# nnaisense/evotorch

Measured on NVIDIA H100. Metric: PGPE generations/sec at popsize=1Mxdim=10k (Rastrigin, fp32), higher is better.
Workload: dtype f32

## Files before the change

### evotorch_b200/_native.py

```python

from __future__ import annotations

import ctypes
import os
from ctypes import c_float, c_int, c_int64, c_size_t, c_uint64, c_void_p
from typing import Optional

import torch

_PKG = os.path.dirname(os.path.abspath(__file__))
LIB_PATH = os.path.join(_PKG, "lib", "libevok.so")

_P = c_void_p
_SIGNATURES = {
    "evok_abi_version": (c_int, []),
    "evok_launch_count": (c_uint64, []),
    "evok_error_string": (ctypes.c_char_p, [c_int]),
    "evok_sample_eval": (c_int, [c_int, _P, c_int64, _P, _P, c_int64, c_int64, c_int64, c_int, c_uint64, c_uint64, _P, _P, _P]),
    "evok_eval": (c_int, [c_int, _P, c_int64, c_int64, c_int64, _P, _P]),
    "evok_rank_workspace_bytes": (c_size_t, [c_int64]),
    "evok_rank": (c_int, [c_int, _P, c_int64, c_int, _P, _P, _P, c_size_t, _P]),
    "evok_argsort": (c_int, [_P, c_int64, c_int, _P, _P, c_size_t, _P]),
    "evok_sample_batched": (c_int, [_P, c_int64, c_int64, _P, c_int64, _P, c_int64, c_int64, c_int64, c_int64, c_int, c_uint64, c_uint64, _P]),
    "evok_rank_batched": (c_int, [c_int, _P, c_int64, c_int64, c_int, _P, _P, c_size_t, _P]),
    "evok_elite_mask_batched": (c_int, [_P, c_int64, c_int64, c_int64, _P, _P, c_size_t, _P]),
    "evok_weights_adjust_batched": (c_int, [_P, c_int64, c_int64, c_int, _P]),
    "evok_grad_batched_workspace_bytes": (c_size_t, [c_int64, c_int64, c_int64]),
    "evok_grad_batched": (c_int, [c_int, _P, c_int64, c_int64, _P, _P, c_int64, _P, c_int64, c_int64, c_int64, c_int64, c_float, c_float, _P, _P, _P,
                                  c_size_t, _P]),
    "evok_clipup_batched": (c_int, [_P, c_int64, c_int64, _P, _P, _P, _P, _P, _P]),
    "evok_sigma_update_batched": (c_int, [_P, _P, c_int64, c_int64, _P, c_int, _P, _P, _P, _P]),
    "evok_rank_table": (c_int, [_P, c_int64, c_int, _P, _P, _P, c_size_t, _P]),
    "evok_cholesky_workspace_bytes": (c_size_t, [c_int64]),
    "evok_cholesky": (c_int, [_P, c_int64, c_int64, _P, c_int64, _P, c_size_t, _P]),
    "evok_cmaes_row_weights": (c_int, [_P, _P, c_int64, c_int64, c_int64, c_int, _P, _P, _P]),
    "evok_cmaes_vector_update": (c_int, [_P, _P, c_int64, _P, _P, _P, _P, _P, c_int64, _P, c_int, _P, _P, _P]),
    "evok_weights_adjust": (c_int, [_P, c_int64, c_int, _P]),
    "evok_elite_mask": (c_int, [_P, c_int64, c_int64, _P, _P, c_size_t, _P]),
    "evok_grad_workspace_bytes": (c_size_t, [c_int64, c_int64]),
    "evok_grad": (c_int, [c_int, _P, c_int64, _P, _P, _P, c_int64, c_int64, c_float, c_float, _P, _P, _P, c_size_t, _P]),
    "evok_grad_regen": (c_int, [c_int, _P, _P, _P, c_int64, c_int64, c_int64, c_uint64, c_uint64, _P, c_float, c_float, _P, _P, _P,
                                c_size_t, _P]),
    "evok_clipup_step": (c_int, [_P, c_int64, _P, c_float, c_float, c_float, _P, _P, _P]),
    "evok_adam_step": (c_int, [_P, c_int64, _P, _P, c_int64, c_float, c_float, c_float, c_float, _P, _P, _P]),
    "evok_sgd_step": (c_int, [_P, c_int64, _P, c_int, c_float, c_float, _P, _P, _P]),
    "evok_axpy": (c_int, [_P, c_int64, c_float, _P, _P]),
    "evok_sigma_update": (c_int, [_P, _P, c_int64, c_float, c_int, _P, c_float, _P, c_float, _P, c_float, _P]),
    "evok_cem_finalize": (c_int, [_P, _P, _P, c_int64, c_int64, _P, _P, _P]),
    "evok_mlp_parameter_length": (c_int64, [c_int, _P]),
    "evok_mlp_forward": (c_int, [_P, c_int64, _P, c_int64, _P, c_int64, c_int64, c_int, _P, _P, _P]),
    "evok_mlp_forward_prep": (c_int, [_P, c_int64, _P, c_int64, _P, c_int64, c_int64, c_int, _P, _P, _P, _P, _P, c_float, c_float, c_float, _P, _P,
                                      c_size_t, _P]),
    "evok_mlp_forward_shared_workspace_bytes": (c_size_t, [c_int64, c_int64, c_int, _P]),
    "evok_mlp_forward_shared": (c_int, [_P, c_int64, c_int64, _P, c_int64, c_int64, c_int, _P, _P, _P, _P, c_size_t, _P]),
    "evok_gemm_gather_rows": (c_int, [_P, c_int64, c_int64, c_int64, c_int64, _P, c_int64, c_int64, c_int64, c_int64, c_int, _P, c_int64, _P]),
    "evok_gemm_gather_rows_workspace_bytes": (c_size_t, [c_int64, c_int64]),
    "evok_gemm_gather_rows_ws": (c_int, [_P, c_int64, c_int64, c_int64, c_int64, _P, c_int64, c_int64, c_int64, c_int64, c_int, _P, c_int64, c_int, _P, c_size_t, _P]),
    "evok_gemm_workspace_bytes": (c_size_t, [c_int64, c_int64, c_int64]),
    "evok_gemm_nt": (c_int, [_P, c_int64, _P, c_int64, c_int64, c_int64, c_int64, _P, c_int64, _P, c_int64, _P, _P, _P, c_size_t, _P]),
    "evok_gemm_nt_affine": (c_int, [_P, c_int64, _P, c_int64, c_int64, c_int64, c_int64, _P, c_int64, _P, _P, c_int64, _P, _P, c_size_t, _P]),
    "evok_transpose_pair": (c_int, [_P, c_int64, c_int64, c_int64, _P, _P, _P, c_int64, _P]),
    "evok_transpose_scale": (c_int, [_P, c_int64, c_int64, c_int64, _P, _P, c_int64, _P]),
    "evok_peer_alloc": (c_int, [c_size_t, _P, _P]),
    "evok_peer_open": (c_int, [_P, _P]),
    "evok_peer_close": (c_int, [_P]),
    "evok_peer_free": (c_int, [_P]),
    "evok_sample_eval_push": (c_int, [c_int, _P, c_int64, _P, _P, c_int64, c_int64, c_int64, c_int, c_uint64, c_uint64, _P, c_int, c_int, _P, _P,
                                      _P, _P, _P]),
    "evok_peer_push": (c_int, [_P, c_int64, c_int64, c_int, c_int, _P, _P, _P, _P]),
    "evok_peer_wait": (c_int, [_P, c_int, _P, _P, c_uint64, _P]),
    "evok_grad_push": (c_int, [c_int, _P, c_int64, _P, _P, _P, c_int64, c_int64, c_int64, c_uint64, c_uint64, _P, c_float, c_float, c_int, c_int,
                               _P, _P, _P, _P, _P, c_size_t, _P]),
    "evok_rank_sharded": (c_int, [c_int, _P, c_int64, c_int, c_int, c_int, _P, _P, _P, _P, _P, _P, _P, c_uint64, _P, _P, _P, c_size_t, _P]),
    "evok_peer_reduce": (c_int, [_P, c_int, c_int64, _P, _P, _P, _P, c_uint64, _P, _P]),
}

EXPORTED_SYMBOLS = tuple(sorted(_SIGNATURES))

_lib: Optional[ctypes.CDLL] = None


class EvokError(RuntimeError):
    pass


def lib() -> ctypes.CDLL:
    global _lib
    if _lib is None:
        if not os.path.exists(LIB_PATH):
            raise EvokError(
                f"{LIB_PATH} is missing: the sm_90a kernel library has not been built. "
                "Run `python -m evotorch_b200.build` (needs nvcc). There is no CPU/torch fallback for CUDA problems."
            )
        handle = ctypes.CDLL(LIB_PATH)
        for name, (res, args) in _SIGNATURES.items():
            fn = getattr(handle, name)
            fn.restype = res
            fn.argtypes = args
        if handle.evok_abi_version() != 1:
            raise EvokError("libevok.so ABI version mismatch; rebuild with `python -m evotorch_b200.build --force`")
        _lib = handle
    return _lib


def available() -> bool:
    return os.path.exists(LIB_PATH)


def check(rc: int, what: str) -> None:
    if rc != 0:
        msg = lib().evok_error_string(rc).decode()
        if rc < 0:
            raise ValueError(f"{what}: {msg} (code {rc})")
        raise EvokError(f"{what}: CUDA error {rc}: {msg}")


def ptr(t: Optional[torch.Tensor]) -> Optional[int]:
    return None if t is None else t.data_ptr()


def stream_of(t: torch.Tensor) -> int:
    return torch.cuda.current_stream(t.device).cuda_stream


_workspaces: dict = {}


def workspace(device: torch.device, nbytes: int, tag: str = "ws") -> torch.Tensor:
    dev = device.index if device.index is not None else torch.cuda.current_device()
    key = (dev, torch.cuda.current_stream(dev).cuda_stream, tag) if _private_depth == 0 else (dev, tag)
    buf = _workspaces.get(key)
    if buf is None or buf.numel() < nbytes:
        buf = torch.empty(max(int(nbytes), 256), dtype=torch.uint8, device=device)
        _workspaces[key] = buf
    return buf


_private_depth = 0


class private_workspaces:

    def __enter__(self) -> dict:
        global _workspaces, _private_depth
        self._saved = _workspaces
        _workspaces = self.store = {}
        _private_depth += 1
        import gc

        self._gc_was_enabled = gc.isenabled()
        gc.collect()
        gc.disable()
        return self.store

    def __exit__(self, *exc):
        global _workspaces, _private_depth
        _workspaces = self._saved
        _private_depth -= 1
        if self._gc_was_enabled:
            import gc

            gc.enable()
        return False
```

### evotorch_b200/algorithms/gaussian.py

```python

from __future__ import annotations

import math
import os
from copy import deepcopy
from typing import Optional

import torch

from .. import ops
from ..core import LazySolutionBatch, PhiloxRecipe, Problem, SolutionBatch
from ..distributed import world
from ..distributions import Distribution, ExpGaussian, ExpSeparableGaussian, SeparableGaussian, SymmetricSeparableGaussian
from ..optimizers import get_optimizer_class
from ..tools.misc import modify_tensor, to_stdev_init
from .searchalgorithm import SearchAlgorithm, SinglePopulationAlgorithmMixin


class GaussianSearchAlgorithm(SearchAlgorithm, SinglePopulationAlgorithmMixin):

    DISTRIBUTION_TYPE = NotImplemented
    DISTRIBUTION_PARAMS = NotImplemented

    def __init__(self, problem: Problem, *, popsize: int, center_learning_rate: float, stdev_learning_rate: float,
                 stdev_init=None, radius_init=None, num_interactions: Optional[int] = None, popsize_max: Optional[int] = None,
                 optimizer=None, optimizer_config: Optional[dict] = None, ranking_method: Optional[str] = None, center_init=None,
                 stdev_min=None, stdev_max=None, stdev_max_change=None, obj_index: Optional[int] = None, distributed: bool = False,
                 popsize_weighted_grad_avg: Optional[bool] = None, ensure_even_popsize: bool = False):
        problem.ensure_numeric()
        problem.ensure_unbounded()
        SearchAlgorithm.__init__(self, problem, center=self._get_mu, stdev=self._get_sigma, mean_eval=self._get_mean_eval)
        self._num_interactions = None if num_interactions is None else int(num_interactions)
        if popsize_max is not None and num_interactions is None:
            raise ValueError("`popsize_max` was expected as None, because `num_interactions` is None."
                             " The argument `popsize_max` is meaningful only when `num_interactions` is given.")
        self._popsize_max = None if popsize_max is None else int(popsize_max)
        self._ensure_even_popsize = bool(ensure_even_popsize)
        if self._ensure_even_popsize and (int(popsize) % 2) != 0 and not distributed:
            raise ValueError(f"`popsize` was expected as an even number. However, the received `popsize` is {popsize}.")

        if center_init is None:
            mu = problem.generate_values(1).reshape(-1)
        else:
            mu = problem.ensure_tensor_length_and_dtype(center_init, allow_scalar=False, about="center_init").clone()
        stdev_init = to_stdev_init(solution_length=problem.solution_length, stdev_init=stdev_init, radius_init=radius_init)
        sigma = problem.ensure_tensor_length_and_dtype(stdev_init, about="stdev_init", allow_scalar=False).clone()

        dist_params = deepcopy(self.DISTRIBUTION_PARAMS) if self.DISTRIBUTION_PARAMS is not None else {}
        dist_params.update({"mu": mu, "sigma": sigma})
        self._distribution: Distribution = self.DISTRIBUTION_TYPE(dist_params, dtype=problem.dtype, device=problem.device)

        self._popsize = int(popsize)
        self._center_learning_rate = float(center_learning_rate)
        self._stdev_learning_rate = float(stdev_learning_rate)
        self._optimizer = self._initialize_optimizer(self._center_learning_rate, optimizer, optimizer_config)
        self._ranking_method = None if ranking_method is None else str(ranking_method)

        def bound(x, about):
            return None if x is None else problem.ensure_tensor_length_and_dtype(x, about=about, allow_scalar=True)

        self._stdev_min = bound(stdev_min, "stdev_min")
        self._stdev_max = bound(stdev_max, "stdev_max")
        self._stdev_max_change = bound(stdev_max_change, "stdev_max_change")

        def host_side(x):
            return None if x is None else (float(x) if x.ndim == 0 else x)

        self._kernel_bounds = dict(lb=host_side(self._stdev_min), ub=host_side(self._stdev_max), max_change=host_side(self._stdev_max_change))
        self._obj_index = problem.normalize_obj_index(obj_index)

        self._distributed = bool(distributed) and world()[1] > 1
        self._step = self._step_distributed if self._distributed else self._step_non_distributed
        if popsize_weighted_grad_avg is not None and not distributed:
            raise ValueError("The argument `popsize_weighted_grad_avg` can only be used in distributed mode.")

        self._mean_eval = None
        self._population: Optional[SolutionBatch] = None
        self._first_iter = True
        self._use_graph = os.environ.get("EVOTORCH_B200_CUDA_GRAPH", "0") == "1"
        self._graph = None
        SinglePopulationAlgorithmMixin.__init__(self, exclude="mean_eval", enable=(not self._distributed))

    def _initialize_optimizer(self, learning_rate: float, optimizer=None, optimizer_config: Optional[dict] = None):
        if optimizer is None:
            return None
        if isinstance(optimizer, str):
            cls = get_optimizer_class(optimizer, optimizer_config)
            return cls(stepsize=float(learning_rate), dtype=self._distribution.dtype, solution_length=self._distribution.solution_length,
                       device=self._distribution.device)
        return optimizer

    def __getstate__(self) -> dict:
        state = dict(self.__dict__)
        state["_graph"] = None
        state.pop("_graph_workspaces", None)
        return state

    def _fill_and_eval_pop(self):
        if self._num_interactions is not None:
            self._fill_and_eval_adaptive_pop()
            return
        if self._population is None:
            if self.problem.lazy_population:
                self._population = LazySolutionBatch(self.problem, self._popsize, device=self._distribution.device)
            else:
                self._population = SolutionBatch(self.problem, popsize=self._popsize, device=self._distribution.device, empty=True)
        self.problem.sample_and_evaluate(self._distribution, self._population)

    def _fill_and_eval_adaptive_pop(self):
        prob = self.problem
        first = prob.status.get("total_interaction_count", 0)
        populations, total = [], 0
        while True:
            newpop = SolutionBatch(prob, popsize=self._popsize, device=self._distribution.device, empty=True)
            total += len(newpop)
            prob.sample_and_evaluate(self._distribution, newpop)
            populations.append(newpop)
            if self._popsize_max is not None and total >= self._popsize_max:
                break
            if prob.status["total_interaction_count"] - first > self._num_interactions:
                break
        self._population = populations[0] if len(populations) == 1 else SolutionBatch.cat(populations)

    def enable_cuda_graph(self, enabled: bool = True):
        self._use_graph = bool(enabled)
        self._graph = None
        return self

    def _graph_capturable(self) -> bool:
        from ..optimizers import ClipUp

        dist, prob = self._distribution, self.problem
        ok = (self._num_interactions is None and isinstance(dist, SeparableGaussian) and ops.uses_kernels(dist.mu) and prob.rng == "philox"
              and prob.evok_objective_id is not None and len(prob.senses) == 1 and prob.eval_data_length == 0
              and (self._optimizer is None or isinstance(self._optimizer, ClipUp))
              and len(prob.before_eval_hook) == 0)
        if self._distributed:
            return (ok and not prob.stores_solution_stats and len(prob.before_eval_hook) == 0 and len(prob.after_eval_hook) == 0
                    and len(prob.before_grad_hook) == 0 and len(prob.after_grad_hook) == 0)
        return ok and self._population is not None

    def _update_in_place(self, gradients: dict):
        dist = self._distribution
        gmu = gradients["mu"].contiguous()
        if self._optimizer is not None:
            self._optimizer.ascent_into_(gmu, dist.mu)
        else:
            ops.axpy_(dist.mu, gmu, self._center_learning_rate)
        ops.sigma_update_(dist.sigma, gradients["sigma"].contiguous(), self._stdev_learning_rate, isinstance(dist, ExpSeparableGaussian),
                          **self._kernel_bounds)

    def _graph_body(self, base_stream: int, counter: torch.Tensor):
        dist, prob, pop = self._distribution, self.problem, self._population
        lazy = isinstance(pop, LazySolutionBatch)
        n = len(pop)
        fitnesses = pop._evdata.view(-1)
        if lazy:
            samples = PhiloxRecipe(seed=prob._philox_seed, stream_id=base_stream - 1, row0=0, n_rows=n, solution_length=prob.solution_length,
                                   symmetric=dist.SYMMETRIC, stream_offset=counter, mu=dist.mu, sigma=dist.sigma)
        else:
            samples = pop._data
        gradients = dist.compute_gradients(samples, fitnesses, objective_sense=prob.senses[self._obj_index], ranking_method=self._ranking_method)
        self._update_in_place(gradients)
        ops.sample_eval(prob.evok_objective_id, None if lazy else samples, dist.mu, dist.sigma, n_rows=n, symmetric=dist.SYMMETRIC,
                        seed=prob._philox_seed, stream_id=base_stream, f=fitnesses, stream_offset=counter)
        counter.add_(1)
        if lazy:
            pop.recipe = PhiloxRecipe(seed=prob._philox_seed, stream_id=base_stream - 1, row0=0, n_rows=n, solution_length=prob.solution_length,
                                      symmetric=dist.SYMMETRIC, stream_offset=counter, mu=dist.mu, sigma=dist.sigma)

    def _capture_graph(self):
        prob = self.problem
        dist = self._distribution
        if not (dist.mu.is_contiguous() and dist.sigma.is_contiguous()):
            self._distribution = dist = dist.modified_copy(mu=dist.mu.contiguous(), sigma=dist.sigma.contiguous())
        self._graph_counter = torch.zeros(1, dtype=torch.int32, device=dist.mu.device)
        self._graph_base_stream = prob._philox_stream
        graph = torch.cuda.CUDAGraph()
        before = ops.launch_count()
        from .. import _native as nat

        with nat.private_workspaces() as store, torch.cuda.graph(graph):
            self._graph_body(self._graph_base_stream, self._graph_counter)
        self._graph_workspaces = store
        self._graph_kernels = ops.launch_count() - before
        ops.count_replayed_launches(-self._graph_kernels)
        self._graph_counter.zero_()
        self._graph = graph

    def _step_graph(self):
        prob, pop = self.problem, self._population
        if self._graph is None:
            self._step_eager()
            self._capture_graph()
            return
        self._graph.replay()
        ops.count_replayed_launches(self._graph_kernels)
        prob._philox_stream += 1
        prob._finish_evaluation(pop)

    def _step_non_distributed(self):
        if self._first_iter:
            self._fill_and_eval_pop()
            self._first_iter = False
            return
        if self._use_graph and self._graph_capturable():
            self._step_graph()
        else:
            self._graph = None
            self._step_eager()

    def _step_eager(self):
        lazy = isinstance(self._population, LazySolutionBatch)
        samples = self._population.recipe if lazy else self._population.access_values(keep_evals=True)
        fitnesses = self._population.access_evals()[:, self._obj_index]
        gradients = self._distribution.compute_gradients(samples, fitnesses, objective_sense=self.problem.senses[self._obj_index],
                                                         ranking_method=self._ranking_method)
        self._update_distribution(gradients)
        self._fill_and_eval_pop()

    def _distributed_body(self, in_place: bool):
        fetched = self.problem.sample_and_compute_gradients(self._distribution, self._popsize, obj_index=self._obj_index,
                                                            num_interactions=self._num_interactions, popsize_max=self._popsize_max,
                                                            ranking_method=self._ranking_method,
                                                            ensure_even_popsize=self._ensure_even_popsize)
        if in_place:
            self._update_in_place(fetched[0]["gradients"])
        else:
            self._update_distribution(fetched[0]["gradients"])
        self._mean_eval = fetched[0]["mean_eval"]

    def _sync_initial_state(self):
        from ..distributed import broadcast_search_state

        dist_ = self._distribution
        tensors = [v for v in dist_.parameters.values() if isinstance(v, torch.Tensor)]
        opt = self._optimizer
        for name in ("_velocity", "_m", "_v", "_buf"):
            t = getattr(opt, name, None) if opt is not None else None
            if isinstance(t, torch.Tensor):
                tensors.append(t)
        broadcast_search_state(tensors)
        self._state_synced = True

    def _step_distributed(self):
        prob = self.problem
        if not self.__dict__.get("_state_synced", False):
            self._sync_initial_state()
        if os.environ.get("EVOTORCH_B200_PEER", "0") == "1" and getattr(prob, "_peer_exchange", None) is None and not self.__dict__.get("_peer_tried"):
            self._peer_tried = True
            from ..distributed import world
            from ..peer import enable_peer_exchange

            if world()[1] > 1 and ops.uses_kernels(self._distribution.mu) and prob.evok_objective_id is not None and prob.rng == "philox":
                enable_peer_exchange(prob, self._popsize)
        if not (self._use_graph and self._graph_capturable()):
            self._graph = None
            self._distributed_body(in_place=False)
            return
        if self._graph is None:
            if self._steps_count < 2:
                self._distributed_body(in_place=False)
                return
            dist = self._distribution
            self._distribution = dist = dist.modified_copy(mu=dist.mu.contiguous().clone(), sigma=dist.sigma.contiguous().clone())
            prob.philox_stream_offset = torch.zeros(1, dtype=torch.int32, device=dist.mu.device)
            base = prob._philox_stream
            torch.cuda.synchronize()
            graph = torch.cuda.CUDAGraph()
            before = ops.launch_count()
            from .. import _native as nat

            with nat.private_workspaces() as store, torch.cuda.graph(graph):
                self._distributed_body(in_place=True)
                prob.philox_stream_offset.add_(1)
            self._graph_workspaces = store
            self._graph_kernels = ops.launch_count() - before
            ops.count_replayed_launches(-self._graph_kernels)
            prob._philox_stream = base
            prob.philox_stream_offset.zero_()
            self._graph = graph
        self._graph.replay()
        ops.count_replayed_launches(self._graph_kernels)
        prob._philox_stream += 1

    def _update_distribution(self, gradients: dict):
        dist = self._distribution
        separable = isinstance(dist, SeparableGaussian)
        if separable and ops.uses_kernels(dist.mu) and ops.uses_kernels(gradients["mu"]):
            new_mu, new_sigma = dist.mu.clone(), dist.sigma.clone()
            gmu = gradients["mu"].contiguous()
            if self._optimizer is not None and hasattr(self._optimizer, "ascent_into_"):
                self._optimizer.ascent_into_(gmu, new_mu)
            elif self._optimizer is not None:
                new_mu += self._optimizer.ascent(gmu)
            else:
                ops.axpy_(new_mu, gmu, self._center_learning_rate)
            ops.sigma_update_(new_sigma, gradients["sigma"].contiguous(), self._stdev_learning_rate,
                              isinstance(dist, ExpSeparableGaussian), **self._kernel_bounds)
            self._distribution = dist.modified_copy(mu=new_mu, sigma=new_sigma)
            return

        controlled = (self._stdev_min is not None) or (self._stdev_max is not None) or (self._stdev_max_change is not None)
        old_sigma = dist.sigma if controlled else None
        learning_rates, optimizers = {}, {}
        if self._optimizer is not None:
            optimizers["mu"] = self._optimizer
        else:
            learning_rates["mu"] = self._center_learning_rate
        learning_rates["sigma"] = self._stdev_learning_rate
        updated = dist.update_parameters(gradients, learning_rates=learning_rates, optimizers=optimizers)
        if controlled:
            updated = updated.modified_copy(
                sigma=modify_tensor(old_sigma, updated.sigma, lb=self._stdev_min, ub=self._stdev_max, max_change=self._stdev_max_change))
        self._distribution = updated

    def _get_mu(self) -> torch.Tensor:
        mu = self._distribution.parameters["mu"]
        return mu.clone() if self._graph is not None else mu

    def _get_sigma(self) -> torch.Tensor:
        sigma = self._distribution.parameters["sigma"]
        return sigma.clone() if self._graph is not None else sigma

    def _get_mean_eval(self) -> Optional[float]:
        if self._population is None:
            return None if self._mean_eval is None else float(self._mean_eval)
        return float(torch.mean(self._population.evals[:, self._obj_index]))

    @property
    def optimizer(self):
        return None if self._optimizer is None else self._optimizer.contained_optimizer

    @property
    def population(self) -> Optional[SolutionBatch]:
        return self._population

    @property
    def obj_index(self) -> int:
        return self._obj_index


class PGPE(GaussianSearchAlgorithm):

    DISTRIBUTION_TYPE = NotImplemented
    DISTRIBUTION_PARAMS = NotImplemented

    def __init__(self, problem: Problem, *, popsize: int, center_learning_rate: float, stdev_learning_rate: float, stdev_init=None,
                 radius_init=None, num_interactions: Optional[int] = None, popsize_max: Optional[int] = None, optimizer="clipup",
                 optimizer_config: Optional[dict] = None, ranking_method: Optional[str] = "centered", center_init=None, stdev_min=None,
                 stdev_max=None, stdev_max_change=0.2, symmetric: bool = True, obj_index: Optional[int] = None,
                 distributed: bool = False, popsize_weighted_grad_avg: Optional[bool] = None):
        if symmetric:
            self.DISTRIBUTION_TYPE = SymmetricSeparableGaussian
            divide_by = "num_directions"
        else:
            self.DISTRIBUTION_TYPE = SeparableGaussian
            divide_by = "num_solutions"
        self.DISTRIBUTION_PARAMS = {"divide_mu_grad_by": divide_by, "divide_sigma_grad_by": divide_by}
        super().__init__(problem, popsize=popsize, center_learning_rate=center_learning_rate, stdev_learning_rate=stdev_learning_rate,
                         stdev_init=stdev_init, radius_init=radius_init, popsize_max=popsize_max, num_interactions=num_interactions,
                         optimizer=optimizer, optimizer_config=optimizer_config, ranking_method=ranking_method, center_init=center_init,
                         stdev_min=stdev_min, stdev_max=stdev_max, stdev_max_change=stdev_max_change, obj_index=obj_index,
                         distributed=distributed, popsize_weighted_grad_avg=popsize_weighted_grad_avg, ensure_even_popsize=symmetric)


def _default_popsize(n: int) -> int:
    return int(4 + math.floor(3 * math.log(n)))


class SNES(GaussianSearchAlgorithm):

    DISTRIBUTION_TYPE = ExpSeparableGaussian
    DISTRIBUTION_PARAMS = None

    def __init__(self, problem: Problem, *, stdev_init=None, radius_init=None, popsize: Optional[int] = None,
                 center_learning_rate: Optional[float] = None, stdev_learning_rate: Optional[float] = None,
                 scale_learning_rate: bool = True, num_interactions: Optional[int] = None, popsize_max: Optional[int] = None,
                 optimizer=None, optimizer_config: Optional[dict] = None, ranking_method: Optional[str] = "nes", center_init=None,
                 stdev_min=None, stdev_max=None, stdev_max_change=None, obj_index: Optional[int] = None, distributed: bool = False,
                 popsize_weighted_grad_avg: Optional[bool] = None):
        n = problem.solution_length
        if popsize is None:
            popsize = _default_popsize(n)
        if center_learning_rate is None:
            center_learning_rate = 1.0
        default_lr = 0.2 * (3 + math.log(n)) / math.sqrt(n)
        if stdev_learning_rate is None:
            stdev_learning_rate = default_lr
        else:
            stdev_learning_rate = float(stdev_learning_rate) * (default_lr if scale_learning_rate else 1.0)
        super().__init__(problem, popsize=popsize, center_learning_rate=center_learning_rate, stdev_learning_rate=stdev_learning_rate,
                         stdev_init=stdev_init, radius_init=radius_init, popsize_max=popsize_max, num_interactions=num_interactions,
                         optimizer=optimizer, optimizer_config=optimizer_config, ranking_method=ranking_method, center_init=center_init,
                         stdev_min=stdev_min, stdev_max=stdev_max, stdev_max_change=stdev_max_change, obj_index=obj_index,
                         distributed=distributed, popsize_weighted_grad_avg=popsize_weighted_grad_avg)


class CEM(GaussianSearchAlgorithm):

    DISTRIBUTION_TYPE = SeparableGaussian
    DISTRIBUTION_PARAMS = NotImplemented

    def __init__(self, problem: Problem, *, popsize: int, parenthood_ratio: float, stdev_init=None, radius_init=None,
                 num_interactions: Optional[int] = None, popsize_max: Optional[int] = None, center_init=None, stdev_min=None,
                 stdev_max=None, stdev_max_change=None, obj_index: Optional[int] = None, distributed: bool = False,
                 popsize_weighted_grad_avg: Optional[bool] = None):
        self.DISTRIBUTION_PARAMS = {"parenthood_ratio": float(parenthood_ratio)}
        super().__init__(problem, popsize=popsize, center_learning_rate=1.0, stdev_learning_rate=1.0, stdev_init=stdev_init,
                         radius_init=radius_init, popsize_max=popsize_max, num_interactions=num_interactions, optimizer=None,
                         optimizer_config=None, ranking_method=None, center_init=center_init, stdev_min=stdev_min, stdev_max=stdev_max,
                         stdev_max_change=stdev_max_change, obj_index=obj_index, distributed=distributed,
                         popsize_weighted_grad_avg=popsize_weighted_grad_avg)


class XNES(GaussianSearchAlgorithm):

    DISTRIBUTION_TYPE = ExpGaussian
    DISTRIBUTION_PARAMS = None

    def __init__(self, problem: Problem, *, stdev_init=None, radius_init=None, popsize: Optional[int] = None,
                 center_learning_rate: Optional[float] = None, stdev_learning_rate: Optional[float] = None,
                 scale_learning_rate: bool = True, num_interactions: Optional[int] = None, popsize_max: Optional[int] = None,
                 optimizer=None, optimizer_config: Optional[dict] = None, ranking_method: Optional[str] = "nes", center_init=None,
                 obj_index: Optional[int] = None, distributed: bool = False, popsize_weighted_grad_avg: Optional[bool] = None):
        n = problem.solution_length
        if popsize is None:
            popsize = _default_popsize(n)
        if center_learning_rate is None:
            center_learning_rate = 1.0
        default_lr = 0.6 * (3 + math.log(n)) / (n * math.sqrt(n))
        if stdev_learning_rate is None:
            stdev_learning_rate = default_lr
        else:
            stdev_learning_rate = float(stdev_learning_rate) * (default_lr if scale_learning_rate else 1.0)
        super().__init__(problem, popsize=popsize, center_learning_rate=center_learning_rate, stdev_learning_rate=stdev_learning_rate,
                         stdev_init=stdev_init, radius_init=radius_init, popsize_max=popsize_max, num_interactions=num_interactions,
                         optimizer=optimizer, optimizer_config=optimizer_config, ranking_method=ranking_method, center_init=center_init,
                         stdev_min=None, stdev_max=None, stdev_max_change=None, obj_index=obj_index, distributed=distributed,
                         popsize_weighted_grad_avg=popsize_weighted_grad_avg)
```

### evotorch_b200/core.py

```python

from __future__ import annotations

import math
from typing import Any, Callable, Iterable, Optional, Union

import torch

from . import ops
from .tools.cloning import Clonable
from .tools.hook import Hook
from .tools.readonlytensor import as_read_only_tensor
from .tools.misc import ensure_tensor_length_and_dtype, extract_generator, make_gaussian, make_uniform, to_torch_dtype

ObjectiveSense = Union[str, Iterable[str]]


class Problem(Clonable):

    def __init__(self, objective_sense: ObjectiveSense, objective_func: Optional[Callable] = None, *, initial_bounds=None, bounds=None,
                 solution_length: Optional[int] = None, dtype=None, eval_dtype=None, device=None, eval_data_length: Optional[int] = None,
                 seed: Optional[int] = None, num_actors=None, actor_config=None, num_gpus_per_actor=None, num_subbatches=None,
                 subbatch_size=None, store_solution_stats: Optional[bool] = None, vectorized: Optional[bool] = None,
                 rng: Optional[str] = None, lazy_population: bool = False):
        if num_actors not in (None, 0, 1):
            import warnings

            warnings.warn(
                f"num_actors={num_actors!r}: evotorch_b200 has no Ray actors. The population is evaluated by this process"
                " (or sharded over the torch.distributed ranks when launched with torchrun and distributed=True is given to the"
                " searcher; see evotorch_b200.distributed).", stacklevel=2)
        self._requested_num_actors = num_actors
        self._dtype = torch.float32 if dtype is None else to_torch_dtype(dtype)
        if eval_dtype is None:
            self._eval_dtype = self._dtype if self._dtype.is_floating_point else torch.float32
        else:
            self._eval_dtype = to_torch_dtype(eval_dtype)
        self._device = torch.device("cpu") if device is None else torch.device(device)
        if solution_length is None:
            raise ValueError(f"Together with a numeric dtype ({self._dtype!r}), expected to receive `solution_length` as an integer."
                             " However, `solution_length` is None.")
        self._solution_length = int(solution_length)

        if isinstance(objective_sense, str):
            senses = [objective_sense]
        else:
            senses = list(objective_sense)
            if len(senses) == 0:
                raise ValueError("Encountered an empty sequence via `objective_sense`.")
        for s in senses:
            if s not in ("min", "max"):
                raise ValueError(f"Invalid objective sense: {s!r}. Instead, please provide the objective sense as 'min' or 'max'.")
        self._senses = senses
        self._objective_sense = objective_sense

        self._initial_lower_bounds = self._initial_upper_bounds = None
        self._lower_bounds = self._upper_bounds = None
        if bounds is not None and initial_bounds is None:
            initial_bounds = bounds
        if initial_bounds is not None:
            self._initial_lower_bounds, self._initial_upper_bounds = self._process_bounds(initial_bounds)
        if bounds is not None:
            self._lower_bounds, self._upper_bounds = self._process_bounds(bounds)

        self._objective_func = objective_func
        if objective_func is None:
            if vectorized is not None:
                raise ValueError("This problem object received no external fitness function; `vectorized` must be left as None.")
            self._vectorized = None
        elif getattr(objective_func, "__evotorch_vectorized__", False):
            if vectorized is not None:
                raise ValueError("Received a fitness function that was decorated via @vectorized; `vectorized` must be left as None.")
            self._vectorized = True
        else:
            self._vectorized = bool(vectorized)

        self._eval_data_length = 0 if eval_data_length is None else int(eval_data_length)
        self._store_solution_stats = None if store_solution_stats is None else bool(store_solution_stats)
        self._best = self._worst = None
        self._best_evals = self._worst_evals = None
        self._after_eval_status: dict = {}
        self._before_eval_hook, self._after_eval_hook = Hook(), Hook()

        self._generator = torch.Generator(device=self._device)
        self._seed = None
        self.manual_seed(seed)
        if rng is None:
            rng = "philox" if self._device.type == "cuda" and self._dtype == torch.float32 else "torch"
        if rng not in ("philox", "torch"):
            raise ValueError(f"rng must be 'philox' or 'torch', got {rng!r}")
        self.rng = rng
        self.lazy_population = bool(lazy_population)

    def _process_bounds(self, pair) -> tuple:
        lb, ub = pair
        out = []
        for b in (lb, ub):
            t = torch.as_tensor(b, dtype=self._dtype, device=self._device)
            if t.ndim not in (0, 1):
                raise ValueError(f"Lower and upper bounds are expected as scalars or as 1-dimensional vectors, got shape {tuple(t.shape)}.")
            if t.ndim == 1 and len(t) != self._solution_length:
                raise ValueError(f"Boundary vectors must have length {self._solution_length}, got {len(t)}.")
            out.append(t)
        return tuple(out)

    def manual_seed(self, seed: Optional[int] = None):
        if seed is None:
            seed = int(torch.randint(0, 2**62, (1,)).item())
            self._seed = None
        else:
            self._seed = int(seed)
        self._generator.manual_seed(int(seed))
        self._philox_seed = int(seed) & 0xFFFFFFFFFFFFFFFF
        self._philox_stream = 0
        self.philox_row0 = 0
        self.philox_stream_offset = None

    def next_philox_stream(self) -> tuple:
        sid = self._philox_stream
        self._philox_stream += 1
        return self._philox_seed, sid

    @property
    def dtype(self) -> torch.dtype:
        return self._dtype

    @property
    def eval_dtype(self) -> torch.dtype:
        return self._eval_dtype

    @property
    def device(self) -> torch.device:
        return self._device

    @property
    def generator(self) -> torch.Generator:
        return self._generator

    @property
    def has_own_generator(self) -> bool:
        return True

    @property
    def objective_sense(self) -> ObjectiveSense:
        return self._senses[0] if len(self._senses) == 1 else self._senses

    @property
    def senses(self) -> list:
        return self._senses

    @property
    def is_single_objective(self) -> bool:
        return len(self._senses) == 1

    @property
    def is_multi_objective(self) -> bool:
        return len(self._senses) > 1

    @property
    def solution_length(self) -> int:
        return self._solution_length

    @property
    def eval_data_length(self) -> int:
        return self._eval_data_length

    @property
    def initial_lower_bounds(self):
        return self._initial_lower_bounds

    @property
    def initial_upper_bounds(self):
        return self._initial_upper_bounds

    @property
    def lower_bounds(self):
        return self._lower_bounds

    @property
    def upper_bounds(self):
        return self._upper_bounds

    @property
    def num_actors(self) -> int:
        return 0

    @property
    def actors(self):
        return None

    @property
    def is_main(self) -> bool:
        return True

    @property
    def is_remote(self) -> bool:
        return False

    @property
    def before_eval_hook(self) -> Hook:
        return self._before_eval_hook

    @property
    def after_eval_hook(self) -> Hook:
        return self._after_eval_hook

    @property
    def before_grad_hook(self) -> Hook:
        return self.__dict__.setdefault("_before_grad_hook", Hook())

    @property
    def after_grad_hook(self) -> Hook:
        return self.__dict__.setdefault("_after_grad_hook", Hook())

    def is_on_cpu(self) -> bool:
        return str(self._device) == "cpu"

    def kill_actors(self):
        """No-op: there are no Ray actors here (one process per GPU replaces them, distributed.py)."""

    @property
    def all_remote_problems(self):
        raise NotImplementedError("Ray actors are out of scope: shard the population over GPUs with torchrun (evotorch_b200/distributed.py)")

    @property
    def status(self) -> dict:
        return self._after_eval_status

    @property
    def stores_solution_stats(self) -> Optional[bool]:
        return self._store_solution_stats

    @property
    def evok_objective_id(self) -> Optional[int]:
        return getattr(self._objective_func, "evok_objective_id", None)

    def _tm(self, dtype, device, use_eval_dtype=False):
        if dtype is None:
            dtype = self._eval_dtype if use_eval_dtype else self._dtype
        return to_torch_dtype(dtype), (self._device if device is None else torch.device(device))

    def _size(self, size, num_solutions):
        if num_solutions is not None:
            if len(size) > 0:
                raise ValueError("Provide either a size or `num_solutions`, not both.")
            return (int(num_solutions), self._solution_length)
        if len(size) == 1 and isinstance(size[0], (tuple, list, torch.Size)):
            return tuple(size[0])
        return tuple(int(s) for s in size)

    def make_tensor(self, data, *, dtype=None, device=None, use_eval_dtype: bool = False) -> torch.Tensor:
        dt, dev = self._tm(dtype, device, use_eval_dtype)
        return torch.as_tensor(data, dtype=dt, device=dev) if isinstance(data, torch.Tensor) else torch.tensor(data, dtype=dt, device=dev)

    def _target(self, size, num_solutions, out, dtype, device, use_eval_dtype) -> torch.Tensor:
        if out is not None:
            if len(size) > 0 or num_solutions is not None or dtype is not None or device is not None or use_eval_dtype:
                raise ValueError("When `out` is given, the arguments `size`, `num_solutions`, `dtype`, `device`, `use_eval_dtype` are not expected")
            return out
        dt, dev = self._tm(dtype, device, use_eval_dtype)
        return torch.empty(self._size(size, num_solutions), dtype=dt, device=dev)

    def make_empty(self, *size, num_solutions=None, out=None, dtype=None, device=None, use_eval_dtype: bool = False) -> torch.Tensor:
        return self._target(size, num_solutions, out, dtype, device, use_eval_dtype)

    def make_zeros(self, *size, num_solutions=None, out=None, dtype=None, device=None, use_eval_dtype: bool = False) -> torch.Tensor:
        return self._target(size, num_solutions, out, dtype, device, use_eval_dtype).zero_()

    def make_ones(self, *size, num_solutions=None, out=None, dtype=None, device=None, use_eval_dtype: bool = False) -> torch.Tensor:
        return self._target(size, num_solutions, out, dtype, device, use_eval_dtype).fill_(1)

    def make_nan(self, *size, num_solutions=None, out=None, dtype=None, device=None, use_eval_dtype: bool = False) -> torch.Tensor:
        return self._target(size, num_solutions, out, dtype, device, use_eval_dtype).fill_(float("nan"))

    def make_I(self, size=None, *, out=None, dtype=None, device=None, use_eval_dtype: bool = False) -> torch.Tensor:
        if isinstance(size, tuple):
            if len(size) != 1:
                raise ValueError(f"When the size argument is given as a tuple, the method `make_I(...)` expects the tuple to have only one"
                                 f" element. The given tuple is {size}.")
            size = size[0]
        if out is not None:
            if size is not None or dtype is not None or device is not None or use_eval_dtype:
                raise ValueError("When `out` is given, the arguments `size`, `dtype`, `device`, `use_eval_dtype` are not expected")
            if out.ndim != 2 or out.shape[0] != out.shape[1]:
                raise ValueError(f"`out` was expected as a square matrix, but its shape is {tuple(out.shape)}")
            out.zero_()
            out.fill_diagonal_(1)
            return out
        dt, dev = self._tm(dtype, device, use_eval_dtype)
        return torch.eye(self._solution_length if size is None else int(size), dtype=dt, device=dev)

    def make_gaussian(self, *size, num_solutions=None, center=None, stdev=None, symmetric: bool = False, out=None, dtype=None,
                      device=None, use_eval_dtype: bool = False, generator=None) -> torch.Tensor:
        out = self._target(size, num_solutions, out, dtype, device, use_eval_dtype)
        return make_gaussian(out=out, center=center, stdev=stdev, symmetric=symmetric,
                             generator=self._generator if generator is None else generator)

    def make_uniform(self, *size, num_solutions=None, lb=None, ub=None, out=None, dtype=None, device=None, use_eval_dtype: bool = False,
                     generator=None) -> torch.Tensor:
        out = self._target(size, num_solutions, out, dtype, device, use_eval_dtype)
        return make_uniform(out=out, lb=lb, ub=ub, generator=self._generator if generator is None else generator)

    def make_randint(self, *size, n, num_solutions=None, out=None, dtype=None, device=None, use_eval_dtype: bool = False,
                     generator=None) -> torch.Tensor:
        out = self._target(size, num_solutions, out, dtype, device, use_eval_dtype)
        gen = extract_generator(self._generator if generator is None else generator)
        n = int(n)
        if out.dtype.is_floating_point:
            out.copy_(torch.randint(0, n, out.shape, generator=gen, device=out.device, dtype=torch.int64))
        else:
            out.random_(0, n, generator=gen)
        return out

    def make_uniform_shaped_like(self, t: torch.Tensor, *, lb=None, ub=None) -> torch.Tensor:
        return self.make_uniform(out=torch.empty_like(t), lb=lb, ub=ub)

    def make_gaussian_shaped_like(self, t: torch.Tensor, *, center=None, stdev=None) -> torch.Tensor:
        return self.make_gaussian(out=torch.empty_like(t), center=center, stdev=stdev)

    def ensure_tensor_length_and_dtype(self, t: Any, *, allow_scalar: bool = False, about: Optional[str] = None) -> torch.Tensor:
        return ensure_tensor_length_and_dtype(t, self._solution_length, self._dtype, about=about, allow_scalar=allow_scalar,
                                              device=self._device)

    def generate_values(self, num_solutions: int) -> torch.Tensor:
        result = torch.empty(int(num_solutions), self._solution_length, dtype=self._dtype, device=self._device)
        self._fill(result)
        return result

    def _fill(self, values: torch.Tensor):
        if self._initial_lower_bounds is None or self._initial_upper_bounds is None:
            raise RuntimeError(
                "The default implementation of the method `_fill(...)` does not know how to initialize solutions because it appears"
                " that this Problem object was not given neither `initial_bounds` nor `bounds` during the moment of initialization."
            )
        return self.make_uniform(out=values, lb=self._initial_lower_bounds, ub=self._initial_upper_bounds)

    def generate_batch(self, popsize: Optional[int] = None, *, empty: bool = False, center=None, stdev=None,
                       symmetric: bool = False) -> "SolutionBatch":
        if (center is None) != (stdev is None):
            raise ValueError("The arguments `center` and `stdev` were expected to be None or non-None at the same time.")
        if center is None:
            if symmetric:
                raise ValueError("The argument `symmetric` can be set as True only when `center` and `stdev` are provided.")
            return SolutionBatch(self, popsize, empty=empty, device=self._device)
        if empty:
            raise ValueError("When `center` and `stdev` are provided, the argument `empty` must be False.")
        result = SolutionBatch(self, popsize, device=self._device, empty=True)
        self.make_gaussian(out=result.access_values(), center=center, stdev=stdev, symmetric=symmetric)
        return result

    def ensure_numeric(self):
        if not (self._dtype.is_floating_point or self._dtype in (torch.int32, torch.int64, torch.int16, torch.int8)):
            raise ValueError("Expected a problem with numeric dtype.")

    def ensure_unbounded(self):
        if self._lower_bounds is not None or self._upper_bounds is not None:
            raise ValueError("Expected an unbounded problem. However, this problem object has its `lower_bounds` and/or `upper_bounds` set.")

    def ensure_single_objective(self):
        if len(self._senses) != 1:
            raise ValueError(f"Expected a single-objective problem, but this problem has {len(self._senses)} objectives.")

    def normalize_obj_index(self, obj_index: Optional[int] = None) -> int:
        n = len(self._senses)
        if obj_index is None:
            if n == 1:
                return 0
            raise ValueError("This problem has multiple objectives: `obj_index` must be given.")
        obj_index = int(obj_index)
        if not (-n <= obj_index < n):
            raise IndexError(f"Objective index out of range: {obj_index}")
        return obj_index % n

    @torch.no_grad()
    def evaluate(self, x: Union["SolutionBatch", "Solution"]):
        if isinstance(x, Solution):
            batch = x.to_batch()
        elif isinstance(x, SolutionBatch):
            batch = x
        else:
            raise TypeError(f"The method `evaluate(...)` expected a Solution or a SolutionBatch as its argument, got {type(x)!r}.")
        self._before_eval_hook(batch)
        self._evaluate_all(batch)
        self._finish_evaluation(batch)

    @property
    def aux_device(self) -> torch.device:
        if self._device.type == "cpu":
            return torch.device("cuda") if torch.cuda.is_available() else self._device
        return self._device

    def _device_of_fitness_function(self) -> Optional[torch.device]:
        for fn in (self._objective_func, self._evaluate_batch, self._evaluate):
            if fn is None:
                continue
            if getattr(fn, "__evotorch_on_aux_device__", False):
                return self.aux_device
            if hasattr(fn, "device"):
                return torch.device(fn.device)
        return None

    def _evaluate_all(self, batch: "SolutionBatch"):
        wanted = self._device_of_fitness_function()
        if wanted is None or torch.device(wanted) == batch.device:
            self._evaluate_batch(batch)
            return
        moved = batch.to(wanted)
        self._evaluate_batch(moved)
        batch._evdata[:] = moved._evdata.to(batch.device)

    def _finish_evaluation(self, batch: "SolutionBatch"):
        self._after_eval_status = {}
        self._after_eval_status.update(self._get_best_and_worst(batch))
        self._after_eval_status.update(self._extra_status(batch))
        self._after_eval_status.update(self._after_eval_hook.accumulate_dict(batch))

    def _extra_status(self, batch: "SolutionBatch") -> dict:
        return {}

    def _evaluate_batch(self, batch: "SolutionBatch"):
        if self._vectorized and self._objective_func is not None:
            result = self._objective_func(batch.values)
            if isinstance(result, tuple):
                batch.set_evals(*result)
            else:
                batch.set_evals(result)
        else:
            for sln in batch:
                self._evaluate(sln)

    def _evaluate(self, solution: "Solution"):
        if self._objective_func is None:
            raise NotImplementedError
        result = self._objective_func(solution.values)
        if isinstance(result, tuple):
            solution.set_evals(*result)
        else:
            solution.set_evals(result)

    def _get_best_and_worst(self, batch: "SolutionBatch") -> dict:
        if self._store_solution_stats is None:
            self._store_solution_stats = str(batch.device) == "cpu"
        if not self._store_solution_stats:
            return {}
        nobjs = len(self._senses)
        if self._best is None:
            self._best, self._worst = [None] * nobjs, [None] * nobjs
            self._best_evals = [math.inf if s == "min" else -math.inf for s in self._senses]
            self._worst_evals = [-math.inf if s == "min" else math.inf for s in self._senses]
        for i, sense in enumerate(self._senses):
            scores = batch.access_evals(i)
            ibest, iworst = batch.argbest(i), batch.argworst(i)
            best_score, worst_score = float(scores[ibest]), float(scores[iworst])
            better = best_score < self._best_evals[i] if sense == "min" else best_score > self._best_evals[i]
            worse = worst_score > self._worst_evals[i] if sense == "min" else worst_score < self._worst_evals[i]
            if better:
                self._best_evals[i], self._best[i] = best_score, batch[int(ibest)].clone()
            if worse:
                self._worst_evals[i], self._worst[i] = worst_score, batch[int(iworst)].clone()
        if nobjs == 1:
            return dict(best=self._best[0], worst=self._worst[0], best_eval=float(self._best[0].evals[0]),
                        worst_eval=float(self._worst[0].evals[0]))
        return {"best": self._best, "worst": self._worst}

    _TRANSIENT = ("_peer_exchange", "_active_peer", "_grad_batches", "_grad_scratch", "_d2h_stage")

    def __getstate__(self) -> dict:
        state = {k: v for k, v in self.__dict__.items() if k not in self._TRANSIENT}
        state["philox_stream_offset"] = None
        return state

    def sample_and_evaluate(self, distribution, batch: "SolutionBatch"):
        obj = self.evok_objective_id
        if isinstance(batch, LazySolutionBatch):
            if not (obj is not None and self.rng == "philox" and len(self._senses) == 1 and hasattr(distribution, "SYMMETRIC")
                    and ops.uses_kernels(distribution.mu)):
                raise ValueError("a lazy population needs a built-in objective, rng='philox', a separable Gaussian and CUDA float32")
            n = len(batch)
            if distribution.SYMMETRIC and n % 2 != 0:
                raise ValueError(f"Symmetric sampling cannot be done if the number of solutions is odd: {n}")
            seed, stream_id = self.next_philox_stream()
            mu, sigma = distribution.mu.contiguous(), distribution.sigma.contiguous()
            batch.recipe = PhiloxRecipe(seed=seed, stream_id=stream_id, row0=self.philox_row0, n_rows=n, solution_length=self._solution_length,
                                        symmetric=distribution.SYMMETRIC, stream_offset=self.philox_stream_offset, mu=mu, sigma=sigma)
            self._before_eval_hook(batch)
            peer = getattr(self, "_active_peer", None)
            if peer is not None:
                ops.sample_eval_push(obj, None, mu, sigma, n_rows=n, symmetric=distribution.SYMMETRIC, seed=seed, stream_id=stream_id,
                                     row0=self.philox_row0, peer=peer, stream_offset=self.philox_stream_offset)
            else:
                ops.sample_eval(obj, None, mu, sigma, n_rows=n, symmetric=distribution.SYMMETRIC, seed=seed, stream_id=stream_id,
                                row0=self.philox_row0, f=batch._evdata.view(-1), stream_offset=self.philox_stream_offset)
            self._finish_evaluation(batch)
            return
        values = batch.access_values()
        fused = (obj is not None and self.rng == "philox" and ops.uses_kernels(values) and len(self._senses) == 1
                 and hasattr(distribution, "SYMMETRIC") and ops.uses_kernels(distribution.mu) and len(self._before_eval_hook) == 0)
        if not fused:
            distribution.sample(out=values, generator=self)
            self.evaluate(batch)
            return
        n = values.shape[0]
        if distribution.SYMMETRIC and n % 2 != 0:
            raise ValueError(f"Symmetric sampling cannot be done if the leftmost dimension of the target tensor is odd: {tuple(values.shape)}")
        seed, stream_id = self.next_philox_stream()
        evdata = batch._evdata
        direct = evdata.shape[1] == 1 and evdata.dtype == torch.float32 and evdata.is_contiguous()
        f = evdata.view(-1) if direct else torch.empty(n, dtype=torch.float32, device=values.device)
        peer = getattr(self, "_active_peer", None)
        if peer is not None:
            ops.sample_eval_push(obj, values, distribution.mu.contiguous(), distribution.sigma.contiguous(), n_rows=n,
                                 symmetric=distribution.SYMMETRIC, seed=seed, stream_id=stream_id, row0=self.philox_row0, peer=peer,
                                 stream_offset=self.philox_stream_offset)
            self._finish_evaluation(batch)
            return
        ops.sample_eval(obj, values, distribution.mu.contiguous(), distribution.sigma.contiguous(), n_rows=n,
                        symmetric=distribution.SYMMETRIC, seed=seed, stream_id=stream_id, row0=self.philox_row0, f=f,
                        stream_offset=self.philox_stream_offset)
        if not direct:
            batch.set_evals(f)
        self._finish_evaluation(batch)

    def sample_and_compute_gradients(self, distribution, popsize: int, *, num_interactions: Optional[int] = None,
                                     popsize_max: Optional[int] = None, obj_index: Optional[int] = None,
                                     ranking_method: Optional[str] = None, with_stats: bool = True,
                                     ensure_even_popsize: bool = False):
        from .distributed import adaptive_sample_and_gradients, sharded_sample_and_gradients

        popsize = int(popsize)
        if ensure_even_popsize and popsize % 2 != 0:
            popsize += 1
        obj_index = self.normalize_obj_index(obj_index)
        hooks = self.__dict__
        if len(hooks.get("_before_grad_hook", ())) >= 1:
            hooks["_before_grad_hook"]()
        if num_interactions is not None:
            result = adaptive_sample_and_gradients(self, distribution, popsize, num_interactions=int(num_interactions),
                                                   popsize_max=None if popsize_max is None else int(popsize_max), obj_index=obj_index,
                                                   ranking_method=ranking_method)
        else:
            result = sharded_sample_and_gradients(self, distribution, popsize, obj_index=obj_index, ranking_method=ranking_method)
        if len(hooks.get("_after_grad_hook", ())) >= 1:
            self._after_eval_status = hooks["_after_grad_hook"].accumulate_dict([result])
        return [result] if with_stats else result["gradients"]

    def _get_local_interaction_count(self) -> int:
        if "total_interaction_count" in self._after_eval_status:
            return int(self._after_eval_status["total_interaction_count"])
        raise NotImplementedError

    def compare_solutions(self, a: "Solution", b: "Solution", obj_index: Optional[int] = None) -> float:
        i = self.normalize_obj_index(obj_index)
        sign = 1.0 if self._senses[i] == "max" else -1.0
        return sign * float(a.evals[i] - b.evals[i])

    def is_better(self, a, b, obj_index=None) -> bool:
        return self.compare_solutions(a, b, obj_index) > 0

    def is_worse(self, a, b, obj_index=None) -> bool:
        return self.compare_solutions(a, b, obj_index) < 0


class SolutionBatch:

    def __init__(self, problem: Optional[Problem] = None, popsize: Optional[int] = None, *, device=None, slice_of=None,
                 like: Optional["SolutionBatch"] = None, merging_of: Iterable = None, empty: Optional[bool] = None):
        if slice_of is not None:
            source, sl = slice_of
            self._data = source._data[sl]
            self._evdata = source._evdata[sl]
            self._senses = source._senses
            self._num_objs = source._num_objs
            return
        if merging_of is not None:
            batches = list(merging_of)
            self._data = torch.cat([b._data for b in batches], dim=0)
            self._evdata = torch.cat([b._evdata for b in batches], dim=0)
            self._senses = batches[0]._senses
            self._num_objs = batches[0]._num_objs
            return
        if like is not None and problem is None:
            popsize = len(like) if popsize is None else int(popsize)
            device = like.device if device is None else device
            self._data = torch.empty(popsize, like._data.shape[1], dtype=like._data.dtype, device=device)
            self._evdata = torch.full((popsize, like._evdata.shape[1]), float("nan"), dtype=like._evdata.dtype, device=device)
            self._senses, self._num_objs = like._senses, like._num_objs
            return
        if problem is None or popsize is None:
            if like is not None and problem is not None and popsize is None:
                popsize = len(like)
            else:
                raise ValueError("SolutionBatch needs `problem` and `popsize` (or `like`, `slice_of`, `merging_of`).")
        device = problem.device if device is None else torch.device(device)
        popsize = int(popsize)
        self._senses = problem.senses
        self._num_objs = len(problem.senses)
        self._data = torch.empty(popsize, problem.solution_length, dtype=problem.dtype, device=device)
        self._evdata = torch.full((popsize, self._num_objs + problem.eval_data_length), float("nan"), dtype=problem.eval_dtype,
                                  device=device)
        if not empty:
            problem._fill(self._data)

    def __len__(self) -> int:
        return self._data.shape[0]

    def __iter__(self):
        for i in range(len(self)):
            yield self[i]

    def __getitem__(self, i):
        if isinstance(i, slice):
            return SolutionBatch(slice_of=(self, i))
        if isinstance(i, (list, torch.Tensor)):
            return self.take(i)
        i = int(i)
        n = len(self)
        if not (-n <= i < n):
            raise IndexError(f"Solution index out of range: {i}")
        return Solution(self, i % n)

    @property
    def device(self) -> torch.device:
        return self._data.device

    @property
    def dtype(self) -> torch.dtype:
        return self._data.dtype

    values_dtype = dtype

    @property
    def eval_dtype(self) -> torch.dtype:
        return self._evdata.dtype

    @property
    def values_shape(self) -> torch.Size:
        return self._data.shape

    @property
    def eval_shape(self) -> torch.Size:
        return self._evdata.shape

    @property
    def solution_length(self) -> int:
        return self._data.shape[1]

    @property
    def senses(self) -> list:
        return self._senses

    @property
    def objective_sense(self):
        return self._senses[0] if len(self._senses) == 1 else self._senses

    @property
    def values(self) -> torch.Tensor:
        return as_read_only_tensor(self._data)

    @property
    def evals(self) -> torch.Tensor:
        return as_read_only_tensor(self._evdata)

    def access_values(self, *, keep_evals: bool = False) -> torch.Tensor:
        if not keep_evals:
            self.forget_evals()
        return self._data

    def access_evals(self, obj_index: Optional[int] = None) -> torch.Tensor:
        return self._evdata if obj_index is None else self._evdata[:, self._normalize_obj_index(obj_index)]

    def forget_evals(self, *, solutions=None):
        if solutions is None:
            self._evdata.fill_(float("nan"))
        else:
            self._evdata[solutions] = float("nan")

    def _normalize_obj_index(self, i) -> int:
        if i is None:
            if self._num_objs != 1:
                raise ValueError("The objective index was expected as an integer (multi-objective batch).")
            return 0
        i = int(i)
        if not (-self._num_objs <= i < self._num_objs):
            raise IndexError(f"Objective index out of range: {i}")
        return i % self._num_objs

    def set_values(self, values: Any, *, solutions=None):
        if solutions is None:
            solutions = slice(None, None, None)
        self._data[solutions] = torch.as_tensor(values, dtype=self._data.dtype, device=self._data.device)
        self._evdata[solutions] = float("nan")

    def set_evals(self, evals: torch.Tensor, eval_data: Optional[torch.Tensor] = None, *, solutions=None):
        if solutions is None:
            solutions = slice(None, None, None)
        num_solutions = self._evdata[solutions].shape[0]
        evals = torch.as_tensor(evals, dtype=self._evdata.dtype, device=self._evdata.device)
        if evals.ndim == 1:
            if self._num_objs != 1 and eval_data is None and evals.shape[0] == num_solutions:
                raise ValueError("A 1-dimensional `evals` tensor can only be used with single-objective problems.")
            evals = evals.reshape(-1, 1)
        elif evals.ndim != 2:
            raise ValueError(f"`evals` was expected with 1 or 2 dimensions, got shape {tuple(evals.shape)}")
        if evals.shape[0] != num_solutions:
            raise ValueError(f"Number of evaluation results ({evals.shape[0]}) does not match the number of solutions ({num_solutions}).")
        total_cols = self._evdata.shape[1]
        if eval_data is not None:
            eval_data = torch.as_tensor(eval_data, dtype=self._evdata.dtype, device=self._evdata.device).reshape(num_solutions, -1)
            if evals.shape[1] != self._num_objs or eval_data.shape[1] != total_cols - self._num_objs:
                raise ValueError("Shapes of `evals` / `eval_data` do not match the problem's objectives / eval_data_length.")
            self._evdata[solutions, : self._num_objs] = evals
            self._evdata[solutions, self._num_objs:] = eval_data
        elif evals.shape[1] == total_cols:
            self._evdata[solutions] = evals
        elif evals.shape[1] == self._num_objs:
            self._evdata[solutions, : self._num_objs] = evals
            self._evdata[solutions, self._num_objs:] = float("nan")
        else:
            raise ValueError(f"`evals` has {evals.shape[1]} columns; expected {self._num_objs} or {total_cols}.")

    def _sort_keys(self, obj_index) -> tuple:
        i = self._normalize_obj_index(obj_index)
        return self._evdata[:, i], self._senses[i] == "max"

    def argsort(self, obj_index: Optional[int] = None) -> torch.Tensor:
        keys, descending = self._sort_keys(obj_index)
        if ops.uses_kernels(keys):
            return ops.argsort(keys.contiguous(), descending)
        return torch.argsort(keys, descending=descending, stable=True)

    def argbest(self, obj_index: Optional[int] = None) -> torch.Tensor:
        keys, is_max = self._sort_keys(obj_index)
        return torch.argmax(keys) if is_max else torch.argmin(keys)

    def argworst(self, obj_index: Optional[int] = None) -> torch.Tensor:
        keys, is_max = self._sort_keys(obj_index)
        return torch.argmin(keys) if is_max else torch.argmax(keys)

    def utility(self, obj_index: Optional[int] = None, *, ranking_method: Optional[str] = None) -> torch.Tensor:
        from .tools.ranking import rank

        keys, is_max = self._sort_keys(obj_index)
        return rank(keys, "raw" if ranking_method is None else ranking_method, higher_is_better=is_max)

    def utils(self, *, ranking_method: Optional[str] = None) -> torch.Tensor:
        return torch.stack([self.utility(i, ranking_method=ranking_method) for i in range(self._num_objs)], dim=1)

    def take(self, indices: Iterable) -> "SolutionBatch":
        idx = torch.as_tensor(indices, device=self._data.device)
        out = SolutionBatch(like=self, popsize=len(idx))
        out._data[:] = self._data[idx]
        out._evdata[:] = self._evdata[idx]
        return out

    def take_best(self, n: int, *, obj_index: Optional[int] = None) -> "SolutionBatch":
        return self.take(self.argsort(obj_index)[: int(n)])

    def split(self, num_pieces: Optional[int] = None, *, max_size: Optional[int] = None) -> list:
        n = len(self)
        if (num_pieces is None) == (max_size is None):
            raise ValueError("Provide exactly one of `num_pieces` and `max_size`.")
        if num_pieces is None:
            num_pieces = math.ceil(n / int(max_size))
        from .tools.misc import split_workload

        pieces, start = [], 0
        for share in split_workload(n, int(num_pieces)):
            pieces.append(SolutionBatch(slice_of=(self, slice(start, start + share))))
            start += share
        return pieces

    def concat(self, other: Union["SolutionBatch", Iterable]) -> "SolutionBatch":
        others = [other] if isinstance(other, SolutionBatch) else list(other)
        return SolutionBatch(merging_of=[self, *others])

    @staticmethod
    def cat(solution_batches: Iterable) -> "SolutionBatch":
        return SolutionBatch(merging_of=list(solution_batches))

    def to(self, device) -> "SolutionBatch":
        if torch.device(device) == self.device:
            return self
        out = SolutionBatch(like=self, device=device)
        out._data[:] = self._data.to(device)
        out._evdata[:] = self._evdata.to(device)
        return out

    def clone(self) -> "SolutionBatch":
        out = SolutionBatch(like=self)
        out._data[:] = self._data
        out._evdata[:] = self._evdata
        return out

    def __copy__(self) -> "SolutionBatch":
        return self.clone()

    def __deepcopy__(self, memo) -> "SolutionBatch":
        return self.clone()

    def __repr__(self) -> str:
        return f"<SolutionBatch: {len(self)} x {self.solution_length}, {self.dtype}, {self.device}>"


class PhiloxRecipe:

    def __init__(self, *, seed: int, stream_id: int, row0: int, n_rows: int, solution_length: int, symmetric: bool,
                 stream_offset: Optional[torch.Tensor], mu: torch.Tensor, sigma: torch.Tensor):
        self.seed, self.stream_id, self.row0, self.n_rows = seed, stream_id, row0, n_rows
        self.solution_length, self.symmetric, self.stream_offset = solution_length, symmetric, stream_offset
        self.mu, self.sigma = mu, sigma

    @property
    def shape(self) -> tuple:
        return (self.n_rows, self.solution_length)

    def materialize(self) -> torch.Tensor:
        out = torch.empty(self.n_rows, self.solution_length, dtype=torch.float32, device=self.mu.device)
        ops.sample_eval(ops.OBJ_NONE, out, self.mu, self.sigma, n_rows=self.n_rows, symmetric=self.symmetric, seed=self.seed,
                        stream_id=self.stream_id, row0=self.row0, stream_offset=self.stream_offset)
        return out


class LazySolutionBatch(SolutionBatch):

    def __init__(self, problem: "Problem", popsize: int, *, device=None):
        device = problem.device if device is None else torch.device(device)
        self._senses = problem.senses
        self._num_objs = len(problem.senses)
        self._popsize, self._solution_length = int(popsize), problem.solution_length
        self._values_dtype = problem.dtype
        self._evdata = torch.full((int(popsize), self._num_objs + problem.eval_data_length), float("nan"), dtype=problem.eval_dtype,
                                  device=device)
        self.recipe: Optional[PhiloxRecipe] = None

    @property
    def _data(self) -> torch.Tensor:
        if self.recipe is None:
            raise ValueError("This lazy population has not been sampled yet.")
        return self.recipe.materialize()

    def __len__(self) -> int:
        return self._popsize

    @property
    def device(self) -> torch.device:
        return self._evdata.device

    @property
    def dtype(self) -> torch.dtype:
        return self._values_dtype

    values_dtype = dtype

    @property
    def solution_length(self) -> int:
        return self._solution_length

    @property
    def values_shape(self) -> torch.Size:
        return torch.Size((self._popsize, self._solution_length))

    def access_values(self, *, keep_evals: bool = False) -> torch.Tensor:
        if not keep_evals:
            raise ValueError("The decision values of a lazy population are read-only (they are a function of the Philox counters).")
        return self._data

    def set_values(self, values: Any, *, solutions=None):
        raise ValueError("The decision values of a lazy population are read-only (they are a function of the Philox counters).")

    def __getitem__(self, i):
        if isinstance(i, (slice, list, torch.Tensor)):
            raise NotImplementedError("slicing a lazy population is not supported; use `.values` to materialise it")
        i = int(i) % self._popsize
        out = SolutionBatch(like=None, problem=None, popsize=None, slice_of=(_Materialized(self, i), slice(0, 1)))
        return Solution(out, 0)

    def __repr__(self) -> str:
        return f"<LazySolutionBatch: {self._popsize} x {self._solution_length}, {self.device}>"


class _Materialized:

    def __init__(self, lazy: LazySolutionBatch, i: int):
        r = lazy.recipe
        first = (i // 2) * 2 if r.symmetric else i
        rows = 2 if r.symmetric else 1
        block = torch.empty(rows, r.solution_length, dtype=torch.float32, device=r.mu.device)
        ops.sample_eval(ops.OBJ_NONE, block, r.mu, r.sigma, n_rows=rows, symmetric=r.symmetric, seed=r.seed, stream_id=r.stream_id,
                        row0=r.row0 + first, stream_offset=r.stream_offset)
        self._data = block[i - first: i - first + 1]
        self._evdata = lazy._evdata[i: i + 1]
        self._senses, self._num_objs = lazy._senses, lazy._num_objs


class Solution:

    def __init__(self, parent: SolutionBatch, index: int):
        self._batch = parent[int(index): int(index) + 1]

    @property
    def values(self) -> torch.Tensor:
        return as_read_only_tensor(self._batch._data[0])

    @property
    def evals(self) -> torch.Tensor:
        return as_read_only_tensor(self._batch._evdata[0])

    @property
    def evaluation(self) -> torch.Tensor:
        return as_read_only_tensor(self._batch._evdata[0])

    def access_values(self, *, keep_evals: bool = False) -> torch.Tensor:
        return self._batch.access_values(keep_evals=keep_evals)[0]

    def access_evals(self) -> torch.Tensor:
        return self._batch.access_evals()[0]

    def set_values(self, values: Any):
        self._batch.set_values(torch.as_tensor(values, dtype=self._batch.dtype, device=self._batch.device).reshape(1, -1))

    def set_evals(self, evals, eval_data=None):
        evals = torch.as_tensor(evals, dtype=self._batch.eval_dtype, device=self._batch.device).reshape(1, -1)
        if eval_data is not None:
            eval_data = torch.as_tensor(eval_data, dtype=self._batch.eval_dtype, device=self._batch.device).reshape(1, -1)
        self._batch.set_evals(evals, eval_data)

    set_evaluation = set_evals

    @property
    def is_evaluated(self) -> bool:
        n = self._batch._num_objs
        return not bool(torch.any(torch.isnan(self._batch._evdata[0, :n])))

    @property
    def senses(self) -> list:
        return self._batch.senses

    @property
    def objective_sense(self):
        return self._batch.objective_sense

    @property
    def dtype(self) -> torch.dtype:
        return self._batch.dtype

    @property
    def eval_dtype(self) -> torch.dtype:
        return self._batch.eval_dtype

    @property
    def device(self) -> torch.device:
        return self._batch.device

    @property
    def shape(self) -> torch.Size:
        return self.values.shape

    def __len__(self) -> int:
        return self._batch.solution_length

    def __iter__(self):
        return iter(self.values)

    def __getitem__(self, i):
        return self.values[i]

    def clone(self) -> "Solution":
        return Solution(self._batch.clone(), 0)

    def __copy__(self) -> "Solution":
        return self.clone()

    def __deepcopy__(self, memo) -> "Solution":
        return self.clone()

    def to(self, device) -> "Solution":
        return Solution(self._batch.to(device), 0)

    def to_batch(self) -> SolutionBatch:
        return self._batch

    def __repr__(self) -> str:
        return f"<Solution values={self.values}, evals={self.evals}>"
```

### evotorch_b200/csrc/evok_grad.cu

```cuda
#include <cstdlib>

#include "evok_common.cuh"

#ifndef EVOK_GRAD_TMA_DEFAULT
#define EVOK_GRAD_TMA_DEFAULT 1
#endif

namespace evok {

#ifndef EVOK_GRAD_UNROLL
#define EVOK_GRAD_UNROLL 4
#endif
#ifndef EVOK_GRAD_MINB
#define EVOK_GRAD_MINB 4
#endif
#ifndef EVOK_GRAD_CTAS_PER_SM
#define EVOK_GRAD_CTAS_PER_SM 4
#endif
constexpr int kGradThreads = 256;
constexpr int kGradUnroll = EVOK_GRAD_UNROLL;
constexpr int kMaxResidentCtas = kNumSMs * 8;

template <int VEC>
struct VecF;
template <>
struct VecF<4> {
  float v[4];
};
template <>
struct VecF<1> {
  float v[1];
};

template <int VEC>
__device__ __forceinline__ VecF<VEC> load_row(const float* p) {
  VecF<VEC> r;
  if (VEC == 4) {
    const float4 t = ld_stream4(p);
    r.v[0] = t.x; r.v[1] = t.y; r.v[2] = t.z; r.v[3] = t.w;
  } else {
    r.v[0] = ld_stream1(p);
  }
  return r;
}

struct GradItems {
  int64_t x, w, mu, sigma, partial;
};

template <int VEC, int TX, bool SYM, bool REGEN>
__global__ void __launch_bounds__(kGradThreads, EVOK_GRAD_MINB)
    grad_partial_kernel(int form, const float* __restrict__ X, int64_t ldx, const float* __restrict__ w, const float* __restrict__ mu,
                        const float* __restrict__ sigma, int64_t n_units, int64_t D, int64_t units_per_chunk, uint64_t unit0,
                        const __grid_constant__ PhiloxKey key, const uint32_t* __restrict__ stream_off, float* __restrict__ partial,
                        const __grid_constant__ GradItems items) {
  constexpr int TY = kGradThreads / TX;
  if (gridDim.z > 1) {
    const int64_t item = blockIdx.z;
    X += item * items.x;
    w += item * items.w;
    mu += item * items.mu;
    sigma += item * items.sigma;
    partial += item * items.partial;
  }
  const uint32_t sw = key.stream_lo + ((REGEN && stream_off) ? __ldg(stream_off) : 0u);
  const int tx = threadIdx.x % TX, ty = threadIdx.x / TX;
  const int64_t col = ((int64_t)blockIdx.x * TX + tx) * VEC;
  const bool active = col < D;

  float m[VEC], c1[VEC], c0[VEC], sg[VEC];
#pragma unroll
  for (int c = 0; c < VEC; ++c) {
    const bool ok = active && (col + c < D);
    const float s = ok ? __ldg(sigma + col + c) : 1.0f;
    m[c] = ok ? __ldg(mu + col + c) : 0.0f;
    sg[c] = s;
    if (form == EVOK_GRAD_EXP) {
      c1[c] = __fdiv_rn(1.0f, s * s);
      c0[c] = 1.0f;
    } else if (form == EVOK_GRAD_MOMENTS) {
      c1[c] = 1.0f;
      c0[c] = 0.0f;
    } else {
      c1[c] = __fdiv_rn(1.0f, s);
      c0[c] = s;
    }
  }

  float s1[VEC], s2[VEC];
#pragma unroll
  for (int c = 0; c < VEC; ++c) s1[c] = s2[c] = 0.0f;

  const int64_t r_begin = (int64_t)blockIdx.y * units_per_chunk;
  const int64_t r_end = min(n_units, r_begin + units_per_chunk);

  for (int64_t r0 = r_begin + ty; r0 < r_end; r0 += (int64_t)TY * kGradUnroll) {
    float a[kGradUnroll], b[kGradUnroll];
    bool need[kGradUnroll];
    VecF<VEC> x[kGradUnroll];
#pragma unroll
    for (int u = 0; u < kGradUnroll; ++u) {
      const int64_t r = r0 + (int64_t)u * TY;
      a[u] = b[u] = 0.0f;
      if (r < r_end) {
        if (SYM) {
          const float wp = __ldg(w + 2 * r), wm = __ldg(w + 2 * r + 1);
          a[u] = 0.5f * (wp - wm);
          b[u] = 0.5f * (wp + wm);
        } else {
          a[u] = b[u] = __ldg(w + r);
        }
      }
      need[u] = active && (a[u] != 0.0f || b[u] != 0.0f);
    }
#pragma unroll
    for (int u = 0; u < kGradUnroll; ++u) {
      const int64_t r = r0 + (int64_t)u * TY;
      if (need[u]) {
        if (REGEN) {
          if (VEC == 4) {
            normals4(key, sw, unit0 + (uint64_t)r, (uint32_t)(col >> 2), x[u].v);
          } else {
            float z[4];
            normals4(key, sw, unit0 + (uint64_t)r, (uint32_t)(col >> 2), z);
            x[u].v[0] = z[col & 3];
          }
        } else {
          x[u] = load_row<VEC>(X + (SYM ? 2 * r : r) * ldx + col);
        }
      }
    }
#pragma unroll
    for (int u = 0; u < kGradUnroll; ++u) {
      if (need[u]) {
#pragma unroll
        for (int c = 0; c < VEC; ++c) {
          const float e = REGEN ? sg[c] * x[u].v[c] : x[u].v[c] - m[c];
          s1[c] = fmaf(a[u], e, s1[c]);
          s2[c] = fmaf(b[u], fmaf(e * e, c1[c], -c0[c]), s2[c]);
        }
      }
    }
  }

  __shared__ float red[TY > 1 ? TY : 1][TX][2 * VEC];
  if (TY > 1) {
#pragma unroll
    for (int c = 0; c < VEC; ++c) {
      red[ty][tx][c] = s1[c];
      red[ty][tx][VEC + c] = s2[c];
    }
    __syncthreads();
    if (ty == 0) {
#pragma unroll
      for (int c = 0; c < VEC; ++c) {
        float t1 = red[0][tx][c], t2 = red[0][tx][VEC + c];
        for (int y = 1; y < TY; ++y) {
          t1 += red[y][tx][c];
          t2 += red[y][tx][VEC + c];
        }
        s1[c] = t1;
        s2[c] = t2;
      }
    }
  }
  if (ty == 0 && active) {
    float* p1 = partial + ((int64_t)blockIdx.y * 2 + 0) * D + col;
    float* p2 = partial + ((int64_t)blockIdx.y * 2 + 1) * D + col;
#pragma unroll
    for (int c = 0; c < VEC; ++c) {
      if (col + c < D) {
        p1[c] = s1[c];
        p2[c] = s2[c];
      }
    }
  }
}

__global__ void __launch_bounds__(256) grad_finalize_kernel(const float* __restrict__ partial, int n_chunks, int64_t D, float scale_mu,
                                                            float scale_sigma, float* __restrict__ out_mu, float* __restrict__ out_sigma,
                                                            int64_t item_stride_partial = 0) {
  const int64_t j = (int64_t)blockIdx.x * blockDim.x + threadIdx.x;
  if (j >= D) return;
  partial += (int64_t)blockIdx.y * item_stride_partial;
  out_mu += (int64_t)blockIdx.y * D;
  out_sigma += (int64_t)blockIdx.y * D;
  float t1 = 0.0f, t2 = 0.0f;
  for (int c = 0; c < n_chunks; ++c) {
    t1 += partial[((int64_t)c * 2 + 0) * D + j];
    t2 += partial[((int64_t)c * 2 + 1) * D + j];
  }
  out_mu[j] = t1 * scale_mu;
  out_sigma[j] = t2 * scale_sigma;
}

struct GradPush {
  PeerSink sink;
  const unsigned long long* epoch;
  unsigned int* done;
};

__global__ void __launch_bounds__(256) grad_finalize_push_kernel(const float* __restrict__ partial, int n_chunks, int64_t D, float scale_mu,
                                                                 float scale_sigma, const __grid_constant__ PeerSink sink,
                                                                 const unsigned long long* epoch, unsigned int* done) {
  const int64_t j = (int64_t)blockIdx.x * blockDim.x + threadIdx.x;
  if (j < D) {
    float t1 = 0.0f, t2 = 0.0f;
    for (int c = 0; c < n_chunks; ++c) {
      t1 += partial[((int64_t)c * 2 + 0) * D + j];
      t2 += partial[((int64_t)c * 2 + 1) * D + j];
    }
    t1 *= scale_mu;
    t2 *= scale_sigma;
    for (int p = 0; p < sink.world; ++p) {
      float* slot = static_cast<float*>(sink.data[p]) + (int64_t)sink.rank * 2 * D;
      slot[j] = t1;
      slot[D + j] = t2;
    }
  }
  peer_signal_tail(sink, epoch, done);
}

static int launch_finalize(const float* partial, int n_chunks, int64_t D, float scale_mu, float scale_sigma, float* out_mu, float* out_sigma,
                           const GradPush* push, cudaStream_t st) {
  const unsigned grid = (unsigned)((D + 255) / 256);
  if (push) grad_finalize_push_kernel<<<grid, 256, 0, st>>>(partial, n_chunks, D, scale_mu, scale_sigma, push->sink, push->epoch, push->done);
  else grad_finalize_kernel<<<grid, 256, 0, st>>>(partial, n_chunks, D, scale_mu, scale_sigma, out_mu, out_sigma);
  EVOK_CHECK_LAUNCH();
  return 0;
}

#ifndef EVOK_GRAD_TMA_ROWS
#define EVOK_GRAD_TMA_ROWS 4
#endif
#ifndef EVOK_GRAD_TMA_STAGES
#define EVOK_GRAD_TMA_STAGES 4
#endif
#ifndef EVOK_GRAD_TMA_CTAS_PER_SM
#define EVOK_GRAD_TMA_CTAS_PER_SM 3
#endif
constexpr int kTmaRows = EVOK_GRAD_TMA_ROWS;
constexpr int kTmaStages = EVOK_GRAD_TMA_STAGES;
constexpr int kTmaCols = 1024;
constexpr int kTmaConsumers = 256;
constexpr int kTmaThreads = kTmaConsumers + 32;
constexpr size_t kTmaSmemBytes = (size_t)kTmaStages * kTmaRows * kTmaCols * sizeof(float) + 2 * kTmaStages * sizeof(uint64_t) + 128;

__device__ __forceinline__ uint32_t smem_u32(const void* p) { return (uint32_t)__cvta_generic_to_shared(p); }
__device__ __forceinline__ void mbar_init(uint64_t* bar, uint32_t count) {
  asm volatile("mbarrier.init.shared::cta.b64 [%0], %1;" ::"r"(smem_u32(bar)), "r"(count) : "memory");
}
__device__ __forceinline__ void mbar_expect_tx(uint64_t* bar, uint32_t bytes) {
  asm volatile("mbarrier.arrive.expect_tx.shared::cta.b64 _, [%0], %1;" ::"r"(smem_u32(bar)), "r"(bytes) : "memory");
}
__device__ __forceinline__ void mbar_arrive(uint64_t* bar) {
  asm volatile("mbarrier.arrive.shared::cta.b64 _, [%0];" ::"r"(smem_u32(bar)) : "memory");
}
__device__ __forceinline__ void mbar_wait(uint64_t* bar, uint32_t parity) {
  asm volatile(
      "{\n"
      ".reg .pred P1;\n"
      "LAB_WAIT:\n"
      "mbarrier.try_wait.parity.shared::cta.b64 P1, [%0], %1;\n"
      "@P1 bra DONE;\n"
      "bra LAB_WAIT;\n"
      "DONE:\n"
      "}" ::"r"(smem_u32(bar)), "r"(parity) : "memory");
}
__device__ __forceinline__ void bulk_load(void* dst_smem, const void* src_gmem, uint32_t bytes, uint64_t* bar) {
  asm volatile("cp.async.bulk.shared::cluster.global.mbarrier::complete_tx::bytes [%0], [%1], %2, [%3];" ::"r"(smem_u32(dst_smem)),
               "l"(src_gmem), "r"(bytes), "r"(smem_u32(bar))
               : "memory");
}

template <bool SYM>
__global__ void __launch_bounds__(kTmaThreads, EVOK_GRAD_TMA_CTAS_PER_SM)
    grad_partial_tma_kernel(int form, const float* __restrict__ X, int64_t ldx, const float* __restrict__ w, const float* __restrict__ mu,
                            const float* __restrict__ sigma, int64_t n_units, int64_t D, int64_t units_per_chunk,
                            float* __restrict__ partial) {
  extern __shared__ __align__(128) unsigned char smem_raw[];
  float* tiles = reinterpret_cast<float*>(smem_raw);
  uint64_t* full = reinterpret_cast<uint64_t*>(smem_raw + (size_t)kTmaStages * kTmaRows * kTmaCols * sizeof(float));
  uint64_t* empty = full + kTmaStages;

  const int tid = threadIdx.x, warp = tid >> 5, lane = tid & 31;
  const int64_t col0 = (int64_t)blockIdx.x * kTmaCols;
  const int64_t width = min((int64_t)kTmaCols, D - col0);
  const int64_t r_begin = (int64_t)blockIdx.y * units_per_chunk;
  const int64_t r_end = min(n_units, r_begin + units_per_chunk);
  const int64_t n_rows = r_end - r_begin;
  const int64_t n_groups = (n_rows + kTmaRows - 1) / kTmaRows;
  const int64_t row_stride = (SYM ? 2 : 1) * ldx;

  if (tid == 0) {
    for (int s = 0; s < kTmaStages; ++s) {
      mbar_init(&full[s], 1);
      mbar_init(&empty[s], kTmaConsumers / 32);
    }
    asm volatile("fence.mbarrier_init.release.cluster;" ::: "memory");
  }
  __syncthreads();

  if (warp == kTmaConsumers / 32) {
    if (lane == 0) {
      const uint32_t row_bytes = (uint32_t)(width * sizeof(float));
      for (int64_t g = 0; g < n_groups; ++g) {
        const int s = (int)(g % kTmaStages);
        const uint32_t use = (uint32_t)(g / kTmaStages);
        if (use > 0) mbar_wait(&empty[s], (use - 1) & 1);
        const int64_t r0 = r_begin + g * kTmaRows;
        const int rows = (int)min((int64_t)kTmaRows, r_end - r0);
        mbar_expect_tx(&full[s], rows * row_bytes);
        float* dst = tiles + (size_t)s * kTmaRows * kTmaCols;
        for (int i = 0; i < rows; ++i) bulk_load(dst + (size_t)i * kTmaCols, X + (r0 + i) * row_stride + col0, row_bytes, &full[s]);
      }
    }
    return;
  }

  const int64_t col = col0 + (int64_t)tid * 4;
  const bool active = col < D;
  float m[4], c1[4], c0[4];
#pragma unroll
  for (int c = 0; c < 4; ++c) {
    const float sg = active ? __ldg(sigma + col + c) : 1.0f;
    m[c] = active ? __ldg(mu + col + c) : 0.0f;
    if (form == EVOK_GRAD_EXP) {
      c1[c] = __fdiv_rn(1.0f, sg * sg);
      c0[c] = 1.0f;
    } else if (form == EVOK_GRAD_MOMENTS) {
      c1[c] = 1.0f;
      c0[c] = 0.0f;
    } else {
      c1[c] = __fdiv_rn(1.0f, sg);
      c0[c] = sg;
    }
  }
  float s1[4] = {0.f, 0.f, 0.f, 0.f}, s2[4] = {0.f, 0.f, 0.f, 0.f};

  for (int64_t g = 0; g < n_groups; ++g) {
    const int s = (int)(g % kTmaStages);
    const uint32_t use = (uint32_t)(g / kTmaStages);
    const int64_t r0 = r_begin + g * kTmaRows;
    const int rows = (int)min((int64_t)kTmaRows, r_end - r0);
    float a[kTmaRows], b[kTmaRows];
#pragma unroll
    for (int i = 0; i < kTmaRows; ++i) {
      a[i] = b[i] = 0.0f;
      if (i < rows) {
        if (SYM) {
          const float wp = __ldg(w + 2 * (r0 + i)), wm = __ldg(w + 2 * (r0 + i) + 1);
          a[i] = 0.5f * (wp - wm);
          b[i] = 0.5f * (wp + wm);
        } else {
          a[i] = b[i] = __ldg(w + r0 + i);
        }
      }
    }
    mbar_wait(&full[s], use & 1);
    const float4* tile = reinterpret_cast<const float4*>(tiles + (size_t)s * kTmaRows * kTmaCols) + tid;
    if (active) {
#pragma unroll
      for (int i = 0; i < kTmaRows; ++i) {
        if (i < rows) {
          const float4 v = tile[(size_t)i * (kTmaCols / 4)];
          const float x[4] = {v.x, v.y, v.z, v.w};
#pragma unroll
          for (int c = 0; c < 4; ++c) {
            const float e = x[c] - m[c];
            s1[c] = fmaf(a[i], e, s1[c]);
            s2[c] = fmaf(b[i], fmaf(e * e, c1[c], -c0[c]), s2[c]);
          }
        }
      }
    }
    __syncwarp();
    if (lane == 0) mbar_arrive(&empty[s]);
  }
  if (active) {
    float* p1 = partial + ((int64_t)blockIdx.y * 2 + 0) * D + col;
    float* p2 = partial + ((int64_t)blockIdx.y * 2 + 1) * D + col;
#pragma unroll
    for (int c = 0; c < 4; ++c) {
      p1[c] = s1[c];
      p2[c] = s2[c];
    }
  }
}

struct GradPlan {
  int vec, tx, n_coltiles, n_chunks;
  int64_t units_per_chunk;
};

static GradPlan plan_grad(int64_t n_units, int64_t D, bool vec_ok) {
  GradPlan p;
  p.vec = vec_ok ? 4 : 1;
  const int64_t col_threads = (D + p.vec - 1) / p.vec;
  p.tx = 32;
  while (p.tx < kGradThreads && p.tx < col_threads) p.tx <<= 1;
  p.n_coltiles = (int)((col_threads + p.tx - 1) / p.tx);
  const int ty = kGradThreads / p.tx;
  int64_t chunks = (int64_t)kNumSMs * EVOK_GRAD_CTAS_PER_SM / p.n_coltiles;
  const int64_t max_useful = (n_units + (int64_t)ty * kGradUnroll * 16 - 1) / ((int64_t)ty * kGradUnroll * 16);
  if (chunks > max_useful) chunks = max_useful;
  if (chunks < 1) chunks = 1;
  if (chunks > 65535) chunks = 65535;
  p.units_per_chunk = (n_units + chunks - 1) / chunks;
  p.n_chunks = (int)((n_units + p.units_per_chunk - 1) / p.units_per_chunk);
  if (p.n_chunks < 1) p.n_chunks = 1;
  return p;
}

template <int VEC, bool SYM, bool REGEN>
static void launch_partial(const GradPlan& p, int form, const float* X, int64_t ldx, const float* w, const float* mu, const float* sigma,
                           int64_t n_units, int64_t D, uint64_t unit0, uint64_t seed, uint64_t stream_id, const uint32_t* stream_off, float* partial,
                           cudaStream_t st, int64_t n_items = 1, const GradItems* items = nullptr) {
  dim3 grid(p.n_coltiles, p.n_chunks, (unsigned)n_items);
  const PhiloxKey key = make_philox_key(seed, stream_id);
  const GradItems it = items ? *items : GradItems{0, 0, 0, 0, 0};
#define EVOK_LAUNCH_TX(TXV)                                                                                                         \
  grad_partial_kernel<VEC, TXV, SYM, REGEN><<<grid, kGradThreads, 0, st>>>(form, X, ldx, w, mu, sigma, n_units, D, p.units_per_chunk, \
                                                                           unit0, key, stream_off, partial, it)
  switch (p.tx) {
    case 32: EVOK_LAUNCH_TX(32); break;
    case 64: EVOK_LAUNCH_TX(64); break;
    case 128: EVOK_LAUNCH_TX(128); break;
    default: EVOK_LAUNCH_TX(256); break;
  }
#undef EVOK_LAUNCH_TX
}

static int grad_impl(int form, const float* X, int64_t ldx, const float* w, const float* mu, const float* sigma, int64_t row0, int64_t n_rows,
                     int64_t D, bool regen, uint64_t seed, uint64_t stream_id, const uint32_t* stream_off, float scale_mu, float scale_sigma, float* out_mu,
                     float* out_sigma, void* ws, size_t ws_bytes, void* stream, const GradPush* push = nullptr) {
  if (!w || !mu || !sigma || !ws || (!regen && !X) || (!push && (!out_mu || !out_sigma))) return EVOK_E_NULLPTR;
  if (form < EVOK_GRAD_SEPARABLE || form > EVOK_GRAD_MOMENTS) return EVOK_E_BADENUM;
  if (n_rows < 0 || D <= 0 || row0 < 0 || (!regen && ldx < D)) return EVOK_E_BADSIZE;
  const bool sym = form == EVOK_GRAD_SYMMETRIC;
  if (sym && ((n_rows & 1) || (row0 & 1))) return EVOK_E_ODDROWS;
  if (ws_bytes < evok_grad_workspace_bytes(n_rows, D)) return EVOK_E_WORKSPACE;
  cudaStream_t st = (cudaStream_t)stream;
  const int64_t n_units = sym ? n_rows / 2 : n_rows;
  const bool vec_ok = regen ? true : ((D % 4 == 0) && (ldx % 4 == 0) && aligned16(X));
  const uint64_t unit0 = (uint64_t)(sym ? row0 / 2 : row0);
  GradPlan p = plan_grad(n_units, D, vec_ok);
  float* partial = (float*)ws;
  if (n_units == 0 && push) return launch_finalize(partial, 0, D, scale_mu, scale_sigma, nullptr, nullptr, push, st);
  if (n_units == 0) {
    cudaMemsetAsync(out_mu, 0, (size_t)D * 4, st);
    cudaMemsetAsync(out_sigma, 0, (size_t)D * 4, st);
    return 0;
  }
  const char* tma_env = getenv("EVOK_GRAD_TMA");
  const int use_tma = tma_env ? atoi(tma_env) : EVOK_GRAD_TMA_DEFAULT;
  if (use_tma && !regen && vec_ok && form != EVOK_GRAD_MOMENTS && D >= 512 && n_units >= 4096) {
    const int n_coltiles = (int)((D + kTmaCols - 1) / kTmaCols);
    int64_t chunks = (int64_t)kNumSMs * EVOK_GRAD_TMA_CTAS_PER_SM / n_coltiles;
    if (chunks < 1) chunks = 1;
    if (chunks > 65535) chunks = 65535;
    const int64_t upc = (n_units + chunks - 1) / chunks;
    const int n_chunks = (int)((n_units + upc - 1) / upc);
    dim3 grid(n_coltiles, n_chunks);
    if (sym) {
      cudaFuncSetAttribute(grad_partial_tma_kernel<true>, cudaFuncAttributeMaxDynamicSharedMemorySize, (int)kTmaSmemBytes);
      grad_partial_tma_kernel<true><<<grid, kTmaThreads, kTmaSmemBytes, st>>>(form, X, ldx, w, mu, sigma, n_units, D, upc, partial);
    } else {
      cudaFuncSetAttribute(grad_partial_tma_kernel<false>, cudaFuncAttributeMaxDynamicSharedMemorySize, (int)kTmaSmemBytes);
      grad_partial_tma_kernel<false><<<grid, kTmaThreads, kTmaSmemBytes, st>>>(form, X, ldx, w, mu, sigma, n_units, D, upc, partial);
    }
    EVOK_CHECK_LAUNCH();
    return launch_finalize(partial, n_chunks, D, scale_mu, scale_sigma, out_mu, out_sigma, push, st);
  }
  if (regen) {
    if (sym) launch_partial<4, true, true>(p, form, X, ldx, w, mu, sigma, n_units, D, unit0, seed, stream_id, stream_off, partial, st);
    else launch_partial<4, false, true>(p, form, X, ldx, w, mu, sigma, n_units, D, unit0, seed, stream_id, stream_off, partial, st);
  } else if (vec_ok) {
    if (sym) launch_partial<4, true, false>(p, form, X, ldx, w, mu, sigma, n_units, D, unit0, seed, stream_id, stream_off, partial, st);
    else launch_partial<4, false, false>(p, form, X, ldx, w, mu, sigma, n_units, D, unit0, seed, stream_id, stream_off, partial, st);
  } else {
    if (sym) launch_partial<1, true, false>(p, form, X, ldx, w, mu, sigma, n_units, D, unit0, seed, stream_id, stream_off, partial, st);
    else launch_partial<1, false, false>(p, form, X, ldx, w, mu, sigma, n_units, D, unit0, seed, stream_id, stream_off, partial, st);
  }
  EVOK_CHECK_LAUNCH();
  return launch_finalize(partial, p.n_chunks, D, scale_mu, scale_sigma, out_mu, out_sigma, push, st);
}

}

using namespace evok;

extern "C" EVOK_API size_t evok_grad_workspace_bytes(int64_t n_rows, int64_t D) {
  (void)n_rows;
  if (D <= 0) return 256;
  return ((size_t)kMaxResidentCtas * 1024 + 2 * (size_t)D + 64) * sizeof(float);
}

extern "C" EVOK_API int evok_grad(int form, const float* X, int64_t ldx, const float* w, const float* mu, const float* sigma, int64_t n_rows,
                         int64_t D, float scale_mu, float scale_sigma, float* out_mu, float* out_sigma, void* ws, size_t ws_bytes,
                         void* stream) {
  return grad_impl(form, X, ldx, w, mu, sigma, 0, n_rows, D, false, 0, 0, nullptr, scale_mu, scale_sigma, out_mu, out_sigma, ws, ws_bytes, stream);
}

extern "C" EVOK_API int evok_grad_regen(int form, const float* w, const float* mu, const float* sigma, int64_t row0, int64_t n_rows, int64_t D,
                               uint64_t seed, uint64_t stream_id, const uint32_t* stream_offset_dev, float scale_mu, float scale_sigma,
                               float* out_mu, float* out_sigma, void* ws, size_t ws_bytes, void* stream) {
  return grad_impl(form, nullptr, 0, w, mu, sigma, row0, n_rows, D, true, seed, stream_id, stream_offset_dev, scale_mu, scale_sigma, out_mu, out_sigma, ws,
                   ws_bytes, stream);
}

extern "C" EVOK_API int evok_grad_push(int form, const float* X, int64_t ldx, const float* w, const float* mu, const float* sigma, int64_t row0,
                                       int64_t n_rows, int64_t D, uint64_t seed, uint64_t stream_id, const uint32_t* stream_offset_dev,
                                       float scale_mu, float scale_sigma, int world, int rank, void* const* peer_slots, void* const* peer_flags,
                                       const uint64_t* epoch_dev, uint32_t* done_dev, void* ws, size_t ws_bytes, void* stream) {
  if (!peer_slots || !peer_flags || !epoch_dev || !done_dev) return EVOK_E_NULLPTR;
  if (world < 1 || world > EVOK_MAX_PEERS || rank < 0 || rank >= world) return EVOK_E_BADSIZE;
  GradPush push{};
  push.sink.world = world;
  push.sink.rank = rank;
  for (int p = 0; p < world; ++p) {
    if (!peer_slots[p] || !peer_flags[p]) return EVOK_E_NULLPTR;
    push.sink.data[p] = peer_slots[p];
    push.sink.flags[p] = static_cast<unsigned long long*>(peer_flags[p]);
  }
  push.epoch = reinterpret_cast<const unsigned long long*>(epoch_dev);
  push.done = done_dev;
  return grad_impl(form, X, X ? ldx : 0, w, mu, sigma, row0, n_rows, D, X == nullptr, seed, stream_id, stream_offset_dev, scale_mu, scale_sigma, nullptr,
                   nullptr, ws, ws_bytes, stream, &push);
}

extern "C" EVOK_API size_t evok_grad_batched_workspace_bytes(int64_t n_items, int64_t n_rows, int64_t D) {
  if (n_items <= 0 || D <= 0) return 256;
  (void)n_rows;
  return ((size_t)kMaxResidentCtas * 1024 + 4 * (size_t)n_items * (size_t)D + 64) * sizeof(float);
}

extern "C" EVOK_API int evok_grad_batched(int form, const float* X, int64_t item_stride_x, int64_t ldx, const float* w, const float* mu,
                                          int64_t item_stride_mu, const float* sigma, int64_t item_stride_sigma, int64_t n_items, int64_t n_rows,
                                          int64_t D, float scale_mu, float scale_sigma, float* out_mu, float* out_sigma, void* ws, size_t ws_bytes,
                                          void* stream) {
  if (!X || !w || !mu || !sigma || !out_mu || !out_sigma || !ws) return EVOK_E_NULLPTR;
  if (form < EVOK_GRAD_SEPARABLE || form > EVOK_GRAD_MOMENTS) return EVOK_E_BADENUM;
  if (n_items < 0 || n_items > 65535 || n_rows < 0 || D <= 0 || ldx < D) return EVOK_E_BADSIZE;
  const bool sym = form == EVOK_GRAD_SYMMETRIC;
  if (sym && (n_rows & 1)) return EVOK_E_ODDROWS;
  if (n_items == 0) return 0;
  cudaStream_t st = (cudaStream_t)stream;
  const int64_t n_units = sym ? n_rows / 2 : n_rows;
  if (n_units == 0) {
    cudaMemsetAsync(out_mu, 0, (size_t)n_items * D * 4, st);
    cudaMemsetAsync(out_sigma, 0, (size_t)n_items * D * 4, st);
    return 0;
  }
  const bool vec_ok = (D % 4 == 0) && (ldx % 4 == 0) && aligned16(X) && item_stride_x % 4 == 0 && item_stride_mu % 4 == 0 && item_stride_sigma % 4 == 0;
  GradPlan p = plan_grad(n_units, D, vec_ok);
  int64_t chunks = ((int64_t)kNumSMs * EVOK_GRAD_CTAS_PER_SM + (int64_t)p.n_coltiles * n_items - 1) / ((int64_t)p.n_coltiles * n_items);
  if (chunks < p.n_chunks) {
    if (chunks < 1) chunks = 1;
    p.units_per_chunk = (n_units + chunks - 1) / chunks;
    p.n_chunks = (int)((n_units + p.units_per_chunk - 1) / p.units_per_chunk);
  }
  GradItems items;
  items.x = item_stride_x;
  items.w = n_rows;
  items.mu = item_stride_mu;
  items.sigma = item_stride_sigma;
  items.partial = (int64_t)p.n_chunks * 2 * D;
  if (ws_bytes < (size_t)n_items * items.partial * sizeof(float)) return EVOK_E_WORKSPACE;
  float* partial = (float*)ws;
  if (vec_ok) {
    if (sym) launch_partial<4, true, false>(p, form, X, ldx, w, mu, sigma, n_units, D, 0, 0, 0, nullptr, partial, st, n_items, &items);
    else launch_partial<4, false, false>(p, form, X, ldx, w, mu, sigma, n_units, D, 0, 0, 0, nullptr, partial, st, n_items, &items);
  } else {
    if (sym) launch_partial<1, true, false>(p, form, X, ldx, w, mu, sigma, n_units, D, 0, 0, 0, nullptr, partial, st, n_items, &items);
    else launch_partial<1, false, false>(p, form, X, ldx, w, mu, sigma, n_units, D, 0, 0, 0, nullptr, partial, st, n_items, &items);
  }
  EVOK_CHECK_LAUNCH();
  grad_finalize_kernel<<<dim3((unsigned)((D + 255) / 256), (unsigned)n_items), 256, 0, st>>>(partial, p.n_chunks, D, scale_mu, scale_sigma, out_mu,
                                                                                             out_sigma, items.partial);
  EVOK_CHECK_LAUNCH();
  return 0;
}
```

### evotorch_b200/distributed.py

```python

from __future__ import annotations

import os
from typing import Optional

import torch
import torch.distributed as dist

from .tools.misc import split_workload
from .tools.ranking import rank


def world() -> tuple:
    if dist.is_available() and dist.is_initialized():
        return dist.get_rank(), dist.get_world_size()
    return 0, 1


def shard_rows(popsize: int, world_size: int, rank_: int, symmetric: bool) -> tuple:
    unit = 2 if symmetric else 1
    if popsize % unit != 0:
        raise ValueError(f"popsize ({popsize}) must be even for a symmetric distribution")
    shares = split_workload(popsize // unit, world_size)
    row0 = unit * sum(shares[:rank_])
    return row0, unit * shares[rank_], [unit * s for s in shares]


def all_gather_rows(local: torch.Tensor, counts: list) -> torch.Tensor:
    rank_, ws = world()
    if ws == 1:
        return local
    if len(set(counts)) == 1:
        out = torch.empty(sum(counts), dtype=local.dtype, device=local.device)
        dist.all_gather_into_tensor(out, local.contiguous())
        return out
    width = max(counts)
    padded = torch.zeros(width, dtype=local.dtype, device=local.device)
    padded[: local.numel()] = local
    gathered = torch.empty(ws * width, dtype=local.dtype, device=local.device)
    dist.all_gather_into_tensor(gathered, padded)
    return torch.cat([gathered[r * width: r * width + counts[r]] for r in range(ws)])


def broadcast_seed(problem) -> None:
    rank_, ws = world()
    if ws == 1 or getattr(problem, "_seed_synced", False):
        return
    t = torch.tensor([problem._philox_seed & 0x7FFFFFFFFFFFFFFF, problem._philox_stream], dtype=torch.int64, device=problem.device)
    dist.broadcast(t, src=0)
    problem._philox_seed, problem._philox_stream = int(t[0].item()), int(t[1].item())
    if problem.rng == "torch":
        problem.generator.manual_seed((problem._philox_seed + 0x9E3779B97F4A7C15 * (rank_ + 1)) & 0x7FFFFFFFFFFFFFFF)
    problem._seed_synced = True


def broadcast_search_state(tensors: list) -> None:
    rank_, ws = world()
    if ws == 1:
        return
    for t in tensors:
        if isinstance(t, torch.Tensor) and t.numel() > 0:
            if t.is_contiguous():
                dist.broadcast(t, src=0)
            else:
                c = t.contiguous()
                dist.broadcast(c, src=0)
                t.copy_(c)


def _results_to_home(problem, grads: dict, mean_eval: torch.Tensor, home_device: torch.device) -> tuple:
    if home_device == problem.device:
        return grads, mean_eval
    if home_device.type != "cpu" or problem.device.type != "cuda":
        return {k: v.to(home_device) for k, v in grads.items()}, mean_eval.to(home_device)
    keys = sorted(grads)
    sizes = [grads[k].numel() for k in keys]
    total = sum(sizes) + 1
    stage = problem.__dict__.get("_d2h_stage")
    if stage is None or stage[0].numel() != total:
        stage = problem.__dict__["_d2h_stage"] = (torch.empty(total, dtype=torch.float32).pin_memory(),
                                                  torch.empty(total, dtype=torch.float32, device=problem.device))
    host, dev = stage
    off = 0
    for k, n in zip(keys, sizes):
        dev[off:off + n].copy_(grads[k].reshape(-1))
        off += n
    dev[off:off + 1].copy_(mean_eval.reshape(1))
    host.copy_(dev, non_blocking=True)
    torch.cuda.current_stream(problem.device).synchronize()
    out, off = {}, 0
    for k, n in zip(keys, sizes):
        out[k] = host[off:off + n].clone().reshape(grads[k].shape)
        off += n
    return out, host[off].clone()


def _usable_peer_exchange(problem, dev_dist, popsize: int, ws: int):
    peer = getattr(problem, "_peer_exchange", None)
    if peer is None or ws == 1:
        return None
    from . import ops

    ok = (peer.popsize == popsize and peer.world == ws and problem.evok_objective_id is not None and problem.rng == "philox"
          and len(problem.senses) == 1 and problem.eval_data_length == 0 and hasattr(dev_dist, "partial_gradients")
          and hasattr(dev_dist, "SYMMETRIC") and ops.uses_kernels(dev_dist.mu) and len(problem.before_eval_hook) == 0)
    if not ok:
        raise ValueError("the attached PeerExchange does not fit this generation (needs: same popsize and world size, a built-in "
                         "objective, rng='philox', one objective, a separable Gaussian on CUDA float32, no before_eval_hook)")
    return peer


def sharded_sample_and_gradients(problem, distribution, popsize: int, *, obj_index: int, ranking_method: Optional[str]) -> dict:
    from .core import LazySolutionBatch, SolutionBatch

    rank_, ws = world()
    home_device = distribution.device
    dev_dist = distribution.to(problem.device)
    symmetric = bool(getattr(dev_dist, "SYMMETRIC", False))
    if ws > 1 and not hasattr(dev_dist, "partial_gradients"):
        raise NotImplementedError(f"{type(dev_dist).__name__} cannot be sharded over ranks (full-covariance search is a small-D method)")
    row0, n_local, counts = shard_rows(popsize, ws, rank_, symmetric)
    broadcast_seed(problem)

    peer = _usable_peer_exchange(problem, dev_dist, popsize, ws)
    cache = problem.__dict__.setdefault("_grad_batches", {})
    batch = cache.get(n_local)
    if batch is None:
        if problem.lazy_population:
            batch = cache[n_local] = LazySolutionBatch(problem, n_local, device=problem.device)
        else:
            batch = cache[n_local] = SolutionBatch(problem, n_local, device=problem.device, empty=True)
        if peer is not None:
            batch._evdata = peer.f_all[row0:row0 + n_local].view(n_local, 1)
    sense = problem.senses[obj_index]
    method = "raw" if ranking_method is None else ranking_method
    sharded_rank = (peer is not None and method in ("centered", "linear", "nes") and dev_dist.accepts_local_weights(method)
                    and os.environ.get("EVOTORCH_B200_SHARDED_RANK", "0") == "1")
    push_in_sampler = peer is not None and not sharded_rank and os.environ.get("EVOTORCH_B200_PUSH_IN_SAMPLER", "0") == "1"
    problem.philox_row0 = row0
    problem._active_peer = peer if push_in_sampler else None
    try:
        problem.sample_and_evaluate(dev_dist, batch)
    finally:
        problem.philox_row0 = 0
        problem._active_peer = None

    samples = batch.recipe if isinstance(batch, LazySolutionBatch) else batch.access_values(keep_evals=True)
    if sharded_rank:
        offsets = [0]
        for c in counts:
            offsets.append(offsets[-1] + c)
        scratch = problem.__dict__.setdefault("_grad_scratch", {})
        w_local = scratch.get(n_local)
        if w_local is None:
            w_local = scratch[n_local] = torch.empty(n_local, dtype=torch.float32, device=problem.device)
        w_local, mean_buf = peer.rank_sharded(batch._evdata.view(-1), method, sense == "max", offsets, w_local)
        dev_dist._peer = peer
        try:
            summed = dev_dist.partial_gradients(samples, w_local, row0, method, local_weights_of=popsize)
        finally:
            dev_dist._peer = None
        grads = dev_dist.finalize_gradients(summed, popsize)
        mean_eval = mean_buf.reshape(())
        grads, mean_eval = _results_to_home(problem, grads, mean_eval, home_device)
        return {"gradients": grads, "num_solutions": popsize, "mean_eval": mean_eval}
    if peer is not None:
        if not push_in_sampler:
            peer.push_fitness(row0, n_local)
        f_all = peer.wait_fitness()
    else:
        f_local = batch.access_evals(obj_index)
        f_all = all_gather_rows(f_local.to(dev_dist.dtype), counts)
    weights_all = rank(f_all, method, higher_is_better=(sense == "max"))

    if peer is not None:
        dev_dist._peer = peer
        try:
            summed = dev_dist.partial_gradients(samples, weights_all, row0, method)
        finally:
            dev_dist._peer = None
        grads = dev_dist.finalize_gradients(summed, popsize)
    elif hasattr(dev_dist, "partial_gradients"):
        partial = dev_dist.partial_gradients(samples, weights_all, row0, method)
        if ws > 1:
            keys = sorted(partial)
            stacked = torch.stack([partial[k] for k in keys])
            dist.all_reduce(stacked, op=dist.ReduceOp.SUM)
            partial = {k: stacked[i] for i, k in enumerate(keys)}
        grads = dev_dist.finalize_gradients(partial, popsize)
    else:
        grads = dev_dist._compute_gradients(samples, weights_all, method)

    mean_eval = torch.mean(f_all)
    grads, mean_eval = _results_to_home(problem, grads, mean_eval, home_device)
    return {"gradients": grads, "num_solutions": popsize, "mean_eval": mean_eval}


def adaptive_sample_and_gradients(problem, distribution, popsize: int, *, num_interactions: int, popsize_max: Optional[int], obj_index: int,
                                  ranking_method: Optional[str]) -> dict:
    from .core import SolutionBatch

    if world()[1] > 1:
        raise NotImplementedError("adaptive population size (num_interactions) is not available with a population sharded over ranks: "
                                  "the global ranking needs a fixed, common population size")
    home_device = distribution.device
    dev_dist = distribution.to(problem.device)
    first = problem._get_local_interaction_count()
    batches, total = [], 0
    while True:
        batch = SolutionBatch(problem, popsize, device=problem.device, empty=True)
        problem.sample_and_evaluate(dev_dist, batch)
        batches.append(batch)
        total += popsize
        if problem._get_local_interaction_count() - first > num_interactions:
            break
        if popsize_max is not None and total >= popsize_max:
            break
    merged = batches[0] if len(batches) == 1 else SolutionBatch.cat(batches)
    grads = dev_dist.compute_gradients(merged.access_values(keep_evals=True), merged.access_evals(obj_index),
                                       objective_sense=problem.senses[obj_index], ranking_method=ranking_method)
    mean_eval = torch.mean(merged.access_evals(obj_index))
    if home_device != problem.device:
        grads = {k: v.to(home_device) for k, v in grads.items()}
        mean_eval = mean_eval.to(home_device)
    return {"gradients": grads, "num_solutions": len(merged), "mean_eval": mean_eval}
```

### evotorch_b200/distributions.py

```python

from __future__ import annotations

import math
from copy import copy
from typing import Any, Iterable, Optional

import torch

from . import ops
from .core import PhiloxRecipe
from .tools.cloning import Clonable
from .tools.readonlytensor import as_plain_tensor
from .tools.misc import extract_generator, make_gaussian, to_torch_dtype
from .tools.ranking import rank


def _philox_source(generator: Any):
    return generator if (generator is not None and hasattr(generator, "next_philox_stream")
                         and getattr(generator, "rng", "philox") == "philox") else None


class Distribution(Clonable):

    MANDATORY_PARAMETERS: set = set()
    OPTIONAL_PARAMETERS: set = set()
    PARAMETER_NDIMS: dict = {}

    def __init__(self, *, solution_length: int, parameters: dict, dtype=None, device=None):
        self.__solution_length = int(solution_length)
        found = 0
        for name in parameters:
            if name in self.MANDATORY_PARAMETERS:
                found += 1
            elif name not in self.OPTIONAL_PARAMETERS:
                raise ValueError(f"Unrecognized parameter: {name!r}")
        if found < len(self.MANDATORY_PARAMETERS):
            raise ValueError(
                f"Not all mandatory parameters of this Distribution were specified. Mandatory parameters of this distribution:"
                f" {self.MANDATORY_PARAMETERS}; optional parameters of this distribution: {self.OPTIONAL_PARAMETERS};"
                f" encountered parameters: {set(parameters.keys())}."
            )
        tensors = [v for v in parameters.values() if isinstance(v, torch.Tensor)]
        self.__dtype = to_torch_dtype(dtype) if dtype is not None else tensors[0].dtype
        self.__device = torch.device(device) if device is not None else tensors[0].device
        self.__parameters = {
            k: (v.to(dtype=self.__dtype, device=self.__device) if isinstance(v, torch.Tensor) else v) for k, v in parameters.items()
        }

    @property
    def solution_length(self) -> int:
        return self.__solution_length

    @property
    def device(self) -> torch.device:
        return self.__device

    @property
    def dtype(self) -> torch.dtype:
        return self.__dtype

    @property
    def parameters(self) -> dict:
        return self.__parameters

    def to(self, device) -> "Distribution":
        if torch.device(self.device) == torch.device(device):
            return self
        device = torch.device(device)
        if device.type == "cuda":
            params = {k: (v.to(device, non_blocking=v.is_pinned()) if isinstance(v, torch.Tensor) else v) for k, v in self.parameters.items()}
            return type(self)(solution_length=self.solution_length, parameters=params, device=device)
        return type(self)(solution_length=self.solution_length, parameters=self.parameters, device=device)

    def modified_copy(self, *, dtype=None, device=None, **parameters) -> "Distribution":
        new_parameters = copy(self.parameters)
        new_parameters.update(parameters)
        return type(self)(parameters=new_parameters, dtype=self.dtype if dtype is None else dtype,
                          device=self.device if device is None else device)

    def make_empty(self, *, num_solutions: int) -> torch.Tensor:
        return torch.empty(int(num_solutions), self.solution_length, dtype=self.dtype, device=self.device)

    def make_zeros(self, *, num_solutions: int) -> torch.Tensor:
        return torch.zeros(int(num_solutions), self.solution_length, dtype=self.dtype, device=self.device)

    def _fill(self, out: torch.Tensor, *, generator: Any = None):
        raise NotImplementedError

    def sample(self, num_solutions: Optional[int] = None, *, out: Optional[torch.Tensor] = None, generator: Any = None) -> torch.Tensor:
        if (num_solutions is not None) and (out is not None):
            raise ValueError("Received both `num_solutions` and `out` with values other than None. Please provide only one of them.")
        if (num_solutions is None) and (out is None):
            raise ValueError("Received both `num_solutions` and `out` as None. Please provide one of these arguments.")
        if out is None:
            out = self.make_empty(num_solutions=int(num_solutions))
        else:
            if out.ndim != 2:
                raise ValueError(f"The `sample(...)` method can fill only 2-dimensional tensors. However, the provided `out` tensor has"
                                 f" {out.ndim} dimensions, its shape being {out.shape}.")
            if out.shape[1] != self.solution_length:
                raise ValueError(f"The solution length declared by this distribution is {self.solution_length}. However, the provided"
                                 f" `out` tensor has {out.shape[1]} columns.")
        self._fill(out, generator=generator)
        return out

    def _compute_gradients(self, samples: torch.Tensor, weights: torch.Tensor, ranking_used: Optional[str]) -> dict:
        raise NotImplementedError

    def compute_gradients(self, samples: torch.Tensor, fitnesses: torch.Tensor, *, objective_sense: str,
                          ranking_method: Optional[str] = None) -> dict:
        if objective_sense == "max":
            higher_is_better = True
        elif objective_sense == "min":
            higher_is_better = False
        else:
            raise ValueError(f'`objective_sense` was expected as "min" or as "max". However, it was encountered as {objective_sense!r}.')
        if ranking_method is None:
            ranking_method = "raw"
        fitnesses = as_plain_tensor(torch.as_tensor(fitnesses, dtype=self.dtype))
        samples = as_plain_tensor(samples)
        [num_samples, _] = samples.shape
        [num_fitnesses] = fitnesses.shape
        if num_samples != num_fitnesses:
            raise ValueError(f"The number of samples and the number of fitnesses do not match: {num_samples} != {num_fitnesses}.")
        weights = rank(fitnesses, ranking_method=ranking_method, higher_is_better=higher_is_better)
        return self._compute_gradients(samples, weights, ranking_method)

    def update_parameters(self, gradients: dict, *, learning_rates: Optional[dict] = None, optimizers: Optional[dict] = None) -> "Distribution":
        raise NotImplementedError

    def _follow_gradient(self, param_name: str, x: torch.Tensor, *, learning_rates: Optional[dict] = None,
                         optimizers: Optional[dict] = None) -> torch.Tensor:
        x = torch.as_tensor(x, dtype=self.dtype, device=self.device)
        lr = (learning_rates or {}).get(param_name)
        opt = (optimizers or {}).get(param_name)
        if lr is None and opt is None:
            return x
        if opt is None:
            return lr * x
        if lr is None:
            return opt.ascent(x)
        raise ValueError("Encountered both `learning_rate` and `optimizer` as values other than None.")


def _weighted_colsum(w: torch.Tensor, m: torch.Tensor) -> torch.Tensor:
    return torch.mv(m.T, w) if m.dtype.is_floating_point else torch.sum(w.unsqueeze(-1) * m, dim=0)


class SeparableGaussian(Distribution):

    MANDATORY_PARAMETERS = {"mu", "sigma"}
    OPTIONAL_PARAMETERS = {"divide_mu_grad_by", "divide_sigma_grad_by", "parenthood_ratio"}
    PARAMETER_NDIMS = {"mu": 1, "sigma": 1}
    SYMMETRIC = False
    GRAD_FORM = ops.GRAD_SEPARABLE

    def __init__(self, parameters: dict, *, solution_length: Optional[int] = None, device=None, dtype=None):
        [mu_length] = parameters["mu"].shape
        [sigma_length] = parameters["sigma"].shape
        if solution_length is None:
            solution_length = mu_length
        elif solution_length != mu_length:
            raise ValueError(f"The argument `solution_length` does not match the length of `mu` provided in `parameters`."
                             f" solution_length={solution_length}, parameters[\"mu\"]={mu_length}.")
        if mu_length != sigma_length:
            raise ValueError(f"The tensors `mu` and `sigma` provided within `parameters` have mismatching lengths."
                             f" parameters[\"mu\"]={mu_length}, parameters[\"sigma\"]={sigma_length}.")
        super().__init__(solution_length=solution_length, parameters=parameters, device=device, dtype=dtype)

    @property
    def mu(self) -> torch.Tensor:
        return self.parameters["mu"]

    @mu.setter
    def mu(self, new_mu: Iterable):
        self.parameters["mu"] = torch.as_tensor(new_mu, dtype=self.dtype, device=self.device)

    @property
    def sigma(self) -> torch.Tensor:
        return self.parameters["sigma"]

    @sigma.setter
    def sigma(self, new_sigma: Iterable):
        self.parameters["sigma"] = torch.as_tensor(new_sigma, dtype=self.dtype, device=self.device)

    def _fill(self, out: torch.Tensor, *, generator: Any = None):
        src = _philox_source(generator)
        if src is not None and ops.uses_kernels(out) and out.stride(1) == 1:
            if self.SYMMETRIC and out.shape[0] % 2 != 0:
                raise ValueError(f"Symmetric sampling cannot be done if the leftmost dimension of the target tensor is odd: {tuple(out.shape)}")
            seed, stream_id = src.next_philox_stream()
            ops.sample_eval(ops.OBJ_NONE, out, self.mu.contiguous(), self.sigma.contiguous(), n_rows=out.shape[0],
                            symmetric=self.SYMMETRIC, seed=seed, stream_id=stream_id, row0=getattr(src, "philox_row0", 0))
        else:
            make_gaussian(out=out, center=self.mu, stdev=self.sigma, symmetric=self.SYMMETRIC, generator=extract_generator(generator))

    def _grad_scale(self, param_name: str, weights: torch.Tensor, n_total: Optional[int] = None):
        option = self.parameters.get(f"divide_{param_name}_grad_by")
        n = weights.shape[0] if n_total is None else int(n_total)
        if option is None:
            return 1.0, None
        if option == "num_solutions":
            return 1.0 / n, None
        if option == "num_directions":
            return 1.0 / (n // 2), None
        if option == "total_weight":
            return 1.0, torch.sum(torch.abs(weights))
        if option == "weight_stdev":
            return 1.0, torch.std(weights)
        raise ValueError(f"The parameter divide_{param_name}_grad_by has an unrecognized value: {option}")

    def _prepared_weights(self, weights: torch.Tensor, ranking_used: Optional[str]) -> torch.Tensor:
        if ranking_used not in self._UNTOUCHED_RANKINGS:
            if ops.uses_kernels(weights):
                return ops.weights_adjust_(weights.clone(), 1)
            return weights - torch.mean(weights)
        return weights

    _UNTOUCHED_RANKINGS = ("centered", "normalized")

    def _weighted_sums(self, form: int, samples: torch.Tensor, w: torch.Tensor, scale_mu: float, scale_sigma: float) -> tuple:
        mu, sigma = self.mu, self.sigma
        peer = getattr(self, "_peer", None)
        if peer is not None:
            if isinstance(samples, PhiloxRecipe):
                ops.grad_push(form, None, w.contiguous(), mu.contiguous(), sigma.contiguous(), scale_mu=scale_mu, scale_sigma=scale_sigma, peer=peer,
                              seed=samples.seed, stream_id=samples.stream_id, row0=samples.row0, stream_offset=samples.stream_offset)
            else:
                ops.grad_push(form, samples, w.contiguous(), mu.contiguous(), sigma.contiguous(), scale_mu=scale_mu, scale_sigma=scale_sigma, peer=peer)
            return peer.reduce_gradients()
        if isinstance(samples, PhiloxRecipe):
            return ops.grad_regen(form, w.contiguous(), mu.contiguous(), sigma.contiguous(), seed=samples.seed, stream_id=samples.stream_id,
                                  row0=samples.row0, scale_mu=scale_mu, scale_sigma=scale_sigma, stream_offset=samples.stream_offset)
        if ops.uses_kernels(samples) and ops.uses_kernels(w):
            return ops.grad(form, samples, w.contiguous(), mu.contiguous(), sigma.contiguous(), scale_mu, scale_sigma)
        if form == ops.GRAD_SYMMETRIC:
            eps = samples[0::2] - mu
            a, b = (w[0::2] - w[1::2]) / 2, (w[0::2] + w[1::2]) / 2
        else:
            eps = samples - mu
            a = b = w
        if form == ops.GRAD_EXP:
            g = ((eps / sigma) ** 2) - 1
        elif form == ops.GRAD_MOMENTS:
            g = eps**2
        else:
            g = ((eps**2) - (sigma**2)) / sigma
        return _weighted_colsum(a, eps) * scale_mu, _weighted_colsum(b, g) * scale_sigma

    def accepts_local_weights(self, ranking_used: Optional[str]) -> bool:
        if "parenthood_ratio" in self.parameters:
            return False
        for name in ("mu", "sigma"):
            if self.parameters.get(f"divide_{name}_grad_by") not in (None, "num_solutions", "num_directions"):
                return False
        return ranking_used in self._UNTOUCHED_RANKINGS and ranking_used in ("centered", "linear", "nes")

    def partial_gradients(self, samples: torch.Tensor, all_weights: torch.Tensor, row0: int, ranking_used: Optional[str],
                          local_weights_of: Optional[int] = None) -> dict:
        n_local = samples.shape[0]
        if local_weights_of is not None:
            if not self.accepts_local_weights(ranking_used):
                raise ValueError("this distribution / ranking needs the utilities of the whole population")
            smu, _ = self._grad_scale("mu", all_weights, local_weights_of)
            ssig, _ = self._grad_scale("sigma", all_weights, local_weights_of)
            gmu, gsig = self._weighted_sums(self.GRAD_FORM, samples, all_weights, smu, ssig)
            return {"mu": gmu, "sigma": gsig}
        if "parenthood_ratio" in self.parameters:
            num_elites = math.floor(all_weights.shape[0] * self.parameters["parenthood_ratio"])
            if ops.uses_kernels(all_weights):
                mask = ops.elite_mask(all_weights.contiguous(), num_elites)
            else:
                mask = torch.zeros_like(all_weights)
                mask[torch.argsort(all_weights, descending=True, stable=True)[:num_elites]] = 1
            s1, s2 = self._weighted_sums(ops.GRAD_MOMENTS, samples, mask[row0:row0 + n_local], 1.0, 1.0)
            return {"elite_sum": s1, "elite_sqsum": s2}
        w = self._prepared_weights(all_weights, ranking_used)
        smu, dmu = self._grad_scale("mu", w)
        ssig, dsig = self._grad_scale("sigma", w)
        gmu, gsig = self._weighted_sums(self.GRAD_FORM, samples, w[row0:row0 + n_local], smu, ssig)
        if dmu is not None:
            gmu = gmu / dmu
        if dsig is not None:
            gsig = gsig / dsig
        return {"mu": gmu, "sigma": gsig}

    def finalize_gradients(self, summed: dict, num_solutions: int) -> dict:
        if "elite_sum" in summed:
            num_elites = math.floor(num_solutions * self.parameters["parenthood_ratio"])
            s1, s2 = summed["elite_sum"], summed["elite_sqsum"]
            if ops.uses_kernels(s1):
                gmu, gsig = ops.cem_finalize(s1.contiguous(), s2.contiguous(), self.sigma.contiguous(), num_elites)
            else:
                gmu = s1 / num_elites
                var = (s2 - s1 * s1 / num_elites) / (num_elites - 1)
                gsig = torch.sqrt(torch.clamp_min(var, 0)) - self.sigma
            return {"mu": gmu, "sigma": gsig}
        return summed

    def _compute_gradients(self, samples: torch.Tensor, weights: torch.Tensor, ranking_used: Optional[str]) -> dict:
        return self.finalize_gradients(self.partial_gradients(samples, weights, 0, ranking_used), weights.shape[0])

    def update_parameters(self, gradients: dict, *, learning_rates: Optional[dict] = None, optimizers: Optional[dict] = None):
        new_mu = self.mu + self._follow_gradient("mu", gradients["mu"], learning_rates=learning_rates, optimizers=optimizers)
        new_sigma = self.sigma + self._follow_gradient("sigma", gradients["sigma"], learning_rates=learning_rates, optimizers=optimizers)
        return self.modified_copy(mu=new_mu, sigma=new_sigma)

    def relative_entropy(dist_0: "SeparableGaussian", dist_1: "SeparableGaussian") -> float:
        cov_0, cov_1 = dist_0.sigma.pow(2.0), dist_1.sigma.pow(2.0)
        mu_delta = dist_1.mu - dist_0.mu
        k = dist_0.solution_length
        return 0.5 * (torch.sum(cov_0 / cov_1) - k + torch.sum(mu_delta.pow(2.0) / cov_1) + torch.sum(torch.log(cov_1))
                      - torch.sum(torch.log(cov_0)))


class SymmetricSeparableGaussian(SeparableGaussian):

    SYMMETRIC = True
    GRAD_FORM = ops.GRAD_SYMMETRIC


class ExpSeparableGaussian(SeparableGaussian):

    OPTIONAL_PARAMETERS: set = set()
    GRAD_FORM = ops.GRAD_EXP

    def _prepared_weights(self, weights: torch.Tensor, ranking_used: Optional[str]) -> torch.Tensor:
        if ranking_used != "nes":
            if ops.uses_kernels(weights):
                return ops.weights_adjust_(weights.clone(), 2)
            return weights / torch.sum(torch.abs(weights))
        return weights

    _UNTOUCHED_RANKINGS = ("nes",)

    def update_parameters(self, gradients: dict, *, learning_rates: Optional[dict] = None, optimizers: Optional[dict] = None):
        new_mu = self.mu + self._follow_gradient("mu", gradients["mu"], learning_rates=learning_rates, optimizers=optimizers)
        new_sigma = self.sigma * torch.exp(
            0.5 * self._follow_gradient("sigma", gradients["sigma"], learning_rates=learning_rates, optimizers=optimizers))
        return self.modified_copy(mu=new_mu, sigma=new_sigma)


class ExpGaussian(Distribution):

    MANDATORY_PARAMETERS = {"mu", "sigma"}
    OPTIONAL_PARAMETERS = {"sigma_inv"}
    PARAMETER_NDIMS = {"mu": 1, "sigma": 2, "sigma_inv": 2}

    def __init__(self, parameters: dict, *, solution_length: Optional[int] = None, device=None, dtype=None):
        parameters = dict(parameters)
        [mu_length] = parameters["mu"].shape
        if parameters["sigma"].ndim == 1:
            parameters["sigma"] = torch.diag(parameters["sigma"])
        if "sigma_inv" not in parameters:
            parameters["sigma_inv"] = torch.inverse(parameters["sigma"])
        [sigma_length, _] = parameters["sigma"].shape
        if solution_length is None:
            solution_length = mu_length
        elif solution_length != mu_length:
            raise ValueError(f"The argument `solution_length` does not match the length of `mu` provided in `parameters`.")
        if mu_length != sigma_length:
            raise ValueError("The tensors `mu` and `sigma` provided within `parameters` have mismatching lengths.")
        super().__init__(solution_length=solution_length, parameters=parameters, device=device, dtype=dtype)
        self.eye = torch.eye(solution_length, dtype=self.dtype, device=self.device)

    @property
    def mu(self) -> torch.Tensor:
        return self.parameters["mu"]

    @property
    def sigma(self) -> torch.Tensor:
        return self.parameters["sigma"]

    @property
    def sigma_inv(self) -> torch.Tensor:
        return self.parameters["sigma_inv"]

    A = sigma
    A_inv = sigma_inv

    @property
    def cov(self) -> torch.Tensor:
        return self.sigma.transpose(0, 1) @ self.sigma

    def to_global_coordinates(self, local_coordinates: torch.Tensor) -> torch.Tensor:
        if ops.uses_kernels(local_coordinates) and ops.uses_kernels(self.A) and local_coordinates.ndim == 2:
            z = local_coordinates.contiguous()
            out = torch.empty_like(z)
            ops.gemm_nt(z, self.A.contiguous(), torch.empty_like(z), out2=out, bias=self.mu.contiguous())
            return out
        return self.mu.unsqueeze(0) + (self.A @ local_coordinates.T).T

    def to_local_coordinates(self, global_coordinates: torch.Tensor) -> torch.Tensor:
        centered = global_coordinates - self.mu.unsqueeze(0)
        if ops.uses_kernels(centered) and ops.uses_kernels(self.A_inv) and centered.ndim == 2:
            return ops.gemm_nt(centered.contiguous(), self.A_inv.contiguous())
        return (self.A_inv @ centered.T).T

    def _fill(self, out: torch.Tensor, *, generator: Any = None):
        make_gaussian(out=out, generator=extract_generator(generator))
        out[:] = self.to_global_coordinates(out)

    def _compute_gradients(self, samples: torch.Tensor, weights: torch.Tensor, ranking_used: Optional[str]) -> dict:
        z = self.to_local_coordinates(samples)
        if ranking_used not in ("centered", "normalized"):
            weights = weights - torch.mean(weights)
        d_grad = torch.mv(z.T, weights)
        if ops.uses_kernels(z) and ops.uses_kernels(weights):
            zc = z.contiguous()
            outer = ops.gemm_nt(ops.transpose_scale(zc, weights.contiguous()), ops.transpose_scale(zc))
        else:
            outer = (z.T * weights) @ z
        m_grad = outer - torch.sum(weights) * self.eye
        return {"d": d_grad, "M": m_grad}

    def update_parameters(self, gradients: dict, *, learning_rates: Optional[dict] = None, optimizers: Optional[dict] = None):
        learning_rates = dict(learning_rates or {})
        learning_rates.setdefault("d", learning_rates.get("mu"))
        learning_rates.setdefault("M", learning_rates.get("sigma"))
        optimizers = dict(optimizers or {})
        if "mu" in optimizers:
            optimizers.setdefault("d", optimizers["mu"])
            learning_rates["d"] = None
        update_d = self._follow_gradient("d", gradients["d"], learning_rates=learning_rates, optimizers=optimizers)
        update_m = self._follow_gradient("M", gradients["M"], learning_rates=learning_rates, optimizers=optimizers)
        new_mu = self.mu + torch.mv(self.A, update_d)
        new_a = self.A @ torch.matrix_exp(0.5 * update_m)
        new_a_inv = torch.matrix_exp(-0.5 * update_m) @ self.A_inv
        return self.modified_copy(mu=new_mu, sigma=new_a, sigma_inv=new_a_inv)
```

### evotorch_b200/ops.py

```python

from __future__ import annotations

import math
from typing import Optional

import torch

from . import _native as nat
from .tools.readonlytensor import as_plain_tensor

OBJ_NONE, OBJ_SPHERE, OBJ_RASTRIGIN, OBJ_ACKLEY = 0, 1, 2, 3
OBJECTIVE_IDS = {"sphere": OBJ_SPHERE, "rastrigin": OBJ_RASTRIGIN, "ackley": OBJ_ACKLEY}
RANK_IDS = {"centered": 0, "linear": 1, "nes": 2, "normalized": 3, "raw": 4}
GRAD_SEPARABLE, GRAD_SYMMETRIC, GRAD_EXP, GRAD_MOMENTS = 0, 1, 2, 3
NAN = float("nan")


_timers: Optional[dict] = None


def enable_timers() -> None:
    global _timers
    _timers = {}


def disable_timers() -> None:
    global _timers
    _timers = None


class _timed:
    __slots__ = ("name", "start")

    def __init__(self, name: str):
        self.name = name

    def __enter__(self):
        if _timers is not None:
            self.start = torch.cuda.Event(enable_timing=True)
            self.start.record()
        return self

    def __exit__(self, *exc):
        if _timers is not None:
            end = torch.cuda.Event(enable_timing=True)
            end.record()
            _timers.setdefault(self.name, []).append((self.start, end))
        return False


def timer_results() -> dict:
    out = {}
    for name, pairs in (_timers or {}).items():
        ms = [a.elapsed_time(b) for a, b in pairs]
        out[name] = (len(ms), sum(ms) / max(len(ms), 1))
    return out


_replayed_launches = 0


def count_replayed_launches(n: int) -> None:
    global _replayed_launches
    _replayed_launches += int(n)


def launch_count() -> int:
    return int(nat.lib().evok_launch_count()) + _replayed_launches


def uses_kernels(t: torch.Tensor) -> bool:
    return t.is_cuda and t.dtype == torch.float32


def _vec(t: torch.Tensor, name: str, n: Optional[int] = None) -> torch.Tensor:
    if not (t.is_cuda and t.dtype == torch.float32 and t.ndim == 1 and t.is_contiguous()):
        raise ValueError(f"{name}: expected a contiguous 1-D float32 CUDA tensor, got {tuple(t.shape)} {t.dtype} {t.device}")
    if n is not None and t.numel() != n:
        raise ValueError(f"{name}: expected length {n}, got {t.numel()}")
    return as_plain_tensor(t)


def _mat(t: torch.Tensor, name: str) -> torch.Tensor:
    if not (t.is_cuda and t.dtype == torch.float32 and t.ndim == 2 and t.stride(1) == 1 and t.stride(0) >= t.shape[1]):
        raise ValueError(f"{name}: expected a row-major 2-D float32 CUDA tensor, got {tuple(t.shape)} strides {t.stride()} {t.dtype}")
    return as_plain_tensor(t)


def _offset_ptr(stream_offset: Optional[torch.Tensor]) -> Optional[int]:
    if stream_offset is None:
        return None
    if not (stream_offset.is_cuda and stream_offset.dtype == torch.int32 and stream_offset.numel() >= 1):
        raise ValueError("stream_offset: expected an int32 CUDA tensor with one element")
    return stream_offset.data_ptr()


def sample_eval(objective: int, X: Optional[torch.Tensor], mu: torch.Tensor, sigma: torch.Tensor, *, n_rows: int, symmetric: bool,
                seed: int, stream_id: int, row0: int = 0, f: Optional[torch.Tensor] = None,
                stream_offset: Optional[torch.Tensor] = None) -> None:
    D = mu.numel()
    _vec(mu, "mu"); _vec(sigma, "sigma", D)
    ldx = 0
    if X is not None:
        _mat(X, "X")
        if X.shape != (n_rows, D):
            raise ValueError(f"X: expected shape {(n_rows, D)}, got {tuple(X.shape)}")
        ldx = X.stride(0)
    if f is not None:
        _vec(f, "f", n_rows)
    if objective != OBJ_NONE and f is None:
        raise ValueError("f: a fitness buffer is required when an objective is fused into the sampler")
    if symmetric and (n_rows % 2 or row0 % 2):
        raise ValueError("symmetric sampling needs an even number of rows and an even first row")
    if n_rows == 0:
        return
    with _timed("sample_eval" if objective != OBJ_NONE else "sample"):
        rc = nat.lib().evok_sample_eval(objective, nat.ptr(X), ldx, mu.data_ptr(), sigma.data_ptr(), row0, n_rows, D, int(symmetric),
                                        seed & 0xFFFFFFFFFFFFFFFF, stream_id & 0xFFFFFFFFFFFFFFFF, _offset_ptr(stream_offset), nat.ptr(f),
                                        nat.stream_of(mu))
    nat.check(rc, "evok_sample_eval")


def sample_eval_push(objective: int, X: Optional[torch.Tensor], mu: torch.Tensor, sigma: torch.Tensor, *, n_rows: int, symmetric: bool,
                     seed: int, stream_id: int, row0: int, peer, stream_offset: Optional[torch.Tensor] = None) -> None:
    D = mu.numel()
    _vec(mu, "mu"); _vec(sigma, "sigma", D)
    ldx = 0
    if X is not None:
        _mat(X, "X")
        if X.shape != (n_rows, D):
            raise ValueError(f"X: expected shape {(n_rows, D)}, got {tuple(X.shape)}")
        ldx = X.stride(0)
    if row0 + n_rows > peer.popsize:
        raise ValueError("rows beyond the population the peer exchange was sized for")
    with _timed("sample_eval"):
        rc = nat.lib().evok_sample_eval_push(objective, nat.ptr(X), ldx, mu.data_ptr(), sigma.data_ptr(), row0, n_rows, D, int(symmetric),
                                             seed & 0xFFFFFFFFFFFFFFFF, stream_id & 0xFFFFFFFFFFFFFFFF, _offset_ptr(stream_offset), peer.world,
                                             peer.rank, peer.peer_f, peer.peer_flags_f, peer.epoch_f, peer._counter(0), nat.stream_of(mu))
    nat.check(rc, "evok_sample_eval_push")


def grad_push(form: int, X: Optional[torch.Tensor], w: torch.Tensor, mu: torch.Tensor, sigma: torch.Tensor, *, scale_mu: float,
              scale_sigma: float, peer, seed: int = 0, stream_id: int = 0, row0: int = 0, stream_offset: Optional[torch.Tensor] = None) -> None:
    n, D = w.numel(), mu.numel()
    _vec(w, "weights"); _vec(mu, "mu"); _vec(sigma, "sigma", D)
    ldx = 0
    if X is not None:
        _mat(X, "X")
        if X.shape != (n, D):
            raise ValueError(f"X: expected shape {(n, D)}, got {tuple(X.shape)}")
        ldx = X.stride(0)
    ws = nat.workspace(mu.device, nat.lib().evok_grad_workspace_bytes(n, D), "grad")
    with _timed("grad" if X is not None else "grad_regen"):
        rc = nat.lib().evok_grad_push(form, nat.ptr(X), ldx, w.data_ptr(), mu.data_ptr(), sigma.data_ptr(), row0, n, D, seed & 0xFFFFFFFFFFFFFFFF,
                                      stream_id & 0xFFFFFFFFFFFFFFFF, _offset_ptr(stream_offset), scale_mu, scale_sigma, peer.world, peer.rank,
                                      peer.peer_slots, peer.peer_flags_g, peer.epoch_g, peer._counter(1), ws.data_ptr(), ws.numel(),
                                      nat.stream_of(mu))
    nat.check(rc, "evok_grad_push")


def evaluate(objective: int, X: torch.Tensor, f: Optional[torch.Tensor] = None) -> torch.Tensor:
    _mat(X, "X")
    n, D = X.shape
    if f is None:
        f = torch.empty(n, dtype=torch.float32, device=X.device)
    _vec(f, "f", n)
    with _timed("eval"):
        rc = nat.lib().evok_eval(objective, X.data_ptr(), X.stride(0), n, D, f.data_ptr(), nat.stream_of(X))
    nat.check(rc, "evok_eval")
    return f


def _rank_ws(device: torch.device, n: int) -> torch.Tensor:
    return nat.workspace(device, nat.lib().evok_rank_workspace_bytes(n), "rank")


def rank(f: torch.Tensor, method: str, higher_is_better: bool, out: Optional[torch.Tensor] = None,
         perm: Optional[torch.Tensor] = None) -> torch.Tensor:
    f = _vec(f, "fitnesses")
    n = f.numel()
    w = torch.empty_like(f) if out is None else _vec(out, "out", n)
    if perm is not None and not (perm.is_cuda and perm.dtype == torch.int64 and perm.is_contiguous() and perm.numel() == n):
        raise ValueError("perm: expected a contiguous int64 CUDA tensor of the same length")
    ws = _rank_ws(f.device, n)
    method_id = RANK_IDS[method]
    with _timed("rank"):
        rc = nat.lib().evok_rank(method_id, f.data_ptr(), n, int(bool(higher_is_better)), w.data_ptr(), nat.ptr(perm), ws.data_ptr(),
                                 ws.numel(), nat.stream_of(f))
    nat.check(rc, "evok_rank")
    return w


def argsort(keys: torch.Tensor, descending: bool) -> torch.Tensor:
    keys = _vec(keys, "keys")
    n = keys.numel()
    perm = torch.empty(n, dtype=torch.int64, device=keys.device)
    ws = _rank_ws(keys.device, n)
    nat.check(nat.lib().evok_argsort(keys.data_ptr(), n, int(bool(descending)), perm.data_ptr(), ws.data_ptr(), ws.numel(),
                                     nat.stream_of(keys)), "evok_argsort")
    return perm


def rank_table(keys: torch.Tensor, descending: bool, table: torch.Tensor, out: Optional[torch.Tensor] = None) -> torch.Tensor:
    keys = _vec(keys, "keys")
    n = keys.numel()
    _vec(table, "table", n)
    out = torch.empty_like(keys) if out is None else _vec(out, "out", n)
    ws = _rank_ws(keys.device, n)
    with _timed("rank"):
        rc = nat.lib().evok_rank_table(keys.data_ptr(), n, int(bool(descending)), table.data_ptr(), out.data_ptr(), ws.data_ptr(), ws.numel(),
                                       nat.stream_of(keys))
    nat.check(rc, "evok_rank_table")
    return out


def cmaes_row_weights(assigned: torch.Tensor, Z: torch.Tensor, active: bool, w_pos: torch.Tensor, w_act: torch.Tensor) -> None:
    _mat(Z, "Z")
    n, d = Z.shape
    _vec(assigned, "assigned", n); _vec(w_pos, "w_pos", n); _vec(w_act, "w_act", n)
    nat.check(nat.lib().evok_cmaes_row_weights(assigned.data_ptr(), Z.data_ptr(), Z.stride(0), n, d, int(bool(active)), w_pos.data_ptr(),
                                               w_act.data_ptr(), nat.stream_of(Z)), "evok_cmaes_row_weights")


def cmaes_vector_update(local_disp: torch.Tensor, shaped_disp: torch.Tensor, m: torch.Tensor, p_sigma: torch.Tensor, p_c: torch.Tensor,
                        sigma: torch.Tensor, consts, csa_squared: bool, k_out: torch.Tensor, *, steps: int = 0,
                        steps_dev: Optional[torch.Tensor] = None, h_sig_out: Optional[torch.Tensor] = None) -> None:
    import ctypes

    d = m.numel()
    _vec(local_disp, "local_disp", d); _vec(shaped_disp, "shaped_disp", d); _vec(m, "m"); _vec(p_sigma, "p_sigma", d); _vec(p_c, "p_c", d)
    _vec(k_out, "k_out", 3)
    if not (sigma.is_cuda and sigma.dtype == torch.float32 and sigma.numel() == 1):
        raise ValueError("sigma: expected a 1-element float32 CUDA tensor")
    if steps_dev is not None and not (steps_dev.is_cuda and steps_dev.dtype == torch.int64 and steps_dev.numel() == 1):
        raise ValueError("steps_dev: expected a 1-element int64 CUDA tensor")
    carr = (ctypes.c_float * 10)(*[float(x) for x in consts])
    nat.check(nat.lib().evok_cmaes_vector_update(local_disp.data_ptr(), shaped_disp.data_ptr(), d, m.data_ptr(), p_sigma.data_ptr(), p_c.data_ptr(),
                                                 sigma.data_ptr(), nat.ptr(steps_dev), int(steps), carr, int(bool(csa_squared)), k_out.data_ptr(),
                                                 nat.ptr(h_sig_out), nat.stream_of(m)), "evok_cmaes_vector_update")


def weights_adjust_(w: torch.Tensor, mode: int) -> torch.Tensor:
    _vec(w, "weights")
    nat.check(nat.lib().evok_weights_adjust(w.data_ptr(), w.numel(), mode, nat.stream_of(w)), "evok_weights_adjust")
    return w


def elite_mask(w: torch.Tensor, num_elites: int) -> torch.Tensor:
    w = _vec(w, "weights")
    n = w.numel()
    mask = torch.empty_like(w)
    ws = _rank_ws(w.device, n)
    nat.check(nat.lib().evok_elite_mask(w.data_ptr(), n, num_elites, mask.data_ptr(), ws.data_ptr(), ws.numel(), nat.stream_of(w)),
              "evok_elite_mask")
    return mask


def grad(form: int, X: torch.Tensor, w: torch.Tensor, mu: torch.Tensor, sigma: torch.Tensor, scale_mu: float, scale_sigma: float,
         out_mu: Optional[torch.Tensor] = None, out_sigma: Optional[torch.Tensor] = None) -> tuple:
    _mat(X, "samples")
    n, D = X.shape
    _vec(w, "weights", n); _vec(mu, "mu", D); _vec(sigma, "sigma", D)
    out_mu = torch.empty_like(mu) if out_mu is None else _vec(out_mu, "out_mu", D)
    out_sigma = torch.empty_like(mu) if out_sigma is None else _vec(out_sigma, "out_sigma", D)
    ws = nat.workspace(X.device, nat.lib().evok_grad_workspace_bytes(n, D), "grad")
    with _timed("grad"):
        rc = nat.lib().evok_grad(form, X.data_ptr(), X.stride(0), w.data_ptr(), mu.data_ptr(), sigma.data_ptr(), n, D, scale_mu,
                                 scale_sigma, out_mu.data_ptr(), out_sigma.data_ptr(), ws.data_ptr(), ws.numel(), nat.stream_of(X))
    nat.check(rc, "evok_grad")
    return out_mu, out_sigma


def grad_regen(form: int, w: torch.Tensor, mu: torch.Tensor, sigma: torch.Tensor, *, seed: int, stream_id: int, row0: int,
               scale_mu: float, scale_sigma: float, out_mu: Optional[torch.Tensor] = None,
               out_sigma: Optional[torch.Tensor] = None, stream_offset: Optional[torch.Tensor] = None) -> tuple:
    n, D = w.numel(), mu.numel()
    _vec(w, "weights"); _vec(mu, "mu"); _vec(sigma, "sigma", D)
    out_mu = torch.empty_like(mu) if out_mu is None else _vec(out_mu, "out_mu", D)
    out_sigma = torch.empty_like(mu) if out_sigma is None else _vec(out_sigma, "out_sigma", D)
    ws = nat.workspace(mu.device, nat.lib().evok_grad_workspace_bytes(n, D), "grad")
    with _timed("grad_regen"):
        rc = nat.lib().evok_grad_regen(form, w.data_ptr(), mu.data_ptr(), sigma.data_ptr(), row0, n, D, seed & 0xFFFFFFFFFFFFFFFF,
                                       stream_id & 0xFFFFFFFFFFFFFFFF, _offset_ptr(stream_offset), scale_mu, scale_sigma, out_mu.data_ptr(),
                                       out_sigma.data_ptr(), ws.data_ptr(), ws.numel(), nat.stream_of(mu))
    nat.check(rc, "evok_grad_regen")
    return out_mu, out_sigma


def clipup_step(g: torch.Tensor, velocity: torch.Tensor, stepsize: float, momentum: float, max_speed: float,
                step_out: Optional[torch.Tensor] = None, mu: Optional[torch.Tensor] = None) -> None:
    D = g.numel()
    _vec(g, "g"); _vec(velocity, "velocity", D)
    with _timed("mu_step"):
        rc = nat.lib().evok_clipup_step(g.data_ptr(), D, velocity.data_ptr(), stepsize, momentum, max_speed, nat.ptr(step_out),
                                        nat.ptr(mu), nat.stream_of(g))
    nat.check(rc, "evok_clipup_step")


def adam_step(g: torch.Tensor, m: torch.Tensor, v: torch.Tensor, t: int, lr: float, beta1: float, beta2: float, eps: float,
              step_out: Optional[torch.Tensor] = None, mu: Optional[torch.Tensor] = None) -> None:
    D = g.numel()
    _vec(g, "g"); _vec(m, "m", D); _vec(v, "v", D)
    rc = nat.lib().evok_adam_step(g.data_ptr(), D, m.data_ptr(), v.data_ptr(), t, lr, beta1, beta2, eps, nat.ptr(step_out), nat.ptr(mu),
                                  nat.stream_of(g))
    nat.check(rc, "evok_adam_step")


def sgd_step(g: torch.Tensor, buf: Optional[torch.Tensor], first_step: bool, lr: float, momentum: float,
             step_out: Optional[torch.Tensor] = None, mu: Optional[torch.Tensor] = None) -> None:
    D = g.numel()
    _vec(g, "g")
    rc = nat.lib().evok_sgd_step(g.data_ptr(), D, nat.ptr(buf), int(first_step), lr, momentum, nat.ptr(step_out), nat.ptr(mu),
                                 nat.stream_of(g))
    nat.check(rc, "evok_sgd_step")


def axpy_(mu: torch.Tensor, g: torch.Tensor, lr: float) -> None:
    D = g.numel()
    _vec(g, "g"); _vec(mu, "mu", D)
    nat.check(nat.lib().evok_axpy(g.data_ptr(), D, lr, mu.data_ptr(), nat.stream_of(g)), "evok_axpy")


def _bound(x, D: int, device) -> tuple:
    if x is None:
        return None, NAN
    if isinstance(x, torch.Tensor) and x.ndim >= 1 and x.numel() > 1:
        v = x.to(device=device, dtype=torch.float32).contiguous()
        if v.numel() != D:
            raise IndexError(f"bound vector has length {v.numel()}, expected {D}")
        return v, NAN
    return None, float(x)


def sigma_update_(sigma: torch.Tensor, g: torch.Tensor, lr: float, exp_form: bool, lb=None, ub=None, max_change=None) -> None:
    D = sigma.numel()
    _vec(sigma, "sigma"); _vec(g, "g", D)
    lbv, lbs = _bound(lb, D, sigma.device)
    ubv, ubs = _bound(ub, D, sigma.device)
    mcv, mcs = _bound(max_change, D, sigma.device)
    with _timed("sigma_step"):
        rc = nat.lib().evok_sigma_update(sigma.data_ptr(), g.data_ptr(), D, lr, int(exp_form), nat.ptr(lbv), lbs, nat.ptr(ubv), ubs,
                                         nat.ptr(mcv), mcs, nat.stream_of(sigma))
    nat.check(rc, "evok_sigma_update")


def cem_finalize(s1: torch.Tensor, s2: torch.Tensor, sigma: torch.Tensor, num_elites: int) -> tuple:
    D = sigma.numel()
    gm, gs = torch.empty_like(sigma), torch.empty_like(sigma)
    nat.check(nat.lib().evok_cem_finalize(s1.data_ptr(), s2.data_ptr(), sigma.data_ptr(), D, num_elites, gm.data_ptr(), gs.data_ptr(),
                                          nat.stream_of(sigma)), "evok_cem_finalize")
    return gm, gs


def _items(t: torch.Tensor, core_shape: tuple, name: str) -> tuple:
    if not (t.is_cuda and t.dtype == torch.float32):
        raise ValueError(f"{name}: expected a float32 CUDA tensor")
    t = as_plain_tensor(t)
    if tuple(t.shape) == tuple(core_shape):
        return t.contiguous(), None, 0
    if tuple(t.shape[1:]) != tuple(core_shape) or t.ndim != len(core_shape) + 1:
        raise ValueError(f"{name}: expected shape {core_shape} or (items, {', '.join(map(str, core_shape))}), got {tuple(t.shape)}")
    t = t.contiguous()
    return t, t.shape[0], int(t.stride(0))


def sample_batched(out: torch.Tensor, mu: torch.Tensor, sigma: torch.Tensor, *, symmetric: bool, seed: int, stream_id0: int = 0) -> torch.Tensor:
    if not (out.is_cuda and out.dtype == torch.float32 and out.ndim == 3 and out.is_contiguous()):
        raise ValueError("out: expected a contiguous float32 CUDA tensor of shape (items, popsize, D)")
    B, n, d = out.shape
    mu, bm, sm = _items(mu, (d,), "mu")
    sigma, bs, ss = _items(sigma, (d,), "sigma")
    for cnt in (bm, bs):
        if cnt is not None and cnt != B:
            raise ValueError("mu / sigma: number of items differs from out")
    if symmetric and n % 2:
        raise ValueError(f"Symmetric sampling cannot be done if the number of solutions is odd: {n}")
    with _timed("sample"):
        rc = nat.lib().evok_sample_batched(out.data_ptr(), n * d, d, mu.data_ptr(), sm, sigma.data_ptr(), ss, B, n, d, int(symmetric),
                                           seed & 0xFFFFFFFFFFFFFFFF, stream_id0 & 0xFFFFFFFFFFFFFFFF, nat.stream_of(out))
    nat.check(rc, "evok_sample_batched")
    return out


def rank_batched(f: torch.Tensor, method: str, higher_is_better: bool) -> torch.Tensor:
    if not (f.is_cuda and f.dtype == torch.float32 and f.ndim == 2):
        raise ValueError("f: expected a float32 CUDA tensor of shape (items, N)")
    f = as_plain_tensor(f).contiguous()
    B, n = f.shape
    w = torch.empty_like(f)
    lib = nat.lib()
    ws = nat.workspace(f.device, max(lib.evok_rank_workspace_bytes(n), 8 * B + 256), "rank")
    with _timed("rank"):
        rc = lib.evok_rank_batched(RANK_IDS[method], f.data_ptr(), n, B, int(bool(higher_is_better)), w.data_ptr(), ws.data_ptr(), ws.numel(),
                                   nat.stream_of(f))
    nat.check(rc, "evok_rank_batched")
    return w


def elite_mask_batched(w: torch.Tensor, num_elites: int) -> torch.Tensor:
    w = as_plain_tensor(w).contiguous()
    B, n = w.shape
    mask = torch.empty_like(w)
    ws = _rank_ws(w.device, n)
    nat.check(nat.lib().evok_elite_mask_batched(w.data_ptr(), n, B, num_elites, mask.data_ptr(), ws.data_ptr(), ws.numel(), nat.stream_of(w)),
              "evok_elite_mask_batched")
    return mask


def weights_adjust_batched_(w: torch.Tensor, mode: int) -> torch.Tensor:
    B, n = w.shape
    nat.check(nat.lib().evok_weights_adjust_batched(w.data_ptr(), n, B, mode, nat.stream_of(w)), "evok_weights_adjust_batched")
    return w


def grad_batched(form: int, X: torch.Tensor, w: torch.Tensor, mu: torch.Tensor, sigma: torch.Tensor, scale_mu: float, scale_sigma: float) -> tuple:
    if not (X.is_cuda and X.dtype == torch.float32 and X.ndim == 3):
        raise ValueError("X: expected a float32 CUDA tensor of shape (items, N, D)")
    X = as_plain_tensor(X).contiguous()
    B, n, d = X.shape
    w = as_plain_tensor(w).contiguous()
    if tuple(w.shape) != (B, n):
        raise ValueError(f"w: expected shape {(B, n)}, got {tuple(w.shape)}")
    mu, bm, sm = _items(mu, (d,), "mu")
    sigma, bs, ss = _items(sigma, (d,), "sigma")
    out_mu = torch.empty(B, d, dtype=torch.float32, device=X.device)
    out_sigma = torch.empty_like(out_mu)
    lib = nat.lib()
    ws = nat.workspace(X.device, lib.evok_grad_batched_workspace_bytes(B, n, d), "grad_batched")
    with _timed("grad"):
        rc = lib.evok_grad_batched(form, X.data_ptr(), n * d, d, w.data_ptr(), mu.data_ptr(), sm, sigma.data_ptr(), ss, B, n, d, scale_mu, scale_sigma,
                                   out_mu.data_ptr(), out_sigma.data_ptr(), ws.data_ptr(), ws.numel(), nat.stream_of(X))
    nat.check(rc, "evok_grad_batched")
    return out_mu, out_sigma


def _host_floats(values, n: int):
    import ctypes

    vals = [float(v) for v in values]
    if len(vals) != n:
        raise ValueError(f"expected {n} per-item scalars, got {len(vals)}")
    return (ctypes.c_float * n)(*vals)


def clipup_batched_(g: torch.Tensor, velocity: torch.Tensor, center: torch.Tensor, stepsizes, momenta, max_speeds) -> None:
    B, d = center.shape
    for t, name in ((g, "g"), (velocity, "velocity"), (center, "center")):
        if not (t.is_cuda and t.dtype == torch.float32 and t.is_contiguous() and tuple(t.shape) == (B, d)):
            raise ValueError(f"{name}: expected a contiguous float32 CUDA tensor of shape {(B, d)}")
    nat.check(nat.lib().evok_clipup_batched(g.data_ptr(), B, d, velocity.data_ptr(), center.data_ptr(), _host_floats(stepsizes, B),
                                            _host_floats(momenta, B), _host_floats(max_speeds, B), nat.stream_of(g)), "evok_clipup_batched")


def sigma_update_batched_(sigma: torch.Tensor, g: torch.Tensor, lrs, exp_form: bool, lb: Optional[torch.Tensor] = None,
                          ub: Optional[torch.Tensor] = None, max_change: Optional[torch.Tensor] = None) -> None:
    B, d = sigma.shape
    for t, name in ((sigma, "sigma"), (g, "g"), (lb, "lb"), (ub, "ub"), (max_change, "max_change")):
        if t is not None and not (t.is_cuda and t.dtype == torch.float32 and t.is_contiguous() and tuple(t.shape) == (B, d)):
            raise ValueError(f"{name}: expected a contiguous float32 CUDA tensor of shape {(B, d)}")
    nat.check(nat.lib().evok_sigma_update_batched(sigma.data_ptr(), g.data_ptr(), B, d, _host_floats(lrs, B), int(bool(exp_form)), nat.ptr(lb),
                                                  nat.ptr(ub), nat.ptr(max_change), nat.stream_of(sigma)), "evok_sigma_update_batched")


ACT_IDS = {"none": 0, "identity": 0, "tanh": 1, "relu": 2, "sigmoid": 3}


def mlp_forward(params: torch.Tensor, obs: torch.Tensor, dims, acts, out: Optional[torch.Tensor] = None, *,
                obs_sum: Optional[torch.Tensor] = None, obs_sumsq: Optional[torch.Tensor] = None, obs_count: Optional[torch.Tensor] = None,
                min_variance: float = 1e-2, clip: Optional[tuple] = None, active: Optional[torch.Tensor] = None) -> torch.Tensor:
    import ctypes

    _mat(params, "parameters"); _mat(obs, "observations")
    n = params.shape[0]
    dims = [int(d) for d in dims]
    act_ids = [ACT_IDS[a] if isinstance(a, str) else int(a) for a in acts]
    if obs.shape != (n, dims[0]):
        raise ValueError(f"observations: expected shape {(n, dims[0])}, got {tuple(obs.shape)}")
    if out is None:
        out = torch.empty(n, dims[-1], dtype=torch.float32, device=params.device)
    _mat(out, "out")
    d_arr = (ctypes.c_int32 * len(dims))(*dims)
    a_arr = (ctypes.c_int32 * len(act_ids))(*act_ids)
    need = nat.lib().evok_mlp_parameter_length(len(act_ids), d_arr)
    if params.shape[1] != need:
        raise ValueError(f"parameters: expected {need} columns for layer widths {dims}, got {params.shape[1]}")
    if obs_sum is None and active is None:
        with _timed("mlp_forward"):
            rc = nat.lib().evok_mlp_forward(params.data_ptr(), params.stride(0), obs.data_ptr(), obs.stride(0), out.data_ptr(), out.stride(0), n,
                                            len(act_ids), d_arr, a_arr, nat.stream_of(params))
        nat.check(rc, "evok_mlp_forward")
        return out
    if obs_sum is not None:
        _vec(obs_sum, "obs_sum", dims[0]); _vec(obs_sumsq, "obs_sumsq", dims[0])
        if obs_count is None or obs_count.dtype != torch.int64 or obs_count.numel() != 1 or not obs_count.is_cuda:
            raise ValueError("obs_count: expected a 1-element int64 CUDA tensor")
    if active is not None:
        if active.dtype == torch.bool:
            active = active.view(torch.uint8)
        if active.dtype != torch.uint8 or active.numel() != n or not active.is_cuda or not active.is_contiguous():
            raise ValueError(f"active: expected {n} contiguous bool / uint8 flags on the GPU")
    ws = None if active is None else nat.workspace(params.device, 256, "mlp")
    lo, hi = (NAN, NAN) if clip is None else (NAN if clip[0] is None else float(clip[0]), NAN if clip[1] is None else float(clip[1]))
    with _timed("mlp_forward"):
        rc = nat.lib().evok_mlp_forward_prep(params.data_ptr(), params.stride(0), obs.data_ptr(), obs.stride(0), out.data_ptr(), out.stride(0), n,
                                             len(act_ids), d_arr, a_arr, nat.ptr(obs_sum), nat.ptr(obs_sumsq), nat.ptr(obs_count),
                                             float(min_variance), lo, hi, nat.ptr(active), nat.ptr(ws), 0 if ws is None else ws.numel(),
                                             nat.stream_of(params))
    nat.check(rc, "evok_mlp_forward_prep")
    return out


def mlp_forward_shared(params: torch.Tensor, x: torch.Tensor, dims, acts) -> torch.Tensor:
    import ctypes

    _mat(params, "parameters"); _mat(x, "x")
    dims = [int(d) for d in dims]
    act_ids = [ACT_IDS[a] if isinstance(a, str) else int(a) for a in acts]
    n, B = params.shape[0], x.shape[0]
    if x.shape[1] != dims[0]:
        raise ValueError(f"x: expected {dims[0]} columns, got {x.shape[1]}")
    if len(act_ids) < 2 or max(dims[1:]) > 512:
        raise ValueError("mlp_forward_shared handles nets with >= 2 layers and widths <= 512")
    d_arr = (ctypes.c_int32 * len(dims))(*dims)
    a_arr = (ctypes.c_int32 * len(act_ids))(*act_ids)
    lib = nat.lib()
    if params.shape[1] != lib.evok_mlp_parameter_length(len(act_ids), d_arr):
        raise ValueError("parameters: wrong number of columns for these layer widths")
    if x.data_ptr() % 16 != 0 or x.stride(0) % 4 != 0:
        padded = torch.zeros(B, (dims[0] + 3) // 4 * 4, dtype=torch.float32, device=x.device)
        padded[:, :dims[0]] = x
        x = padded[:, :dims[0]]
    out = torch.empty(n, B, dims[-1], dtype=torch.float32, device=params.device)
    ws = nat.workspace(params.device, lib.evok_mlp_forward_shared_workspace_bytes(n, B, len(act_ids), d_arr) + 512, "mlp_shared")
    with _timed("mlp_forward_shared"):
        rc = lib.evok_mlp_forward_shared(params.data_ptr(), params.stride(0), n, x.data_ptr(), x.stride(0), B, len(act_ids), d_arr, a_arr,
                                         out.data_ptr(), ws.data_ptr(), ws.numel(), nat.stream_of(params))
    nat.check(rc, "evok_mlp_forward_shared")
    return out


def gemm_nt(A: torch.Tensor, B: torch.Tensor, out: Optional[torch.Tensor] = None, *, out2: Optional[torch.Tensor] = None,
            alpha: Optional[torch.Tensor] = None, bias: Optional[torch.Tensor] = None) -> torch.Tensor:
    _mat(A, "A"); _mat(B, "B")
    M, K = A.shape
    N, K2 = B.shape
    if K != K2:
        raise ValueError(f"inner dimensions differ: {K} vs {K2}")
    if out is None:
        out = torch.empty(M, N, dtype=torch.float32, device=A.device)
    _mat(out, "out")
    if out2 is not None:
        _mat(out2, "out2")
    if bias is not None:
        _vec(bias, "bias", N)
    nbytes = nat.lib().evok_gemm_workspace_bytes(M, N, K)
    ws = nat.workspace(A.device, nbytes, "gemm")
    with _timed("gemm"):
        rc = nat.lib().evok_gemm_nt(A.data_ptr(), A.stride(0), B.data_ptr(), B.stride(0), M, N, K, out.data_ptr(), out.stride(0), nat.ptr(out2),
                                    0 if out2 is None else out2.stride(0), nat.ptr(alpha), nat.ptr(bias), ws.data_ptr(), ws.numel(),
                                    nat.stream_of(A))
    nat.check(rc, "evok_gemm_nt")
    return out


def weighted_syrk_update(Y: torch.Tensor, w: torch.Tensor, k: torch.Tensor, C: torch.Tensor, u: Optional[torch.Tensor] = None,
                         out: Optional[torch.Tensor] = None) -> torch.Tensor:
    _mat(Y, "Y"); _mat(C, "C")
    n, d = Y.shape
    _vec(w, "w", n); _vec(k, "k", 3)
    if C.shape != (d, d):
        raise ValueError(f"C: expected shape {(d, d)}, got {tuple(C.shape)}")
    if u is not None:
        _vec(u, "u", d)
    out = torch.empty_like(C) if out is None else _mat(out, "out")
    ldo = (n + 3) // 4 * 4
    lib = nat.lib()
    tws = nat.workspace(Y.device, 2 * d * ldo * 4 + 256, "syrk_operands")
    base = (tws.data_ptr() + 255) // 256 * 256
    a_w, a_p = base, base + d * ldo * 4
    nat.check(lib.evok_transpose_pair(Y.data_ptr(), Y.stride(0), n, d, w.data_ptr(), a_w, a_p, ldo, nat.stream_of(Y)), "evok_transpose_pair")
    ws = nat.workspace(Y.device, lib.evok_gemm_workspace_bytes(d, d, n), "gemm")
    with _timed("gemm"):
        rc = lib.evok_gemm_nt_affine(a_w, ldo, a_p, ldo, d, d, n, out.data_ptr(), out.stride(0), k.data_ptr(), C.data_ptr(), C.stride(0), nat.ptr(u),
                                     ws.data_ptr(), ws.numel(), nat.stream_of(Y))
    nat.check(rc, "evok_gemm_nt_affine")
    return out


def cholesky(A: torch.Tensor, out: Optional[torch.Tensor] = None) -> torch.Tensor:
    _mat(A, "A")
    n = A.shape[0]
    if A.shape[1] != n:
        raise ValueError(f"A: expected a square matrix, got {tuple(A.shape)}")
    out = torch.empty_like(A) if out is None else _mat(out, "out")
    if out.data_ptr() == A.data_ptr():
        raise ValueError("out must not alias A")
    lib = nat.lib()
    ws = nat.workspace(A.device, lib.evok_cholesky_workspace_bytes(n), "cholesky")
    with _timed("cholesky"):
        rc = lib.evok_cholesky(A.data_ptr(), A.stride(0), n, out.data_ptr(), out.stride(0), ws.data_ptr(), ws.numel(), nat.stream_of(A))
    nat.check(rc, "evok_cholesky")
    return out


def transpose_scale(X: torch.Tensor, w: Optional[torch.Tensor] = None) -> torch.Tensor:
    _mat(X, "X")
    rows, cols = X.shape
    if w is not None:
        _vec(w, "w", rows)
    out = torch.empty(cols, rows, dtype=torch.float32, device=X.device)
    nat.check(nat.lib().evok_transpose_scale(X.data_ptr(), X.stride(0), rows, cols, nat.ptr(w), out.data_ptr(), out.stride(0),
                                             nat.stream_of(X)), "evok_transpose_scale")
    return out
```

### include/evok.h

```cpp
#ifndef EVOK_H_
#define EVOK_H_

#include <stddef.h>
#include <stdint.h>

#ifdef __cplusplus
extern "C" {
#endif

#define EVOK_ABI_VERSION 1

#if defined(__GNUC__)
#define EVOK_API __attribute__((visibility("default")))
#else
#define EVOK_API
#endif

#define EVOK_E_NULLPTR (-1)
#define EVOK_E_BADSIZE (-2)
#define EVOK_E_BADENUM (-3)
#define EVOK_E_WORKSPACE (-4)
#define EVOK_E_ODDROWS (-5)
#define EVOK_E_ALIGN (-6)

#define EVOK_MAX_PEERS 16

#define EVOK_OBJ_NONE 0
#define EVOK_OBJ_SPHERE 1
#define EVOK_OBJ_RASTRIGIN 2
#define EVOK_OBJ_ACKLEY 3
#define EVOK_OBJ_COUNT 4

#define EVOK_RANK_CENTERED 0
#define EVOK_RANK_LINEAR 1
#define EVOK_RANK_NES 2
#define EVOK_RANK_NORMALIZED 3
#define EVOK_RANK_RAW 4

#define EVOK_GRAD_SEPARABLE 0
#define EVOK_GRAD_SYMMETRIC 1
#define EVOK_GRAD_EXP 2
#define EVOK_GRAD_MOMENTS 3

int evok_abi_version(void);
uint64_t evok_launch_count(void);
const char* evok_error_string(int code);

int evok_sample_eval(int objective, float* X, int64_t ldx, const float* mu, const float* sigma, int64_t row0,
                     int64_t n_rows, int64_t D, int symmetric, uint64_t seed, uint64_t stream_id,
                     const uint32_t* stream_offset_dev, float* f, void* stream);

int evok_eval(int objective, const float* X, int64_t ldx, int64_t n_rows, int64_t D, float* f, void* stream);

size_t evok_rank_workspace_bytes(int64_t N);
int evok_rank(int method, const float* f, int64_t N, int higher_is_better, float* w, int64_t* perm, void* ws,
              size_t ws_bytes, void* stream);

int evok_argsort(const float* keys, int64_t N, int descending, int64_t* perm, void* ws, size_t ws_bytes,
                 void* stream);

int evok_rank_table(const float* keys, int64_t N, int descending, const float* table, float* out, void* ws, size_t ws_bytes, void* stream);

int evok_weights_adjust(float* w, int64_t N, int mode, void* stream);

int evok_elite_mask(const float* w, int64_t N, int64_t num_elites, float* mask, void* ws, size_t ws_bytes,
                    void* stream);

size_t evok_grad_workspace_bytes(int64_t n_rows, int64_t D);
int evok_grad(int form, const float* X, int64_t ldx, const float* w, const float* mu, const float* sigma,
              int64_t n_rows, int64_t D, float scale_mu, float scale_sigma, float* out_mu, float* out_sigma,
              void* ws, size_t ws_bytes, void* stream);

int evok_grad_regen(int form, const float* w, const float* mu, const float* sigma, int64_t row0, int64_t n_rows,
                    int64_t D, uint64_t seed, uint64_t stream_id, const uint32_t* stream_offset_dev, float scale_mu,
                    float scale_sigma, float* out_mu, float* out_sigma, void* ws, size_t ws_bytes, void* stream);

int evok_clipup_step(const float* g, int64_t D, float* velocity, float stepsize, float momentum, float max_speed,
                     float* step_out, float* mu, void* stream);
int evok_adam_step(const float* g, int64_t D, float* m, float* v, int64_t t, float lr, float beta1, float beta2,
                   float eps, float* step_out, float* mu, void* stream);
int evok_sgd_step(const float* g, int64_t D, float* buf, int first_step, float lr, float momentum, float* step_out,
                  float* mu, void* stream);
int evok_axpy(const float* g, int64_t D, float lr, float* mu, void* stream);

int evok_sigma_update(float* sigma, const float* g, int64_t D, float lr, int exp_form, const float* lb_vec,
                      float lb, const float* ub_vec, float ub, const float* mc_vec, float mc, void* stream);

int evok_cem_finalize(const float* s1, const float* s2, const float* sigma, int64_t D, int64_t num_elites,
                      float* grad_mu, float* grad_sigma, void* stream);

#define EVOK_ACT_NONE 0
#define EVOK_ACT_TANH 1
#define EVOK_ACT_RELU 2
#define EVOK_ACT_SIGMOID 3
int64_t evok_mlp_parameter_length(int n_layers, const int32_t* dims_host);
int evok_mlp_forward(const float* params, int64_t ldp, const float* obs, int64_t ldo, float* out, int64_t ldout, int64_t N,
                     int n_layers, const int32_t* dims_host, const int32_t* acts_host, void* stream);

int evok_mlp_forward_prep(const float* params, int64_t ldp, const float* obs, int64_t ldo, float* out, int64_t ldout, int64_t N,
                          int n_layers, const int32_t* dims_host, const int32_t* acts_host, const float* obs_sum, const float* obs_sumsq,
                          const int64_t* obs_count_dev, float min_variance, float clip_lo, float clip_hi, const uint8_t* active,
                          void* ws, size_t ws_bytes, void* stream);

size_t evok_mlp_forward_shared_workspace_bytes(int64_t N, int64_t B, int n_layers, const int32_t* dims_host);
int evok_mlp_forward_shared(const float* params, int64_t ldp, int64_t N, const float* X, int64_t ldx, int64_t B, int n_layers,
                            const int32_t* dims_host, const int32_t* acts_host, float* out, void* ws, size_t ws_bytes, void* stream);
int evok_gemm_gather_rows(const float* params, int64_t batch_stride, int64_t w_offset, int64_t rows_per_batch, int64_t n_batches, const float* X,
                          int64_t ldx, int64_t n_cols, int64_t K, int64_t bias_offset, int act, float* C, int64_t ldc, void* stream);
size_t evok_gemm_gather_rows_workspace_bytes(int64_t n_cols, int64_t K);
int evok_gemm_gather_rows_ws(const float* params, int64_t batch_stride, int64_t w_offset, int64_t rows_per_batch, int64_t n_batches, const float* X,
                             int64_t ldx, int64_t n_cols, int64_t K, int64_t bias_offset, int act, float* C, int64_t ldc, int unit_fastest, void* ws,
                             size_t ws_bytes, void* stream);

size_t evok_gemm_workspace_bytes(int64_t M, int64_t N, int64_t K);
int evok_gemm_nt(const float* A, int64_t lda, const float* B, int64_t ldb, int64_t M, int64_t N, int64_t K, float* C, int64_t ldc,
                 float* C2, int64_t ldc2, const float* alpha_dev, const float* bias, void* ws, size_t ws_bytes, void* stream);
int evok_gemm_nt_affine(const float* A, int64_t lda, const float* B, int64_t ldb, int64_t M, int64_t N, int64_t K, float* C, int64_t ldc,
                        const float* k_dev, const float* E, int64_t lde, const float* u, void* ws, size_t ws_bytes, void* stream);
int evok_transpose_scale(const float* in, int64_t ldi, int64_t rows, int64_t cols, const float* w, float* out, int64_t ldo, void* stream);
int evok_transpose_pair(const float* in, int64_t ldi, int64_t rows, int64_t cols, const float* w, float* out_w, float* out_p, int64_t ldo,
                        void* stream);

int evok_sample_batched(float* X, int64_t item_stride_x, int64_t ldx, const float* mu, int64_t item_stride_mu, const float* sigma,
                        int64_t item_stride_sigma, int64_t n_items, int64_t n_rows, int64_t D, int symmetric, uint64_t seed, uint64_t stream_id0,
                        void* stream);
int evok_rank_batched(int method, const float* f, int64_t N, int64_t n_items, int higher_is_better, float* w, void* ws, size_t ws_bytes,
                      void* stream);
int evok_elite_mask_batched(const float* w, int64_t N, int64_t n_items, int64_t num_elites, float* mask, void* ws, size_t ws_bytes, void* stream);
int evok_weights_adjust_batched(float* w, int64_t N, int64_t n_items, int mode, void* stream);
size_t evok_grad_batched_workspace_bytes(int64_t n_items, int64_t n_rows, int64_t D);
int evok_grad_batched(int form, const float* X, int64_t item_stride_x, int64_t ldx, const float* w, const float* mu, int64_t item_stride_mu,
                      const float* sigma, int64_t item_stride_sigma, int64_t n_items, int64_t n_rows, int64_t D, float scale_mu, float scale_sigma,
                      float* out_mu, float* out_sigma, void* ws, size_t ws_bytes, void* stream);
int evok_clipup_batched(const float* g, int64_t n_items, int64_t D, float* velocity, float* center, const float* stepsize_host,
                        const float* momentum_host, const float* max_speed_host, void* stream);
int evok_sigma_update_batched(float* sigma, const float* g, int64_t n_items, int64_t D, const float* lr_host, int exp_form, const float* lb_vec,
                              const float* ub_vec, const float* mc_vec, void* stream);

int evok_cmaes_row_weights(const float* assigned_weights, const float* Z, int64_t ldz, int64_t N, int64_t D, int active, float* w_positive,
                           float* w_active, void* stream);
int evok_cmaes_vector_update(const float* local_disp, const float* shaped_disp, int64_t D, float* m, float* p_sigma, float* p_c, float* sigma_dev,
                             int64_t* steps_dev, int64_t steps_host, const float* consts_host, int csa_squared, float* k_out, float* h_sig_out,
                             void* stream);

size_t evok_cholesky_workspace_bytes(int64_t n);
int evok_cholesky(const float* A, int64_t lda, int64_t n, float* L, int64_t ldl, void* ws, size_t ws_bytes, void* stream);

int evok_rank_sharded(int method, const float* f_local, int64_t N, int higher_is_better, int world, int rank,
                      const int64_t* row_offsets_host, void* const* peer_keys_host, void* const* peer_fsum_host,
                      void* const* peer_flags_host, uint64_t* epoch_dev, uint32_t* done_dev, uint32_t* err_dev, uint64_t timeout_ns,
                      float* w_local, float* mean_out, void* ws, size_t ws_bytes, void* stream);

int evok_peer_alloc(size_t bytes, void** dev_ptr_out_host, void* handle_out_64B_host);
int evok_peer_open(const void* handle_64B_host, void** dev_ptr_out_host);
int evok_peer_close(void* dev_ptr);
int evok_peer_free(void* dev_ptr);
int evok_sample_eval_push(int objective, float* X, int64_t ldx, const float* mu, const float* sigma, int64_t row0, int64_t n_rows,
                          int64_t D, int symmetric, uint64_t seed, uint64_t stream_id, const uint32_t* stream_offset_dev, int world,
                          int rank, void* const* peer_f_host, void* const* peer_flags_host, const uint64_t* epoch_dev, uint32_t* done_dev,
                          void* stream);
int evok_peer_push(const void* src_local, int64_t n_bytes, int64_t dst_offset_bytes, int world, int rank, void* const* peer_base_host,
                   void* const* peer_flags_host, const uint64_t* epoch_dev, void* stream);
int evok_peer_wait(const uint64_t* flags_local, int world, uint64_t* epoch_dev, uint32_t* err_dev, uint64_t timeout_ns, void* stream);
int evok_grad_push(int form, const float* X, int64_t ldx, const float* w, const float* mu, const float* sigma, int64_t row0,
                   int64_t n_rows, int64_t D, uint64_t seed, uint64_t stream_id, const uint32_t* stream_offset_dev, float scale_mu,
                   float scale_sigma, int world, int rank, void* const* peer_slots_host, void* const* peer_flags_host,
                   const uint64_t* epoch_dev, uint32_t* done_dev, void* ws, size_t ws_bytes, void* stream);
int evok_peer_reduce(const float* slots_local, int world, int64_t n, const uint64_t* flags_local, uint64_t* epoch_dev,
                     uint32_t* done_dev, uint32_t* err_dev, uint64_t timeout_ns, float* out, void* stream);

#ifdef __cplusplus
}
#endif
#endif
```

Baseline: 47.59.

## Regenerate a fraction of sample rows in gradient kernel instead of loading them

Attaches Philox provenance recipes to materialized populations so the gradient kernel knows how each row was sampled. The TMA gradient kernel then recomputes 5 of every 16 row groups from the Philox stream, mu and sigma instead of loading them from HBM. This splits the work between memory bandwidth and ALU to cut global reads of the 1M x 10k sample matrix. It adds Python bookkeeping for provenance (slicing, copy, drop on write) and relies on regenerated values matching the stored samples bit for bit.

```diff
diff --git a/evotorch_b200/_native.py b/evotorch_b200/_native.py
--- a/evotorch_b200/_native.py
+++ b/evotorch_b200/_native.py
@@ -39,6 +39,8 @@
     "evok_elite_mask": (c_int, [_P, c_int64, c_int64, _P, _P, c_size_t, _P]),
     "evok_grad_workspace_bytes": (c_size_t, [c_int64, c_int64]),
     "evok_grad": (c_int, [c_int, _P, c_int64, _P, _P, _P, c_int64, c_int64, c_float, c_float, _P, _P, _P, c_size_t, _P]),
+    "evok_grad_recipe": (c_int, [c_int, _P, c_int64, _P, _P, _P, c_int64, c_int64, c_int64, c_uint64, c_uint64, _P, _P, _P, c_float, c_float, _P,
+                                 _P, _P, c_size_t, _P]),
     "evok_grad_regen": (c_int, [c_int, _P, _P, _P, c_int64, c_int64, c_int64, c_uint64, c_uint64, _P, c_float, c_float, _P, _P, _P,
                                 c_size_t, _P]),
     "evok_clipup_step": (c_int, [_P, c_int64, _P, c_float, c_float, c_float, _P, _P, _P]),
@@ -71,6 +73,8 @@
     "evok_peer_wait": (c_int, [_P, c_int, _P, _P, c_uint64, _P]),
     "evok_grad_push": (c_int, [c_int, _P, c_int64, _P, _P, _P, c_int64, c_int64, c_int64, c_uint64, c_uint64, _P, c_float, c_float, c_int, c_int,
                                _P, _P, _P, _P, _P, c_size_t, _P]),
+    "evok_grad_push_recipe": (c_int, [c_int, _P, c_int64, _P, _P, _P, c_int64, c_int64, c_int64, c_uint64, c_uint64, _P, _P, _P, c_float, c_float,
+                                      c_int, c_int, _P, _P, _P, _P, _P, c_size_t, _P]),
     "evok_rank_sharded": (c_int, [c_int, _P, c_int64, c_int, c_int, c_int, _P, _P, _P, _P, _P, _P, _P, c_uint64, _P, _P, _P, c_size_t, _P]),
     "evok_peer_reduce": (c_int, [_P, c_int, c_int64, _P, _P, _P, _P, c_uint64, _P, _P]),
 }
diff --git a/evotorch_b200/algorithms/gaussian.py b/evotorch_b200/algorithms/gaussian.py
--- a/evotorch_b200/algorithms/gaussian.py
+++ b/evotorch_b200/algorithms/gaussian.py
@@ -9,7 +9,7 @@
 import torch
 
 from .. import ops
-from ..core import LazySolutionBatch, PhiloxRecipe, Problem, SolutionBatch
+from ..core import LazySolutionBatch, PhiloxRecipe, Problem, SampledRows, SolutionBatch
 from ..distributed import world
 from ..distributions import Distribution, ExpGaussian, ExpSeparableGaussian, SeparableGaussian, SymmetricSeparableGaussian
 from ..optimizers import get_optimizer_class
@@ -155,19 +155,16 @@
         lazy = isinstance(pop, LazySolutionBatch)
         n = len(pop)
         fitnesses = pop._evdata.view(-1)
-        if lazy:
-            samples = PhiloxRecipe(seed=prob._philox_seed, stream_id=base_stream - 1, row0=0, n_rows=n, solution_length=prob.solution_length,
-                                   symmetric=dist.SYMMETRIC, stream_offset=counter, mu=dist.mu, sigma=dist.sigma)
-        else:
-            samples = pop._data
+        recipe = PhiloxRecipe(seed=prob._philox_seed, stream_id=base_stream - 1, row0=0, n_rows=n, solution_length=prob.solution_length,
+                              symmetric=dist.SYMMETRIC, stream_offset=counter, mu=dist.mu, sigma=dist.sigma)
+        samples = recipe if lazy else SampledRows(pop._data, recipe)
         gradients = dist.compute_gradients(samples, fitnesses, objective_sense=prob.senses[self._obj_index], ranking_method=self._ranking_method)
         self._update_in_place(gradients)
-        ops.sample_eval(prob.evok_objective_id, None if lazy else samples, dist.mu, dist.sigma, n_rows=n, symmetric=dist.SYMMETRIC,
+        ops.sample_eval(prob.evok_objective_id, None if lazy else pop._data, dist.mu, dist.sigma, n_rows=n, symmetric=dist.SYMMETRIC,
                         seed=prob._philox_seed, stream_id=base_stream, f=fitnesses, stream_offset=counter)
         counter.add_(1)
         if lazy:
-            pop.recipe = PhiloxRecipe(seed=prob._philox_seed, stream_id=base_stream - 1, row0=0, n_rows=n, solution_length=prob.solution_length,
-                                      symmetric=dist.SYMMETRIC, stream_offset=counter, mu=dist.mu, sigma=dist.sigma)
+            pop.recipe = recipe
 
     def _capture_graph(self):
         prob = self.problem
@@ -194,9 +191,18 @@
             self._step_eager()
             self._capture_graph()
             return
+        if not isinstance(pop, LazySolutionBatch) and pop._recipe() is None:
+            self._graph = None
+            self._step_eager()
+            return
         self._graph.replay()
         ops.count_replayed_launches(self._graph_kernels)
         prob._philox_stream += 1
+        if not isinstance(pop, LazySolutionBatch):
+            dist = self._distribution
+            pop._attach_recipe(PhiloxRecipe(seed=prob._philox_seed, stream_id=self._graph_base_stream - 1, row0=0, n_rows=len(pop),
+                                            solution_length=prob.solution_length, symmetric=dist.SYMMETRIC, stream_offset=self._graph_counter,
+                                            mu=dist.mu, sigma=dist.sigma))
         prob._finish_evaluation(pop)
 
     def _step_non_distributed(self):
@@ -212,7 +218,7 @@
 
     def _step_eager(self):
         lazy = isinstance(self._population, LazySolutionBatch)
-        samples = self._population.recipe if lazy else self._population.access_values(keep_evals=True)
+        samples = self._population._values_for_gradient(with_recipe=lazy or isinstance(self._distribution, SeparableGaussian))
         fitnesses = self._population.access_evals()[:, self._obj_index]
         gradients = self._distribution.compute_gradients(samples, fitnesses, objective_sense=self.problem.senses[self._obj_index],
                                                          ranking_method=self._ranking_method)
diff --git a/evotorch_b200/core.py b/evotorch_b200/core.py
--- a/evotorch_b200/core.py
+++ b/evotorch_b200/core.py
@@ -506,16 +506,19 @@
         evdata = batch._evdata
         direct = evdata.shape[1] == 1 and evdata.dtype == torch.float32 and evdata.is_contiguous()
         f = evdata.view(-1) if direct else torch.empty(n, dtype=torch.float32, device=values.device)
+        mu, sigma = distribution.mu.contiguous(), distribution.sigma.contiguous()
+        recipe = PhiloxRecipe(seed=seed, stream_id=stream_id, row0=self.philox_row0, n_rows=n, solution_length=self._solution_length,
+                              symmetric=distribution.SYMMETRIC, stream_offset=self.philox_stream_offset, mu=mu, sigma=sigma)
         peer = getattr(self, "_active_peer", None)
         if peer is not None:
-            ops.sample_eval_push(obj, values, distribution.mu.contiguous(), distribution.sigma.contiguous(), n_rows=n,
-                                 symmetric=distribution.SYMMETRIC, seed=seed, stream_id=stream_id, row0=self.philox_row0, peer=peer,
-                                 stream_offset=self.philox_stream_offset)
+            ops.sample_eval_push(obj, values, mu, sigma, n_rows=n, symmetric=distribution.SYMMETRIC, seed=seed, stream_id=stream_id,
+                                 row0=self.philox_row0, peer=peer, stream_offset=self.philox_stream_offset)
+            batch._attach_recipe(recipe)
             self._finish_evaluation(batch)
             return
-        ops.sample_eval(obj, values, distribution.mu.contiguous(), distribution.sigma.contiguous(), n_rows=n,
-                        symmetric=distribution.SYMMETRIC, seed=seed, stream_id=stream_id, row0=self.philox_row0, f=f,
-                        stream_offset=self.philox_stream_offset)
+        ops.sample_eval(obj, values, mu, sigma, n_rows=n, symmetric=distribution.SYMMETRIC, seed=seed, stream_id=stream_id,
+                        row0=self.philox_row0, f=f, stream_offset=self.philox_stream_offset)
+        batch._attach_recipe(recipe)
         if not direct:
             batch.set_evals(f)
         self._finish_evaluation(batch)
@@ -570,6 +573,10 @@
             self._evdata = source._evdata[sl]
             self._senses = source._senses
             self._num_objs = source._num_objs
+            self._prov = getattr(source, "_prov", None)
+            start, _, step = sl.indices(source._data.shape[0])
+            base = getattr(source, "_prov_row", None)
+            self._prov_row = base + start if base is not None and step == 1 else None
             return
         if merging_of is not None:
             batches = list(merging_of)
@@ -577,6 +584,7 @@
             self._evdata = torch.cat([b._evdata for b in batches], dim=0)
             self._senses = batches[0]._senses
             self._num_objs = batches[0]._num_objs
+            self._prov, self._prov_row = _Provenance(), 0
             return
         if like is not None and problem is None:
             popsize = len(like) if popsize is None else int(popsize)
@@ -584,7 +592,9 @@
             self._data = torch.empty(popsize, like._data.shape[1], dtype=like._data.dtype, device=device)
             self._evdata = torch.full((popsize, like._evdata.shape[1]), float("nan"), dtype=like._evdata.dtype, device=device)
             self._senses, self._num_objs = like._senses, like._num_objs
+            self._prov, self._prov_row = _Provenance(), 0
             return
+        self._prov, self._prov_row = _Provenance(), 0
         if problem is None or popsize is None:
             if like is not None and problem is not None and popsize is None:
                 popsize = len(like)
@@ -661,9 +671,35 @@
         return as_read_only_tensor(self._evdata)
 
     def access_values(self, *, keep_evals: bool = False) -> torch.Tensor:
+        self._drop_recipe()
         if not keep_evals:
             self.forget_evals()
         return self._data
+
+    def _drop_recipe(self):
+        prov = getattr(self, "_prov", None)
+        if prov is not None:
+            prov.recipe = None
+
+    def _attach_recipe(self, recipe: "PhiloxRecipe"):
+        if getattr(self, "_prov_row", None) == 0 and recipe.n_rows == len(self):
+            self._prov.recipe = recipe
+
+    def _recipe(self) -> Optional["PhiloxRecipe"]:
+        prov, row = getattr(self, "_prov", None), getattr(self, "_prov_row", None)
+        r = None if prov is None else prov.recipe
+        if r is None or row is None:
+            return None
+        n = len(self)
+        if row == 0 and n == r.n_rows:
+            return r
+        if row + n > r.n_rows or (r.symmetric and (row % 2 or n % 2)):
+            return None
+        return r.rows(row, n)
+
+    def _values_for_gradient(self, *, with_recipe: bool = True):
+        r = self._recipe() if with_recipe else None
+        return self._data if r is None else SampledRows(self._data, r)
 
     def access_evals(self, obj_index: Optional[int] = None) -> torch.Tensor:
         return self._evdata if obj_index is None else self._evdata[:, self._normalize_obj_index(obj_index)]
@@ -687,6 +723,7 @@
     def set_values(self, values: Any, *, solutions=None):
         if solutions is None:
             solutions = slice(None, None, None)
+        self._drop_recipe()
         self._data[solutions] = torch.as_tensor(values, dtype=self._data.dtype, device=self._data.device)
         self._evdata[solutions] = float("nan")
 
@@ -789,6 +826,8 @@
         out = SolutionBatch(like=self)
         out._data[:] = self._data
         out._evdata[:] = self._evdata
+        out._prov.recipe = self._prov.recipe if getattr(self, "_prov", None) is not None else None
+        out._prov_row = getattr(self, "_prov_row", None)
         return out
 
     def __copy__(self) -> "SolutionBatch":
@@ -813,11 +852,35 @@
     def shape(self) -> tuple:
         return (self.n_rows, self.solution_length)
 
+    def rows(self, start: int, n: int) -> "PhiloxRecipe":
+        return PhiloxRecipe(seed=self.seed, stream_id=self.stream_id, row0=self.row0 + start, n_rows=n, solution_length=self.solution_length,
+                            symmetric=self.symmetric, stream_offset=self.stream_offset, mu=self.mu, sigma=self.sigma)
+
     def materialize(self) -> torch.Tensor:
         out = torch.empty(self.n_rows, self.solution_length, dtype=torch.float32, device=self.mu.device)
         ops.sample_eval(ops.OBJ_NONE, out, self.mu, self.sigma, n_rows=self.n_rows, symmetric=self.symmetric, seed=self.seed,
                         stream_id=self.stream_id, row0=self.row0, stream_offset=self.stream_offset)
         return out
+
+
+class _Provenance:
+
+    __slots__ = ("recipe",)
+
+    def __init__(self, recipe: Optional[PhiloxRecipe] = None):
+        self.recipe = recipe
+
+
+class SampledRows:
+
+    __slots__ = ("values", "recipe")
+
+    def __init__(self, values: torch.Tensor, recipe: PhiloxRecipe):
+        self.values, self.recipe = values, recipe
+
+    @property
+    def shape(self) -> torch.Size:
+        return self.values.shape
 
 
 class LazySolutionBatch(SolutionBatch):
@@ -866,6 +929,9 @@
 
     def set_values(self, values: Any, *, solutions=None):
         raise ValueError("The decision values of a lazy population are read-only (they are a function of the Philox counters).")
+
+    def _values_for_gradient(self, *, with_recipe: bool = True):
+        return self.recipe
 
     def __getitem__(self, i):
         if isinstance(i, (slice, list, torch.Tensor)):
diff --git a/evotorch_b200/csrc/evok_grad.cu b/evotorch_b200/csrc/evok_grad.cu
--- a/evotorch_b200/csrc/evok_grad.cu
+++ b/evotorch_b200/csrc/evok_grad.cu
@@ -273,11 +273,39 @@
                : "memory");
 }
 
+#ifndef EVOK_GRAD_REGEN_NUM
+#define EVOK_GRAD_REGEN_NUM 5
+#endif
+#ifndef EVOK_GRAD_REGEN_DEN
+#define EVOK_GRAD_REGEN_DEN 16
+#endif
+struct GradRecipe {
+  PhiloxKey key;
+  const uint32_t* stream_off;
+  const float* mu_s;
+  const float* sigma_s;
+  uint64_t unit0;
+  int num, den;
+};
+
+struct RegenWalk {
+  int num, den, acc = 0;
+  __device__ __forceinline__ RegenWalk(int n, int d) : num(n), den(d) {}
+  __device__ __forceinline__ bool next() {
+    acc += num;
+    if (acc >= den) {
+      acc -= den;
+      return true;
+    }
+    return false;
+  }
+};
+
 template <bool SYM>
 __global__ void __launch_bounds__(kTmaThreads, EVOK_GRAD_TMA_CTAS_PER_SM)
     grad_partial_tma_kernel(int form, const float* __restrict__ X, int64_t ldx, const float* __restrict__ w, const float* __restrict__ mu,
                             const float* __restrict__ sigma, int64_t n_units, int64_t D, int64_t units_per_chunk,
-                            float* __restrict__ partial) {
+                            float* __restrict__ partial, const __grid_constant__ GradRecipe rc) {
   extern __shared__ __align__(128) unsigned char smem_raw[];
   float* tiles = reinterpret_cast<float*>(smem_raw);
   uint64_t* full = reinterpret_cast<uint64_t*>(smem_raw + (size_t)kTmaStages * kTmaRows * kTmaCols * sizeof(float));
@@ -304,9 +332,13 @@
   if (warp == kTmaConsumers / 32) {
     if (lane == 0) {
       const uint32_t row_bytes = (uint32_t)(width * sizeof(float));
+      RegenWalk walk(rc.num, rc.den);
+      int64_t rd = 0;
       for (int64_t g = 0; g < n_groups; ++g) {
-        const int s = (int)(g % kTmaStages);
-        const uint32_t use = (uint32_t)(g / kTmaStages);
+        if (walk.next()) continue;
+        const int s = (int)(rd % kTmaStages);
+        const uint32_t use = (uint32_t)(rd / kTmaStages);
+        ++rd;
         if (use > 0) mbar_wait(&empty[s], (use - 1) & 1);
         const int64_t r0 = r_begin + g * kTmaRows;
         const int rows = (int)min((int64_t)kTmaRows, r_end - r0);
@@ -337,10 +369,19 @@
     }
   }
   float s1[4] = {0.f, 0.f, 0.f, 0.f}, s2[4] = {0.f, 0.f, 0.f, 0.f};
-
+  auto accumulate = [&](float ai, float bi, const float (&x)[4]) {
+#pragma unroll
+    for (int c = 0; c < 4; ++c) {
+      const float e = x[c] - m[c];
+      s1[c] = fmaf(ai, e, s1[c]);
+      s2[c] = fmaf(bi, fmaf(e * e, c1[c], -c0[c]), s2[c]);
+    }
+  };
+  const uint32_t sw = rc.num ? rc.key.stream_lo + (rc.stream_off ? __ldg(rc.stream_off) : 0u) : 0u;
+
+  RegenWalk walk(rc.num, rc.den);
+  int64_t rd = 0;
   for (int64_t g = 0; g < n_groups; ++g) {
-    const int s = (int)(g % kTmaStages);
-    const uint32_t use = (uint32_t)(g / kTmaStages);
     const int64_t r0 = r_begin + g * kTmaRows;
     const int rows = (int)min((int64_t)kTmaRows, r_end - r0);
     float a[kTmaRows], b[kTmaRows];
@@ -357,6 +398,25 @@
         }
       }
     }
+    if (walk.next()) {
+      if (active) {
+        const float4 ms = __ldg(reinterpret_cast<const float4*>(rc.mu_s + col));
+        const float4 ss = __ldg(reinterpret_cast<const float4*>(rc.sigma_s + col));
+#pragma unroll
+        for (int i = 0; i < kTmaRows; ++i) {
+          if (i < rows) {
+            float z[4];
+            normals4(rc.key, sw, rc.unit0 + (uint64_t)(r0 + i), (uint32_t)(col >> 2), z);
+            const float x[4] = {fmaf(ss.x, z[0], ms.x), fmaf(ss.y, z[1], ms.y), fmaf(ss.z, z[2], ms.z), fmaf(ss.w, z[3], ms.w)};
+            accumulate(a[i], b[i], x);
+          }
+        }
+      }
+      continue;
+    }
+    const int s = (int)(rd % kTmaStages);
+    const uint32_t use = (uint32_t)(rd / kTmaStages);
+    ++rd;
     mbar_wait(&full[s], use & 1);
     const float4* tile = reinterpret_cast<const float4*>(tiles + (size_t)s * kTmaRows * kTmaCols) + tid;
     if (active) {
@@ -365,12 +425,7 @@
         if (i < rows) {
           const float4 v = tile[(size_t)i * (kTmaCols / 4)];
           const float x[4] = {v.x, v.y, v.z, v.w};
-#pragma unroll
-          for (int c = 0; c < 4; ++c) {
-            const float e = x[c] - m[c];
-            s1[c] = fmaf(a[i], e, s1[c]);
-            s2[c] = fmaf(b[i], fmaf(e * e, c1[c], -c0[c]), s2[c]);
-          }
+          accumulate(a[i], b[i], x);
         }
       }
     }
@@ -431,9 +486,26 @@
 #undef EVOK_LAUNCH_TX
 }
 
+static void regen_split(int* num, int* den) {
+  *num = EVOK_GRAD_REGEN_NUM;
+  *den = EVOK_GRAD_REGEN_DEN;
+  const char* env = getenv("EVOK_GRAD_REGEN");
+  if (env && *env) {
+    char* end = nullptr;
+    const long n = strtol(env, &end, 10);
+    const long d = (end && *end == '/') ? strtol(end + 1, nullptr, 10) : 1;
+    *num = (int)n;
+    *den = (int)d;
+  }
+  if (*den < 1 || *den > 4096) *den = 1, *num = 0;
+  if (*num < 0) *num = 0;
+  if (*num > *den) *num = *den;
+}
+
 static int grad_impl(int form, const float* X, int64_t ldx, const float* w, const float* mu, const float* sigma, int64_t row0, int64_t n_rows,
                      int64_t D, bool regen, uint64_t seed, uint64_t stream_id, const uint32_t* stream_off, float scale_mu, float scale_sigma, float* out_mu,
-                     float* out_sigma, void* ws, size_t ws_bytes, void* stream, const GradPush* push = nullptr) {
+                     float* out_sigma, void* ws, size_t ws_bytes, void* stream, const GradPush* push = nullptr, const float* mu_s = nullptr,
+                     const float* sigma_s = nullptr) {
   if (!w || !mu || !sigma || !ws || (!regen && !X) || (!push && (!out_mu || !out_sigma))) return EVOK_E_NULLPTR;
   if (form < EVOK_GRAD_SEPARABLE || form > EVOK_GRAD_MOMENTS) return EVOK_E_BADENUM;
   if (n_rows < 0 || D <= 0 || row0 < 0 || (!regen && ldx < D)) return EVOK_E_BADSIZE;
@@ -462,12 +534,23 @@
     const int64_t upc = (n_units + chunks - 1) / chunks;
     const int n_chunks = (int)((n_units + upc - 1) / upc);
     dim3 grid(n_coltiles, n_chunks);
+    GradRecipe rc{};
+    rc.num = 0;
+    rc.den = 1;
+    if (mu_s && sigma_s && aligned16(mu_s) && aligned16(sigma_s)) {
+      regen_split(&rc.num, &rc.den);
+      rc.key = make_philox_key(seed, stream_id);
+      rc.stream_off = stream_off;
+      rc.mu_s = mu_s;
+      rc.sigma_s = sigma_s;
+      rc.unit0 = unit0;
+    }
     if (sym) {
       cudaFuncSetAttribute(grad_partial_tma_kernel<true>, cudaFuncAttributeMaxDynamicSharedMemorySize, (int)kTmaSmemBytes);
-      grad_partial_tma_kernel<true><<<grid, kTmaThreads, kTmaSmemBytes, st>>>(form, X, ldx, w, mu, sigma, n_units, D, upc, partial);
+      grad_partial_tma_kernel<true><<<grid, kTmaThreads, kTmaSmemBytes, st>>>(form, X, ldx, w, mu, sigma, n_units, D, upc, partial, rc);
     } else {
       cudaFuncSetAttribute(grad_partial_tma_kernel<false>, cudaFuncAttributeMaxDynamicSharedMemorySize, (int)kTmaSmemBytes);
-      grad_partial_tma_kernel<false><<<grid, kTmaThreads, kTmaSmemBytes, st>>>(form, X, ldx, w, mu, sigma, n_units, D, upc, partial);
+      grad_partial_tma_kernel<false><<<grid, kTmaThreads, kTmaSmemBytes, st>>>(form, X, ldx, w, mu, sigma, n_units, D, upc, partial, rc);
     }
     EVOK_CHECK_LAUNCH();
     return launch_finalize(partial, n_chunks, D, scale_mu, scale_sigma, out_mu, out_sigma, push, st);
@@ -502,6 +585,15 @@
   return grad_impl(form, X, ldx, w, mu, sigma, 0, n_rows, D, false, 0, 0, nullptr, scale_mu, scale_sigma, out_mu, out_sigma, ws, ws_bytes, stream);
 }
 
+extern "C" EVOK_API int evok_grad_recipe(int form, const float* X, int64_t ldx, const float* w, const float* mu, const float* sigma, int64_t row0,
+                                         int64_t n_rows, int64_t D, uint64_t seed, uint64_t stream_id, const uint32_t* stream_offset_dev,
+                                         const float* mu_s, const float* sigma_s, float scale_mu, float scale_sigma, float* out_mu, float* out_sigma,
+                                         void* ws, size_t ws_bytes, void* stream) {
+  if (!X) return EVOK_E_NULLPTR;
+  return grad_impl(form, X, ldx, w, mu, sigma, row0, n_rows, D, false, seed, stream_id, stream_offset_dev, scale_mu, scale_sigma, out_mu, out_sigma, ws,
+                   ws_bytes, stream, nullptr, mu_s, sigma_s);
+}
+
 extern "C" EVOK_API int evok_grad_regen(int form, const float* w, const float* mu, const float* sigma, int64_t row0, int64_t n_rows, int64_t D,
                                uint64_t seed, uint64_t stream_id, const uint32_t* stream_offset_dev, float scale_mu, float scale_sigma,
                                float* out_mu, float* out_sigma, void* ws, size_t ws_bytes, void* stream) {
@@ -509,10 +601,10 @@
                    ws_bytes, stream);
 }
 
-extern "C" EVOK_API int evok_grad_push(int form, const float* X, int64_t ldx, const float* w, const float* mu, const float* sigma, int64_t row0,
-                                       int64_t n_rows, int64_t D, uint64_t seed, uint64_t stream_id, const uint32_t* stream_offset_dev,
-                                       float scale_mu, float scale_sigma, int world, int rank, void* const* peer_slots, void* const* peer_flags,
-                                       const uint64_t* epoch_dev, uint32_t* done_dev, void* ws, size_t ws_bytes, void* stream) {
+static int grad_push_impl(int form, const float* X, int64_t ldx, const float* w, const float* mu, const float* sigma, int64_t row0, int64_t n_rows,
+                          int64_t D, uint64_t seed, uint64_t stream_id, const uint32_t* stream_offset_dev, const float* mu_s, const float* sigma_s,
+                          float scale_mu, float scale_sigma, int world, int rank, void* const* peer_slots, void* const* peer_flags,
+                          const uint64_t* epoch_dev, uint32_t* done_dev, void* ws, size_t ws_bytes, void* stream) {
   if (!peer_slots || !peer_flags || !epoch_dev || !done_dev) return EVOK_E_NULLPTR;
   if (world < 1 || world > EVOK_MAX_PEERS || rank < 0 || rank >= world) return EVOK_E_BADSIZE;
   GradPush push{};
@@ -526,7 +618,25 @@
   push.epoch = reinterpret_cast<const unsigned long long*>(epoch_dev);
   push.done = done_dev;
   return grad_impl(form, X, X ? ldx : 0, w, mu, sigma, row0, n_rows, D, X == nullptr, seed, stream_id, stream_offset_dev, scale_mu, scale_sigma, nullptr,
-                   nullptr, ws, ws_bytes, stream, &push);
+                   nullptr, ws, ws_bytes, stream, &push, X ? mu_s : nullptr, X ? sigma_s : nullptr);
+}
+
+extern "C" EVOK_API int evok_grad_push(int form, const float* X, int64_t ldx, const float* w, const float* mu, const float* sigma, int64_t row0,
+                                       int64_t n_rows, int64_t D, uint64_t seed, uint64_t stream_id, const uint32_t* stream_offset_dev,
+                                       float scale_mu, float scale_sigma, int world, int rank, void* const* peer_slots, void* const* peer_flags,
+                                       const uint64_t* epoch_dev, uint32_t* done_dev, void* ws, size_t ws_bytes, void* stream) {
+  return grad_push_impl(form, X, ldx, w, mu, sigma, row0, n_rows, D, seed, stream_id, stream_offset_dev, nullptr, nullptr, scale_mu, scale_sigma, world,
+                        rank, peer_slots, peer_flags, epoch_dev, done_dev, ws, ws_bytes, stream);
+}
+
+extern "C" EVOK_API int evok_grad_push_recipe(int form, const float* X, int64_t ldx, const float* w, const float* mu, const float* sigma, int64_t row0,
+                                              int64_t n_rows, int64_t D, uint64_t seed, uint64_t stream_id, const uint32_t* stream_offset_dev,
+                                              const float* mu_s, const float* sigma_s, float scale_mu, float scale_sigma, int world, int rank,
+                                              void* const* peer_slots, void* const* peer_flags, const uint64_t* epoch_dev, uint32_t* done_dev, void* ws,
+                                              size_t ws_bytes, void* stream) {
+  if (!X) return EVOK_E_NULLPTR;
+  return grad_push_impl(form, X, ldx, w, mu, sigma, row0, n_rows, D, seed, stream_id, stream_offset_dev, mu_s, sigma_s, scale_mu, scale_sigma, world, rank,
+                        peer_slots, peer_flags, epoch_dev, done_dev, ws, ws_bytes, stream);
 }
 
 extern "C" EVOK_API size_t evok_grad_batched_workspace_bytes(int64_t n_items, int64_t n_rows, int64_t D) {
diff --git a/evotorch_b200/distributed.py b/evotorch_b200/distributed.py
--- a/evotorch_b200/distributed.py
+++ b/evotorch_b200/distributed.py
@@ -145,7 +145,7 @@
         problem.philox_row0 = 0
         problem._active_peer = None
 
-    samples = batch.recipe if isinstance(batch, LazySolutionBatch) else batch.access_values(keep_evals=True)
+    samples = batch._values_for_gradient(with_recipe=hasattr(dev_dist, "partial_gradients"))
     if sharded_rank:
         offsets = [0]
         for c in counts:
diff --git a/evotorch_b200/distributions.py b/evotorch_b200/distributions.py
--- a/evotorch_b200/distributions.py
+++ b/evotorch_b200/distributions.py
@@ -8,7 +8,7 @@
 import torch
 
 from . import ops
-from .core import PhiloxRecipe
+from .core import PhiloxRecipe, SampledRows
 from .tools.cloning import Clonable
 from .tools.readonlytensor import as_plain_tensor
 from .tools.misc import extract_generator, make_gaussian, to_torch_dtype
@@ -118,6 +118,8 @@
         if ranking_method is None:
             ranking_method = "raw"
         fitnesses = as_plain_tensor(torch.as_tensor(fitnesses, dtype=self.dtype))
+        if isinstance(samples, SampledRows) and not isinstance(self, SeparableGaussian):
+            samples = samples.values
         samples = as_plain_tensor(samples)
         [num_samples, _] = samples.shape
         [num_fitnesses] = fitnesses.shape
@@ -221,19 +223,23 @@
 
     def _weighted_sums(self, form: int, samples: torch.Tensor, w: torch.Tensor, scale_mu: float, scale_sigma: float) -> tuple:
         mu, sigma = self.mu, self.sigma
+        recipe = None
+        if isinstance(samples, SampledRows):
+            samples, recipe = samples.values, samples.recipe
         peer = getattr(self, "_peer", None)
         if peer is not None:
             if isinstance(samples, PhiloxRecipe):
                 ops.grad_push(form, None, w.contiguous(), mu.contiguous(), sigma.contiguous(), scale_mu=scale_mu, scale_sigma=scale_sigma, peer=peer,
                               seed=samples.seed, stream_id=samples.stream_id, row0=samples.row0, stream_offset=samples.stream_offset)
             else:
-                ops.grad_push(form, samples, w.contiguous(), mu.contiguous(), sigma.contiguous(), scale_mu=scale_mu, scale_sigma=scale_sigma, peer=peer)
+                ops.grad_push(form, samples, w.contiguous(), mu.contiguous(), sigma.contiguous(), scale_mu=scale_mu, scale_sigma=scale_sigma, peer=peer,
+                              recipe=recipe)
             return peer.reduce_gradients()
         if isinstance(samples, PhiloxRecipe):
             return ops.grad_regen(form, w.contiguous(), mu.contiguous(), sigma.contiguous(), seed=samples.seed, stream_id=samples.stream_id,
                                   row0=samples.row0, scale_mu=scale_mu, scale_sigma=scale_sigma, stream_offset=samples.stream_offset)
         if ops.uses_kernels(samples) and ops.uses_kernels(w):
-            return ops.grad(form, samples, w.contiguous(), mu.contiguous(), sigma.contiguous(), scale_mu, scale_sigma)
+            return ops.grad(form, samples, w.contiguous(), mu.contiguous(), sigma.contiguous(), scale_mu, scale_sigma, recipe=recipe)
         if form == ops.GRAD_SYMMETRIC:
             eps = samples[0::2] - mu
             a, b = (w[0::2] - w[1::2]) / 2, (w[0::2] + w[1::2]) / 2
diff --git a/evotorch_b200/ops.py b/evotorch_b200/ops.py
--- a/evotorch_b200/ops.py
+++ b/evotorch_b200/ops.py
@@ -141,21 +141,30 @@
 
 
 def grad_push(form: int, X: Optional[torch.Tensor], w: torch.Tensor, mu: torch.Tensor, sigma: torch.Tensor, *, scale_mu: float,
-              scale_sigma: float, peer, seed: int = 0, stream_id: int = 0, row0: int = 0, stream_offset: Optional[torch.Tensor] = None) -> None:
+              scale_sigma: float, peer, seed: int = 0, stream_id: int = 0, row0: int = 0, stream_offset: Optional[torch.Tensor] = None,
+              recipe=None) -> None:
     n, D = w.numel(), mu.numel()
     _vec(w, "weights"); _vec(mu, "mu"); _vec(sigma, "sigma", D)
     ldx = 0
+    r = None
     if X is not None:
         _mat(X, "X")
         if X.shape != (n, D):
             raise ValueError(f"X: expected shape {(n, D)}, got {tuple(X.shape)}")
         ldx = X.stride(0)
+        r = _usable_recipe(recipe, form, n, D)
     ws = nat.workspace(mu.device, nat.lib().evok_grad_workspace_bytes(n, D), "grad")
     with _timed("grad" if X is not None else "grad_regen"):
-        rc = nat.lib().evok_grad_push(form, nat.ptr(X), ldx, w.data_ptr(), mu.data_ptr(), sigma.data_ptr(), row0, n, D, seed & 0xFFFFFFFFFFFFFFFF,
-                                      stream_id & 0xFFFFFFFFFFFFFFFF, _offset_ptr(stream_offset), scale_mu, scale_sigma, peer.world, peer.rank,
-                                      peer.peer_slots, peer.peer_flags_g, peer.epoch_g, peer._counter(1), ws.data_ptr(), ws.numel(),
-                                      nat.stream_of(mu))
+        if r is None:
+            rc = nat.lib().evok_grad_push(form, nat.ptr(X), ldx, w.data_ptr(), mu.data_ptr(), sigma.data_ptr(), row0, n, D, seed & 0xFFFFFFFFFFFFFFFF,
+                                          stream_id & 0xFFFFFFFFFFFFFFFF, _offset_ptr(stream_offset), scale_mu, scale_sigma, peer.world, peer.rank,
+                                          peer.peer_slots, peer.peer_flags_g, peer.epoch_g, peer._counter(1), ws.data_ptr(), ws.numel(),
+                                          nat.stream_of(mu))
+        else:
+            rc = nat.lib().evok_grad_push_recipe(form, X.data_ptr(), ldx, w.data_ptr(), mu.data_ptr(), sigma.data_ptr(), r.row0, n, D,
+                                                 r.seed & 0xFFFFFFFFFFFFFFFF, r.stream_id & 0xFFFFFFFFFFFFFFFF, _offset_ptr(r.stream_offset),
+                                                 r.mu.data_ptr(), r.sigma.data_ptr(), scale_mu, scale_sigma, peer.world, peer.rank, peer.peer_slots,
+                                                 peer.peer_flags_g, peer.epoch_g, peer._counter(1), ws.data_ptr(), ws.numel(), nat.stream_of(mu))
     nat.check(rc, "evok_grad_push")
 
 
@@ -256,17 +265,33 @@
     return mask
 
 
+def _usable_recipe(recipe, form: int, n: int, D: int):
+    if recipe is None:
+        return None
+    if recipe.n_rows != n or recipe.solution_length != D or bool(recipe.symmetric) != (form == GRAD_SYMMETRIC):
+        return None
+    _vec(recipe.mu, "recipe.mu", D); _vec(recipe.sigma, "recipe.sigma", D)
+    return recipe
+
+
 def grad(form: int, X: torch.Tensor, w: torch.Tensor, mu: torch.Tensor, sigma: torch.Tensor, scale_mu: float, scale_sigma: float,
-         out_mu: Optional[torch.Tensor] = None, out_sigma: Optional[torch.Tensor] = None) -> tuple:
+         out_mu: Optional[torch.Tensor] = None, out_sigma: Optional[torch.Tensor] = None, *, recipe=None) -> tuple:
     _mat(X, "samples")
     n, D = X.shape
     _vec(w, "weights", n); _vec(mu, "mu", D); _vec(sigma, "sigma", D)
     out_mu = torch.empty_like(mu) if out_mu is None else _vec(out_mu, "out_mu", D)
     out_sigma = torch.empty_like(mu) if out_sigma is None else _vec(out_sigma, "out_sigma", D)
     ws = nat.workspace(X.device, nat.lib().evok_grad_workspace_bytes(n, D), "grad")
+    r = _usable_recipe(recipe, form, n, D)
     with _timed("grad"):
-        rc = nat.lib().evok_grad(form, X.data_ptr(), X.stride(0), w.data_ptr(), mu.data_ptr(), sigma.data_ptr(), n, D, scale_mu,
-                                 scale_sigma, out_mu.data_ptr(), out_sigma.data_ptr(), ws.data_ptr(), ws.numel(), nat.stream_of(X))
+        if r is None:
+            rc = nat.lib().evok_grad(form, X.data_ptr(), X.stride(0), w.data_ptr(), mu.data_ptr(), sigma.data_ptr(), n, D, scale_mu,
+                                     scale_sigma, out_mu.data_ptr(), out_sigma.data_ptr(), ws.data_ptr(), ws.numel(), nat.stream_of(X))
+        else:
+            rc = nat.lib().evok_grad_recipe(form, X.data_ptr(), X.stride(0), w.data_ptr(), mu.data_ptr(), sigma.data_ptr(), r.row0, n, D,
+                                            r.seed & 0xFFFFFFFFFFFFFFFF, r.stream_id & 0xFFFFFFFFFFFFFFFF, _offset_ptr(r.stream_offset),
+                                            r.mu.data_ptr(), r.sigma.data_ptr(), scale_mu, scale_sigma, out_mu.data_ptr(), out_sigma.data_ptr(),
+                                            ws.data_ptr(), ws.numel(), nat.stream_of(X))
     nat.check(rc, "evok_grad")
     return out_mu, out_sigma
 
diff --git a/include/evok.h b/include/evok.h
--- a/include/evok.h
+++ b/include/evok.h
@@ -70,6 +70,11 @@
 int evok_grad(int form, const float* X, int64_t ldx, const float* w, const float* mu, const float* sigma,
               int64_t n_rows, int64_t D, float scale_mu, float scale_sigma, float* out_mu, float* out_sigma,
               void* ws, size_t ws_bytes, void* stream);
+
+int evok_grad_recipe(int form, const float* X, int64_t ldx, const float* w, const float* mu, const float* sigma, int64_t row0,
+                     int64_t n_rows, int64_t D, uint64_t seed, uint64_t stream_id, const uint32_t* stream_offset_dev,
+                     const float* mu_s, const float* sigma_s, float scale_mu, float scale_sigma, float* out_mu, float* out_sigma,
+                     void* ws, size_t ws_bytes, void* stream);
 
 int evok_grad_regen(int form, const float* w, const float* mu, const float* sigma, int64_t row0, int64_t n_rows,
                     int64_t D, uint64_t seed, uint64_t stream_id, const uint32_t* stream_offset_dev, float scale_mu,
@@ -166,6 +171,11 @@
                    int64_t n_rows, int64_t D, uint64_t seed, uint64_t stream_id, const uint32_t* stream_offset_dev, float scale_mu,
                    float scale_sigma, int world, int rank, void* const* peer_slots_host, void* const* peer_flags_host,
                    const uint64_t* epoch_dev, uint32_t* done_dev, void* ws, size_t ws_bytes, void* stream);
+int evok_grad_push_recipe(int form, const float* X, int64_t ldx, const float* w, const float* mu, const float* sigma, int64_t row0,
+                          int64_t n_rows, int64_t D, uint64_t seed, uint64_t stream_id, const uint32_t* stream_offset_dev,
+                          const float* mu_s, const float* sigma_s, float scale_mu, float scale_sigma, int world, int rank,
+                          void* const* peer_slots_host, void* const* peer_flags_host, const uint64_t* epoch_dev, uint32_t* done_dev,
+                          void* ws, size_t ws_bytes, void* stream);
 int evok_peer_reduce(const float* slots_local, int world, int64_t n, const uint64_t* flags_local, uint64_t* epoch_dev,
                      uint32_t* done_dev, uint32_t* err_dev, uint64_t timeout_ns, float* out, void* stream);
 
```

Result: no change. 47.89, median of 6 (+0.6%).
